# yyNoBug/VAE_segmentation

Measured on AMD Instinct MI355X. Metric: 3D train-step volumes/sec at 96^3 batch=2 (joint VAE+seg), higher is better.
Workload: dtype bf16; 1 GPU; configs[1]: 96^3 joint VAE+seg training step (joint_train), batch=2/GPU, bf16 activations + fp32 accumulate, SGD momentum 0.9, VAE frozen, HIP-graph replay; global_batch=2, parallelism=dp1, activation_recomputation=False, tail_in_graph=True, nranks=1, grad_exchange=none (1 rank)

## Files before the change

### include/vaeseg.h

```cpp
#ifndef VAESEG_H
#define VAESEG_H
#include <stddef.h>
#include <stdint.h>

#ifdef __cplusplus
extern "C" {
#endif

#define VS_VERSION 500

enum { VS_F32 = 0, VS_BF16 = 1, VS_F16 = 2, VS_F32X3 = 3  };
#ifndef VS_STAT_SLOTS
#define VS_STAT_SLOTS 4
#endif
enum { VS_OK = 0, VS_EINVAL = -1, VS_ESHAPE = -2, VS_EDTYPE = -3, VS_EWORKSPACE = -4, VS_EALIGN = -5 };

enum {
    VS_CONV_K3 = 0,
    VS_CONV_K2S2 = 1,
    VS_CONV_T2S2 = 2,
    VS_WGRAD_SLABS = 16,
    VS_CONV_UP = 3
};

// ... 1 lines not shown
    VS_PACK_ROWS_D0 = 0,
    VS_PACK_ROWS_D1_FLIP = 1,
    VS_PACK_SCATTER_D1 = 2
};

int vs_version(void);
int vs_stat_slots(void);
int vs_stat_interleaved(void);
const char* vs_strerror(int code);
int vs_get_deterministic(void);

int vs_up_supported(int cin, int cm, int co, int dtype);
int vs_up_compose_sizes(int cin, int cm, int co, size_t* out6);
int vs_up_compose(const float* w2, const float* b2, const float* w3, float* weff, void* img_fwd, void* img_bwd, int* taps_fwd, int* taps_bwd,
                  float* btab, int cin, int cm, int co, int dtype, void* stream);
int vs_up_conv_fwd(const void* x, const double* x_stats, const void* img_fwd, const int* taps_fwd, const float* btab, void* y, double* y_stats,
                   int n, int d, int h, int w, int cin, int co, int dtype, float eps, void* stream);
int vs_up_faces(const void* gy, double* G, int n, int fd, int fh, int fw, int co, int dtype, void* stream);
int vs_up_chain(const float* dweff27, const double* G, const float* w2, const float* b2, const float* w3, float* dw2, float* db2, float* dw3,
                int cin, int cm, int co, void* stream);
int vs_up_conv_bwd_data(const void* gy, const void* img_bwd, const int* taps_bwd, void* gx, const void* mask_x, const double* mask_stats,
                        double* sums, int n, int d, int h, int w, int co, int cin, int dtype, float eps, void* stream);

size_t vs_packed_weight_bytes(int rows, int c_pad, int ntaps, int dtype);
int vs_pack_weight(const float* src, void* dst, int d0, int d1, int ntaps, int c_pad, int form, int dtype, void* stream);

typedef struct vs_pack_desc {
    const float* src;
    void* dst;
    int d0, d1, ntaps, c_pad, form, dtype;
    int first_block;
    int pad_;
    long long total;
} vs_pack_desc;
int vs_pack_weight_multi(const vs_pack_desc* descs, int n_desc, int total_blocks, void* stream);

int vs_conv_gather_fwd(const void* x, const double* x_stats, const void* w_packed, const float* bias,
                       void* y, double* y_stats, int n, int d, int h, int w, int c_in, int m_out,
                       int kind, int dtype, float eps, void* stream);

int vs_conv_scatter_fwd(const void* x, const double* x_stats, const void* w_packed, const float* bias,
                        void* y, int n, int d, int h, int w, int c_in, int m_out, int dtype, float eps, void* stream);

int vs_conv_gather_bwd_data(const void* x, const void* w_packed, void* y, const void* mask_x, const double* mask_stats,
                            double* sums, int n, int d, int h, int w, int c_in, int m_out, int kind, int dtype, float eps,
                            void* stream);
int vs_conv_scatter_bwd_data(const void* x, const void* w_packed, void* y, const void* mask_x, const double* mask_stats,
                             double* sums, int n, int d, int h, int w, int c_in, int m_out, int dtype, float eps, void* stream);
int vs_conv_k3_fused_apply_supported(int n, int d, int h, int w, int c_in, int m_out, int lazy_input, int dtype);
int vs_conv_k3_bwd_data_wgrad_supported(int n, int d, int h, int w, int c_in, int m_out, int dtype);
int vs_conv_k3_bwd_data_wgrad_slabs(int n, int d, int h, int w);
int vs_conv_k3_bwd_data_wgrad(const void* g, const void* act_x, const double* act_stats, const double* act_sums, const void* w_packed, void* y,
                              const void* mask_x, const double* mask_stats, double* sums, float* slabs, int n, int d, int h, int w, int c_in,
                              int m_out, int dtype, float eps, void* stream);
int vs_conv_k3_softmax2_bwd_data(const float* prob, const float* gprob, const void* gprob_cl, const void* w_packed, void* y, const void* mask_x,
                                 const double* mask_stats, double* sums, float* slabs, double* bias_part, int n, int d, int h, int w, int dtype,
                                 float eps, float drop_p, unsigned long long drop_seed, void* stream);
typedef struct vs_config {
    int k3_small;
    int k3_tall;
    int k3_wgs_per_cu;
    int k3t_wgs_per_cu;
    int k3f_min_wgs;
    int mt_min_wgs;
    int f32_limbs;
    int g1_limbs;
    int k3x_ck;
    int k3x_toeplitz;
    int fuse_wgrad;
    int epilogue_apply;
    int chain;
    int k2s2_stream;
    int k2s8_wgs_per_cu;
    int up_wgs_per_cu;
    int up_rb;
    int wgrad_uber;
    int wgrad_mpack;
    int wgrad_swap;
    int wgrad_big;
    int wgrad_xcd;
    int k3_short_tiles;
    int wgrad_bias_fold;
    int hist_form;
    long long wgrad_wgs;
    long long wgrad_f32_tiles;
    long long wgrad_group_wgs;
    long long wgrad_big_min_voxels;
} vs_config;
int vs_config_bytes(void);
int vs_config_from_env(vs_config* c);
int vs_get_config(vs_config* out);
int vs_set_config(const vs_config* cfg);
int vs_conv_k3_bwd_data_applied_supported(int n, int d, int h, int w, int c_in, int m_out, int dtype);
int vs_conv_k3_bwd_data_applied(const void* x, const void* w_packed, void* y, const void* mask_x, const double* mask_stats, double* sums,
                                unsigned int* sync, unsigned int* fault, int n, int d, int h, int w, int c_in, int m_out, int dtype, float eps, void* stream);
int vs_conv_s2_bwd_data_applied_supported(int n, int d, int h, int w, int c_in, int m_out, int scatter, int dtype);
int vs_conv_s2_bwd_data_applied(const void* x, const void* w_packed, void* y, const void* mask_x, const double* mask_stats, double* sums, const void* add,
                                unsigned int* sync, unsigned int* fault, int n, int d, int h, int w, int c_in, int m_out, int scatter, int dtype, float eps,
                                void* stream);
typedef struct vs_chain_layer {
    const void* x;
    const double* x_stats;
    const void* w_packed;
    void* y;
    double* y_stats;
    const void* mask_x;
    const double* mask_stats;
    double* sums;
    int c_in, m_out;
    int apply;
    int reserved_;
} vs_chain_layer;
int vs_conv_k3_chain_supported(int n, int d, int h, int w, int c_max, int dtype);
long long vs_conv_k3_chain_sync_bytes(int n);
int vs_conv_k3_chain(const vs_chain_layer* layers, int n_layers, int backward, const void* add, unsigned int* sync, unsigned int* fault,
                     int n, int d, int h, int w, int dtype, float eps, void* stream);
int vs_conv_k3_f32_limbs(int d, int h, int w, int c_in);

int vs_conv_k3_bwd_data_fused_apply(const void* g, const void* act_x, const double* act_stats, const double* act_sums,
                                    const void* w_packed, void* y, const void* mask_x, const double* mask_stats, double* sums,
                                    void* dx_out, int n, int d, int h, int w, int c_in, int m_out, int dtype, float eps, void* stream);

int vs_conv_k3_softmax2_fwd(const void* x, const double* x_stats, const void* w_packed, const float* bias,
                            float* prob, int n, int d, int h, int w, int c_in, int dtype, float eps, void* stream);
int vs_conv_k3_softmax2_dropout_fwd(const void* x, const double* x_stats, const void* w_packed, const float* bias,
                                    float* prob, int n, int d, int h, int w, int c_in, int dtype, float eps, float drop_p,
                                    unsigned long long drop_seed, void* stream);
int vs_conv_k3_softmax2_cl_fwd(const void* x, const double* x_stats, const void* w_packed, const float* bias,
                               float* prob, void* prob_cl, int n, int d, int h, int w, int c_in, int dtype, float eps, float drop_p,
                               unsigned long long drop_seed, void* stream);

size_t vs_conv_wgrad_workspace_bytes(int n, int dp, int hp, int wp, int m_ch, int c_ch, int kind);
int vs_conv_wgrad(const void* p, const double* p_stats, const void* q, const double* q_stats, float* dw,
                  void* workspace, size_t workspace_bytes, int n, int dp, int hp, int wp, int m_ch, int c_ch,
                  int m_real, int c_real, int kind, int dtype, float eps, void* stream);
typedef struct vs_wgrad_desc {
    const void* p; const double* p_stats;
    const void* q; const double* q_stats;
    float* dw;
    const void* bias_g; float* db;
    long long bias_rows;
    int bias_c_ch, bias_c_real;
    int n, dp, hp, wp, m_ch, c_ch, m_real, c_real, kind;
    int reserved_;
} vs_wgrad_desc;
size_t vs_conv_wgrad_multi_workspace_bytes(const vs_wgrad_desc* descs, int count, int dtype);
int vs_conv_wgrad_multi(const vs_wgrad_desc* descs, int count, void* workspace, size_t workspace_bytes, int dtype,
                        float eps, void* stream);
int vs_bias_grad(const void* g, float* db, long long rows, int c_ch, int c_real, int dtype, void* stream);
int vs_bias_grad_acc(const void* g, float* db, long long rows, int c_ch, int c_real, int dtype, int accumulate, void* stream);

int vs_instnorm_stats(const void* x, double* stats, int n, long long voxels, int c, int dtype, void* stream);
int vs_instnorm_relu_fwd(const void* x, const double* x_stats, const void* x2, const double* x2_stats,
                         void* out, int n, long long voxels, int c, int dtype, float eps, void* stream);
int vs_instnorm_relu_bwd_reduce(const void* g, const void* x, const double* x_stats, double* sums,
                                int n, long long voxels, int c, int dtype, float eps, void* stream);
int vs_instnorm_relu_bwd_apply(const void* g, const void* x, const double* x_stats, const double* sums,
                               void* gx, int n, long long voxels, int c, int dtype, float eps, void* stream);
int vs_instnorm_relu_bwd_apply_add(const void* g, const void* x, const double* x_stats, const double* sums, const void* add,
                                   void* gx, int n, long long voxels, int c, int dtype, float eps, void* stream);
int vs_zero_fill(void* p, long long bytes, void* stream);
int vs_instnorm_relu_bwd_pair(const void* g, const void* x1, const double* x1_stats, double* sums1, void* gx1,
                              const void* x2, const double* x2_stats, double* sums2, void* gx2, int n, long long voxels,
                              int c, int dtype, float eps, void* stream);

enum { VS_NORM_INSTANCE = 0, VS_NORM_BATCH = 1, VS_NORM_BATCH_EVAL = 2, VS_NORM_NONE = 3 };
// ... 89 lines not shown
int vs_fill_holes(const float* mask, float* out, int n, int c, int d, int h, int w, int connectivity, void* workspace, void* stream);

int vs_region_props(const int* labels, int n, int c, int d, int h, int w, int max_rows, long long* table, int* overflow, void* stream);
int vs_contingency(const int* a, const int* b, int n, int c, int d, int h, int w, int rows_a, int rows_b, long long* table, int* overflow,
                   void* stream);

int vs_histogram(const float* x, const int* labels, int n, int c, int d, int h, int w, int bins, int rows, double lo, double hi, int from_data,
                 double* edges, long long* table, long long* outside, int* overflow, void* stream);
int vs_joint_histogram(const float* x, const float* y, int n, int c, int d, int h, int w, int bins_x, int bins_y, const double* range4, int from_data,
                       double* edges_x, double* edges_y, long long* table, long long* outside, void* stream);
int vs_mutual_information(const long long* table, int n, int c, int bins_x, int bins_y, double sigma, int normalized, double* workspace, double* mi,
                          void* stream);

size_t vs_quantile_workspace_bytes(int planes, long long V, int Q);
int vs_quantile(const float* x, const unsigned char* mask, int use_above, float above, const double* p01, int Q, double* q_out, float* lo_out,
                float* hi_out, long long* count, long long* rejected, void* workspace, int planes, int d, int h, int w, void* stream);
int vs_intensity_map(const float* x, const double* src, const double* dst, int L, int clamp, float* y, int planes, int d, int h, int w, void* stream);

#define VS_PATCH_CHUNK 4096
enum { VS_PATCH_F32 = 0, VS_PATCH_U8 = 1 };
int vs_patch_chunk(void);
size_t vs_patch_index_bytes(int d, int h, int w, int n_class);
int vs_patch_index(const void* label, int dtype, int d, int h, int w, int n_class, int* table, void* stream);
int vs_patch_pick(const void* label, int dtype, const int* table, int n_class, int n_sel, int classes, const unsigned int* words, const int* forced,
                  int r, int d, int h, int w, int pd, int ph, int pw, int* picks, void* stream);
int vs_patch_gather(const float* src0, const float* src1, const float* src2, const float* src3, float cval0, float cval1, float cval2, float cval3,
                    int n_src, const int* picks, int r, int d, int h, int w, int pd, int ph, int pw, int margin, float* out, void* stream);

int vs_sw_plan(int d, int h, int w, int patch, double overlap, int* origins, int capacity);
int vs_sw_gather(const float* volume, float* batch, const int* origins, const int* first, int nw, int b, int c, int d, int h, int w, int patch,
                 float cval, void* stream);
int vs_sw_accumulate(const float* prob, float* acc, float* wsum, const int* origins, const int* first, int nw, int b, int k, int d, int h, int w,
                     int patch, const float* wz, const float* wy, const float* wx, void* stream);
int vs_sw_gather_tta(const float* volume, float* batch, const int* origins, const int* first, int nw, int b, int c, int d, int h, int w, int patch,
                     float cval, int nf, int codes, void* stream);
int vs_sw_accumulate_tta(const float* prob, float* acc, float* wsum, const int* origins, const int* first, int nw, int b, int k, int d, int h, int w,
                         int patch, const float* wz, const float* wy, const float* wx, int nf, int codes, void* stream);
int vs_sw_finalize(const float* acc, const float* wsum, float* prob, unsigned char* label, float* onehot, int k, int d, int h, int w, void* stream);

int vs_uncrop(const float* prob, unsigned char* label, float* prob_out, int k, int patch, int d, int h, int w, int lo_z, int lo_y, int lo_x,
              int hi_z, int hi_y, int hi_x, int off_z, int off_y, int off_x, int side, int interp, void* stream);

enum { VS_SCAN_I16 = 0, VS_SCAN_U8 = 1, VS_SCAN_I8 = 2, VS_SCAN_F32 = 3 };
int vs_scan_orient(const void* raw, int dtype, float* out, int x, int y, int z, int flip0, int flip1, int flip2, void* stream);
int vs_scan_to_native(const void* src, int src_is_label, unsigned char* label, float* prob_out, int k, int d1, int h1, int w1, int x, int y, int z,
                      int flip0, int flip1, int flip2, int interp, void* stream);

int vs_linear_fwd(const void* x, int x_dtype, const float* wgt, const float* bias, float* y, int batch, int k_in,
                  int j_out, int pc, int pv, int relu, void* stream);
int vs_linear_fwd_pair(const void* x, int x_dtype, const float* w1, const float* b1, float* y1, int relu1, const float* w2,
                       const float* b2, float* y2, int relu2, int batch, int k_in, int j_out, int pc, int pv, void* stream);
int vs_linear_fwd_perm_out(const float* z, const float* wgt, const float* bias, void* y, int y_dtype, int batch,
                           int k_in, int j_out, int pc, int pv, void* stream);
int vs_linear_bwd(const void* x, int x_dtype, const float* wgt, const float* gy, const float* y_for_relu,
                  void* gx, float* gw, float* gb, int batch, int k_in, int j_out, int pc, int pv, void* stream);
int vs_linear_perm_out_bwd(const float* z, const float* wgt, const void* gy, int y_dtype, float* gz, float* gw,
                           float* gb, int batch, int k_in, int j_out, int pc, int pv, void* stream);

int vs_reparam_fwd(const float* mean, const float* std_, const float* noise, float scale, float* z, long long count, void* stream);
int vs_reparam_bwd(const float* gz, const float* noise, float scale, float* gmean, float* gstd, long long count, void* stream);
int vs_latent_normal_philox(float* noise, long long count, unsigned long long seed, unsigned long long draw, void* stream);
int vs_reparam_philox_fwd(const float* mean, const float* std_, const unsigned long long* state, float scale, float* z, float* noise_out,
                          long long count, void* stream);
int vs_latent_advance(unsigned long long* state, void* stream);
int vs_kl_fwd(const float* mean, const float* std_, float* out, int batch, int dim, void* stream);
int vs_kl_bwd(const float* mean, const float* std_, const float* gout, float* gmean, float* gstd, int batch, int dim, void* stream);

int vs_dice_fwd(const float* s, const float* t, double* sums, float* per_sample, float* mean_out,
                int batch, int channels, long long voxels, int bot, int top, float eps, void* stream);
int vs_dice_bwd(const float* s, const float* t, const double* sums, const float* gout, int gout_is_mean, float* gs,
                float* gt, int batch, int channels, long long voxels, int bot, int top, float eps, void* stream);
size_t vs_dice_loss_multi_scratch_doubles(int k, int batch, int channels);
int vs_dice_loss_multi_fwd(const float* s, const float* const* t, const float* w, int k, double* scratch, float* terms,
                           float* final_out, int batch, int channels, long long voxels, int bot, int top, float eps, void* stream);
int vs_dice_loss_multi_bwd(const float* s, const float* const* t, const float* w, int k, const double* scratch,
                           const float* gout, float* gs, float* const* gt, int batch, int channels, long long voxels,
                           int bot, int top, float eps, void* stream);
int vs_dice_loss_multi_labels_fwd(const float* s, const float* const* t, const float* const* labels, const float* w, int k, double* scratch,
                                  float* terms, float* final_out, int batch, int channels, long long voxels, int bot, int top, float eps,
                                  void* stream);
int vs_dice_loss_multi_labels_bwd(const float* s, const float* const* t, const float* const* labels, const float* w, int k,
                                  const double* scratch, const float* gout, float* gs, float* const* gt, int batch, int channels,
                                  long long voxels, int bot, int top, float eps, void* stream);
size_t vs_seg_loss_scratch_doubles(int batch, int channels);
int vs_seg_loss_fwd(const float* p, const float* label, const float* class_w, double* scratch, float* terms, float* final_out, int batch, int channels,
                    long long voxels, int bot, int top, float eps, float dice_w, float ce_w, int batch_dice, float gamma, void* stream);
int vs_seg_loss_bwd(const float* p, const float* label, const float* class_w, const double* scratch, const float* gout, float* gp, int batch, int channels,
                    long long voxels, int bot, int top, float eps, float dice_w, float ce_w, int batch_dice, float gamma, void* stream);
int vs_bce_fwd(const float* p, const float* t, float* out, double* scratch, long long count, void* stream);
int vs_bce_bwd(const float* p, const float* t, const float* gout, float* gp, long long count, void* stream);

int vs_sgd_momentum_multi(float* const* params, const float* const* grads, float* const* bufs, const long long* sizes,
                          const int* block_map, int n_blocks, float lr, float momentum, float weight_decay,
                          int first_step, void* stream);
int vs_adam_multi(float* const* params, const float* const* grads, float* const* exp_avg, float* const* exp_avg_sq,
                  const long long* sizes, const int* block_map, int n_blocks, float lr, double beta1, double beta2,
                  float eps, float weight_decay, int step, void* stream);
int vs_sgd_momentum_scaled_multi(float* const* params, const float* const* grads, float* const* bufs, const long long* sizes,
                                 const int* block_map, int n_blocks, float lr, float momentum, float weight_decay,
                                 int first_step, const float* loss_scale, const float* found_inf, void* stream);
int vs_sgd_momentum_dev_multi(float* const* params, const float* const* grads, float* const* bufs, const long long* sizes,
                              const int* block_map, int n_blocks, const float* hyper, const float* loss_scale,
                              const float* found_inf, void* stream);
int vs_adam_scaled_multi(float* const* params, const float* const* grads, float* const* exp_avg, float* const* exp_avg_sq,
                         const long long* sizes, const int* block_map, int n_blocks, float lr, double beta1, double beta2,
                         float eps, float weight_decay, int step, const float* loss_scale, const float* found_inf, void* stream);
int vs_grad_finite_multi(const float* const* grads, const long long* sizes, const int* block_map, int n_blocks,
                         float* found_inf, void* stream);
int vs_loss_scale_update(float* scale, int* growth_tracker, float* found_inf, float growth_factor, float backoff_factor,
                         int growth_interval, void* stream);
int vs_ema_multi(float* const* teacher, const float* const* student, const long long* sizes, const int* block_map,
                 int n_blocks, float alpha, void* stream);
int vs_copy_scale_multi(const float* const* srcs, float* const* dsts, const long long* sizes, const int* block_map,
                        int n_blocks, float scale, void* stream);
int vs_scale_copy(const float* src, float* dst, long long count, float scale, void* stream);

#ifdef __cplusplus
}
#endif
#endif
```

### vae_segmentation_amd/csrc/common.h

```cpp
#pragma once
#include <hip/hip_runtime.h>
#include <stdint.h>
#include <stdlib.h>
#include <type_traits>
#include "../../include/vaeseg.h"

const vs_config& vs_cfg();

typedef __attribute__((ext_vector_type(8))) __bf16 bf16x8;
typedef _Float16 vs_half;
typedef __attribute__((ext_vector_type(8))) _Float16 f16x8;
typedef __attribute__((ext_vector_type(2))) _Float16 f16x2;
typedef __attribute__((ext_vector_type(4))) float f32x4;
typedef __attribute__((ext_vector_type(4))) unsigned int u32x4;
typedef __attribute__((ext_vector_type(2))) unsigned int u32x2;

#define VS_WAVE 64

__device__ __forceinline__ float bf2f(unsigned short h) { return __uint_as_float(((unsigned int)h) << 16); }
__device__ __forceinline__ unsigned short f2bf(float f) {
    __bf16 b = (__bf16)f;
    return __builtin_bit_cast(unsigned short, b);
}
__device__ __forceinline__ float round_bf(float f) { return bf2f(f2bf(f)); }
// ... 192 lines not shown
        r -= q * down[s];
        atomicAdd((unsigned long long*)(st + stat_index(pair, pairs, s) + which), (unsigned long long)(long long)q);
    }
#else
    atomicAdd(st + stat_index(pair, pairs, (int)(blockIdx.x & (VS_STAT_SLOTS - 1))) + which, tot);
#endif
}

__device__ __forceinline__ void pair_to_mean_rstd(const double (&st)[2], double inv_count, float eps, float& mean, float& rstd) {
    double m = st[0] * inv_count;
    double var = st[1] * inv_count - m * m;
    if (var < 0.0) var = 0.0;
    mean = (float)m;
    rstd = (float)(1.0 / sqrt(var + (double)eps));
}
__device__ __forceinline__ void stats_to_mean_rstd(const double* st, size_t pair, size_t pairs, double inv_count, float eps, float& mean, float& rstd) {
    double v[2];
    stat_load(st, pair, pairs, v);
    pair_to_mean_rstd(v, inv_count, eps, mean, rstd);
}

__device__ __forceinline__ void stats_to_mean_rstd_fast(const double* st, double inv_count, float eps, float& mean, float& rstd) {
    const double m = st[0] * inv_count;
    double var = st[1] * inv_count - m * m;
    if (var < 0.0) var = 0.0;
    const float v = (float)(var + (double)eps);
    float r = rsqrtf(v);
    r = r * (1.5f - 0.5f * v * r * r);
    mean = (float)m;
    rstd = r;
}
__device__ __forceinline__ void stats_to_mean_rstd_fast(const double* st, size_t pair, size_t pairs, double inv_count, float eps, float& mean, float& rstd) {
    double v[2];
    stat_load(st, pair, pairs, v);
    stats_to_mean_rstd_fast(v, inv_count, eps, mean, rstd);
}

__device__ __forceinline__ float hash_uniform(unsigned long long seed, unsigned long long idx) {
    unsigned long long x = idx * 0x9E3779B97F4A7C15ull + seed;
    x = (x ^ (x >> 30)) * 0xBF58476D1CE4E5B9ull;
    x = (x ^ (x >> 27)) * 0x94D049BB133111EBull;
    x ^= x >> 31;
    return (float)(x >> 40) * (1.0f / 16777216.0f);
}
__device__ __forceinline__ float dropout_scale(unsigned long long seed, unsigned long long idx, float p) {
    return hash_uniform(seed, idx) >= p ? 1.0f / (1.0f - p) : 0.0f;
}

typedef __attribute__((ext_vector_type(2))) float f32x2;
typedef __attribute__((ext_vector_type(2))) short i16x2;
typedef __attribute__((ext_vector_type(2))) __bf16 bf16x2;
typedef __attribute__((ext_vector_type(4))) int i32x4;

__device__ i32x4 vs_raw_buffer_load_b128(i32x4 rsrc, int voffset, int soffset, int aux) __asm("llvm.amdgcn.raw.buffer.load.v4i32");

typedef __attribute__((ext_vector_type(2))) int i32x2;
__device__ i32x2 vs_raw_buffer_load_b64(i32x4 rsrc, int voffset, int soffset, int aux) __asm("llvm.amdgcn.raw.buffer.load.v2i32");
__device__ int vs_raw_buffer_load_b32(i32x4 rsrc, int voffset, int soffset, int aux) __asm("llvm.amdgcn.raw.buffer.load.i32");
__device__ void vs_raw_buffer_store_b128(i32x4 data, i32x4 rsrc, int voffset, int soffset, int aux) __asm("llvm.amdgcn.raw.buffer.store.v4i32");
__device__ void vs_raw_buffer_store_b64(i32x2 data, i32x4 rsrc, int voffset, int soffset, int aux) __asm("llvm.amdgcn.raw.buffer.store.v2i32");

__device__ __forceinline__ int fdiv(int n, unsigned int m, unsigned int sh) { return (int)((__umulhi((unsigned int)n, m) + (unsigned int)n) >> sh); }

__device__ __forceinline__ i32x4 make_rsrc(const void* base, unsigned int bytes) {
    const unsigned long long a = (unsigned long long)base;
    i32x4 r;
    r[0] = (int)(unsigned int)a;
    r[1] = (int)(unsigned int)((a >> 32) & 0xffffu);
    r[2] = (int)bytes;
    r[3] = 0x00020000;
    return r;
}

__device__ __forceinline__ float vs_in_bwd_apply1(float g, float x, float mean, float rstd, float m1, float m2) {
#pragma clang fp contract(off)
    const float xh = (x - mean) * rstd;
    const float gm = xh > 0.f ? g : 0.f;
    const float base = gm - m1;
    float out = rstd * __builtin_fmaf(-xh, m2, base);
    asm volatile("" : "+v"(out));
    return out;
}

template <typename T> struct H16;
template <> struct H16<unsigned short> {
    __device__ static __forceinline__ unsigned int pack2(f32x2 v) { return __builtin_bit_cast(unsigned int, __builtin_convertvector(v, bf16x2)); }
    __device__ static __forceinline__ float lo(unsigned int w) { return __uint_as_float(w << 16); }
    __device__ static __forceinline__ float hi(unsigned int w) { return __uint_as_float(w & 0xffff0000u); }
};
template <> struct H16<vs_half> {
    __device__ static __forceinline__ unsigned int pack2(f32x2 v) { return __builtin_bit_cast(unsigned int, __builtin_convertvector(v, f16x2)); }
    __device__ static __forceinline__ float lo(unsigned int w) { return (float)__builtin_bit_cast(f16x2, w)[0]; }
    __device__ static __forceinline__ float hi(unsigned int w) { return (float)__builtin_bit_cast(f16x2, w)[1]; }
};

template <typename T>
__device__ __forceinline__ void store4(T* p, const float (&v)[4]) {
    if constexpr (sizeof(T) == 4) {
        *(f32x4*)p = f32x4{v[0], v[1], v[2], v[3]};
    } else {
        u32x2 pk;
        pk[0] = H16<T>::pack2(f32x2{v[0], v[1]});
        pk[1] = H16<T>::pack2(f32x2{v[2], v[3]});
        *(u32x2*)p = pk;
    }
}
template <typename T>
__device__ __forceinline__ void widen4(const unsigned int* w, float (&v)[4]) {
    if constexpr (sizeof(T) == 4) {
        v[0] = __uint_as_float(w[0]); v[1] = __uint_as_float(w[1]); v[2] = __uint_as_float(w[2]); v[3] = __uint_as_float(w[3]);
    } else {
        v[0] = H16<T>::lo(w[0]); v[1] = H16<T>::hi(w[0]); v[2] = H16<T>::lo(w[1]); v[3] = H16<T>::hi(w[1]);
    }
}

template <typename T>
__device__ __forceinline__ u32x4 act8(const u32x4 raw, const f32x2 (&sc)[4], const f32x2 (&sh)[4]) {
    u32x4 r;
#pragma unroll
    for (int i = 0; i < 4; ++i) {
        f32x2 v;
        v[0] = H16<T>::lo(raw[i]);
        v[1] = H16<T>::hi(raw[i]);
        v = v * sc[i] + sh[i];
        i16x2 s = __builtin_bit_cast(i16x2, H16<T>::pack2(v));
        s = __builtin_elementwise_max(s, i16x2{0, 0});
        r[i] = __builtin_bit_cast(unsigned int, s);
    }
    return r;
}

__device__ __forceinline__ void vs_limb_split4(const float (&v)[4], unsigned int (&out)[3][2]) {
#pragma unroll
    for (int q = 0; q < 2; ++q) {
        const f32x2 x = f32x2{v[2 * q], v[2 * q + 1]};
        const unsigned int p0 = H16<unsigned short>::pack2(x);
        const f32x2 r1 = x - f32x2{H16<unsigned short>::lo(p0), H16<unsigned short>::hi(p0)};
        const unsigned int p1 = H16<unsigned short>::pack2(r1);
        const f32x2 r2 = r1 - f32x2{H16<unsigned short>::lo(p1), H16<unsigned short>::hi(p1)};
        out[0][q] = p0; out[1][q] = p1; out[2][q] = H16<unsigned short>::pack2(r2);
    }
}

__device__ __forceinline__ void vs_limb_pair(const u32x4& f0, const u32x4& f1, u32x4 (&out)[3]) {
    float v0[4], v1[4];
#pragma unroll
    for (int j = 0; j < 4; ++j) { v0[j] = __uint_as_float(f0[j]); v1[j] = __uint_as_float(f1[j]); }
    unsigned int l0[3][2], l1[3][2];
    vs_limb_split4(v0, l0);
    vs_limb_split4(v1, l1);
#pragma unroll
    for (int l = 0; l < 3; ++l) out[l] = u32x4{l0[l][0], l0[l][1], l1[l][0], l1[l][1]};
}
__device__ __forceinline__ void vs_limb_mfma(const u32x4 (&al)[3], const u32x4 (&bl)[3], f32x4& lead, f32x4& small) {
    small = mfma16(al[0], bl[2], small, (unsigned short*)nullptr);
    small = mfma16(al[1], bl[1], small, (unsigned short*)nullptr);
    small = mfma16(al[2], bl[0], small, (unsigned short*)nullptr);
    small = mfma16(al[0], bl[1], small, (unsigned short*)nullptr);
    small = mfma16(al[1], bl[0], small, (unsigned short*)nullptr);
    lead = mfma16(al[0], bl[0], lead, (unsigned short*)nullptr);
}

static __host__ __device__ inline bool vs_k3_toeplitz(int rows, int c_pad, int ntaps, int dtype) {
    return (dtype == VS_BF16 || dtype == VS_F16) && ntaps == 27 && c_pad == 8 && rows <= 8;
}
static __host__ __device__ inline bool vs_k3_toeplitz_f32(int rows, int c_pad, int ntaps, int dtype) {
// ... 38 lines not shown
```

### vae_segmentation_amd/csrc/config.hip

```cpp
#include <mutex>
#include <stdlib.h>
#include "common.h"

static vs_config g_cfg;
static std::once_flag g_cfg_once;
static std::mutex g_cfg_mutex;

static int env_int(const char* name, int dflt) { const char* s = getenv(name); return s ? atoi(s) : dflt; }
static long long env_ll(const char* name, long long dflt) { const char* s = getenv(name); return s ? atoll(s) : dflt; }

extern "C" int vs_config_from_env(vs_config* c) {
    if (!c) return VS_EINVAL;
    c->k3_small = env_int("VS_K3_SMALL", 1);
    c->k3_tall = env_int("VS_K3_TALL", -1);
    c->k3_wgs_per_cu = env_int("VS_K3_WGS_PER_CU", 0);
    c->k3t_wgs_per_cu = env_int("VS_K3T_WGS_PER_CU", 2);
    c->k3f_min_wgs = env_int("VS_K3F_MIN_WGS", 512);
    c->mt_min_wgs = env_int("VS_MT_MIN_WGS", 1024);
    c->f32_limbs = env_int("VS_F32_LIMBS", 1);
    c->g1_limbs = env_int("VS_G1_LIMBS", 1);
    c->k3x_ck = env_int("VS_K3X_CK", 8);
    c->k3x_toeplitz = env_int("VS_K3X_TOEPLITZ", 1);
    c->fuse_wgrad = env_int("VS_FUSE_WGRAD", 1);
    c->epilogue_apply = env_int("VS_EPILOGUE_APPLY", 1);
    c->chain = env_int("VS_CHAIN", 1);
    c->k2s2_stream = env_int("VS_K2S2_STREAM", 1);
    c->k2s8_wgs_per_cu = env_int("VS_K2S8_WGS_PER_CU", 4);
    c->up_wgs_per_cu = env_int("VS_UP_WGS_PER_CU", 2);
    c->up_rb = env_int("VS_UP_RB", 0);
    c->wgrad_uber = env_int("VS_WGRAD_UBER", 1);
    c->wgrad_mpack = env_int("VS_WGRAD_MPACK", 1);
    c->wgrad_swap = env_int("VS_WGRAD_SWAP", 1);
    c->wgrad_big = env_int("VS_WGRAD_BIG", 1);
    c->wgrad_xcd = env_int("VS_WGRAD_XCD", 2);
    c->k3_short_tiles = env_int("VS_K3_SHORT_TILES", 2);
    c->wgrad_bias_fold = env_int("VS_WGRAD_BIAS_FOLD", 1);
    c->hist_form = env_int("VS_HIST_FORM", 0);
    c->wgrad_wgs = env_ll("VS_WGRAD_WGS", 512);
    c->wgrad_f32_tiles = env_ll("VS_WGRAD_F32_TILES", 8);
    c->wgrad_group_wgs = env_ll("VS_WGRAD_GROUP_WGS", 0);
    c->wgrad_big_min_voxels = env_ll("VS_WGRAD_BIG_MIN_VOXELS", 400000);
    return VS_OK;
}

const vs_config& vs_cfg() {
    std::call_once(g_cfg_once, [] { vs_config_from_env(&g_cfg); });
    return g_cfg;
}

extern "C" int vs_config_bytes(void) { return (int)sizeof(vs_config); }

extern "C" int vs_get_config(vs_config* out) {
    if (!out) return VS_EINVAL;
    const vs_config& c = vs_cfg();
    std::lock_guard<std::mutex> lock(g_cfg_mutex);
    *out = c;
    return VS_OK;
}

extern "C" int vs_set_config(const vs_config* in) {
    if (!in) return VS_EINVAL;
    if (in->k3x_ck != 8 && in->k3x_ck != 16) return VS_EINVAL;
    if (in->k3_wgs_per_cu < 0 || in->k3t_wgs_per_cu < 1 || in->k2s8_wgs_per_cu < 1 || in->up_wgs_per_cu < 1 || in->wgrad_wgs < 1 || in->wgrad_f32_tiles < 1 ||
        in->wgrad_group_wgs < 0 || in->wgrad_big_min_voxels < 0 || in->mt_min_wgs < 0 || in->k3f_min_wgs < 0 || in->hist_form < 0 || in->hist_form > 3) return VS_EINVAL;
    vs_cfg();
    std::lock_guard<std::mutex> lock(g_cfg_mutex);
    g_cfg = *in;
    return VS_OK;
}
```

### vae_segmentation_amd/csrc/conv_api.hip

```cpp
#include <stdlib.h>
#include "igemm_dispatch.h"

int g1_dispatch_k3_f32(const G1Params& p, int ck, int mt, int epi, int tiles, int row_tiles, hipStream_t s);
int g1_dispatch_k3_bf16(const G1Params& p, int ck, int mt, int epi, int tiles, int row_tiles, hipStream_t s);
int g1_dispatch_k3_f16(const G1Params& p, int ck, int mt, int epi, int tiles, int row_tiles, hipStream_t s);
int g1_dispatch_k3_x3(const G1Params& p, int ck, int mt, int epi, int tiles, int row_tiles, hipStream_t s);
int g1_k3_fa_supported(const G1Params& p, int ck, int mt, int lazy_in);
int g1_k3_ea_supported(const G1Params& p, int ck, int mt, long long wgs);
int k3x_fa_supported(const G1Params& p, int ck, int mt);
int k3x_ea_supported(const G1Params& p, int ck, int mt, long long wgs);
int k3tw_slab_count(int n, int d, int h, int w);
int k2s2_scatter8_launch(const G1Params& p, int dtype, hipStream_t stream);

extern "C" int vs_conv_k3_f32_limbs(int d, int h, int w, int c_in) {
    const int on = vs_cfg().f32_limbs;
    if (!on) return 0;
    const int small = vs_cfg().k3_small;
    if (small && c_in % 32 == 0 && c_in <= 1024 && (long long)(d + 2) * (h + 2) * (w + 2) <= 512) return 0;
    return 1;
}

struct ConvTiles { int ck, mt, row_tiles; bool limbs; };

static ConvTiles k3_tiles(G1Params& p, int dtype, int ck, int mt, int rows16, long long tiles) {
// ... 220 lines not shown
    return plan_wgrad(n, d, h, w, c_in, m_out, false, dtype).status == VS_OK;
}

extern "C" int vs_conv_k3_bwd_data_wgrad_slabs(int n, int d, int h, int w) {
    if (n <= 0 || d <= 0 || h <= 0 || w <= 0) return 0;
    return k3tw_slab_count(n, d, h, w);
}

extern "C" int vs_conv_k3_bwd_data_wgrad(const void* g, const void* act_x, const double* act_stats, const double* act_sums, const void* w_packed, void* y,
                                         const void* mask_x, const double* mask_stats, double* sums, float* slabs, int n, int d, int h, int w, int c_in,
                                         int m_out, int dtype, float eps, void* stream) {
    if (!g || !slabs || !mask_x || !mask_stats || !sums) return VS_EINVAL;
    if ((act_x == nullptr) != (act_stats == nullptr) || (act_x == nullptr) != (act_sums == nullptr)) return VS_EINVAL;
    const ConvPlan pl = plan_wgrad(n, d, h, w, c_in, m_out, act_x != nullptr, dtype);
    if (pl.status) return VS_ESHAPE;
    if (((uintptr_t)slabs & 15) || (act_x && ((uintptr_t)act_x & 15))) return VS_EALIGN;
    G1Params p = bwd_params(pl, g, w_packed, y, mask_x, mask_stats, sums, eps);
    p.x_stats = act_stats; p.fa_x = act_x; p.fa_sums = act_sums; p.wg_ws = slabs;
    return launch_conv(pl, p, stream);
}

extern "C" int vs_conv_k3_softmax2_bwd_data(const float* prob, const float* gprob, const void* gprob_cl, const void* w_packed, void* y, const void* mask_x,
                                            const double* mask_stats, double* sums, float* slabs, double* bias_part, int n, int d, int h, int w, int dtype,
                                            float eps, float drop_p, unsigned long long drop_seed, void* stream) {
    if (!prob || (!gprob && !gprob_cl) || !w_packed || !y || !mask_x || !mask_stats || !sums) return VS_EINVAL;
    if (bias_part && !slabs) return VS_EINVAL;
    const ConvPlan pl = plan_wgrad(n, d, h, w, 8, 8, false, dtype);
    if (pl.status) return VS_ESHAPE;
    if (((uintptr_t)w_packed & 15) || ((uintptr_t)y & 15) || ((uintptr_t)mask_x & 15) || (gprob_cl && ((uintptr_t)gprob_cl & 15)) || (slabs && ((uintptr_t)slabs & 15)) ||
        ((uintptr_t)prob & 3) || ((uintptr_t)gprob & 3)) return VS_EALIGN;
    if (!(drop_p >= 0.f && drop_p < 1.f)) return VS_EINVAL;
    G1Params p = bwd_params(pl, nullptr, w_packed, y, mask_x, mask_stats, sums, eps);
    p.sm_prob = prob; p.sm_gprob = gprob; p.sm_gcl = gprob_cl; p.wg_ws = slabs; p.wg_bias = bias_part;
    p.drop_p = drop_p; p.drop_seed = drop_seed;
    return dispatch_k3(p, dtype, pl.t, EPI_RAW, 0, (hipStream_t)stream);
}

extern "C" int vs_conv_scatter_fwd(const void* x, const double* x_stats, const void* w_packed, const float* bias, void* y,
                                   int n, int d, int h, int w, int c_in, int m_out, int dtype, float eps, void* stream) {
    const ConvPlan pl = plan_scatter({n, d, h, w, c_in, m_out, VS_CONV_T2S2, dtype, (x_stats ? X_STATS : 0) | (bias ? BIAS : 0)});
    G1Params p = pl.g;
    p.x = x; p.x_stats = x_stats; p.wp = w_packed; p.bias = bias; p.y = y; p.eps = eps;
    return launch_conv(pl, p, stream);
}

extern "C" int vs_conv_scatter_bwd_data(const void* x, const void* w_packed, void* y, const void* mask_x, const double* mask_stats, double* sums,
                                        int n, int d, int h, int w, int c_in, int m_out, int dtype, float eps, void* stream) {
    if (!mask_x || !mask_stats || !sums) return VS_EINVAL;
    const ConvPlan pl = plan_scatter({n, d, h, w, c_in, m_out, VS_CONV_T2S2, dtype, SUMS});
    return launch_conv(pl, bwd_params(pl, x, w_packed, y, mask_x, mask_stats, sums, eps), stream);
}

static ConvPlan plan_s2_applied(int n, int d, int h, int w, int c_in, int m_out, int scatter, int dtype) {
    return scatter ? plan_scatter({n, d, h, w, c_in, m_out, VS_CONV_T2S2, dtype, SUMS | EA}) : plan_gather({n, d, h, w, c_in, m_out, VS_CONV_K2S2, dtype, SUMS | EA});
}
extern "C" int vs_conv_s2_bwd_data_applied_supported(int n, int d, int h, int w, int c_in, int m_out, int scatter, int dtype) {
    return plan_s2_applied(n, d, h, w, c_in, m_out, scatter, dtype).status == VS_OK;
}

extern "C" int vs_conv_s2_bwd_data_applied(const void* x, const void* w_packed, void* y, const void* mask_x, const double* mask_stats, double* sums, const void* add,
                                           unsigned int* sync, unsigned int* fault, int n, int d, int h, int w, int c_in, int m_out, int scatter, int dtype, float eps,
                                           void* stream) {
    if (!mask_x || !mask_stats || !sums || !sync || !fault) return VS_EINVAL;
    if (((uintptr_t)sync & 127) || ((uintptr_t)fault & 3) || (add && ((uintptr_t)add & 15))) return VS_EALIGN;
    const ConvPlan pl = plan_s2_applied(n, d, h, w, c_in, m_out, scatter, dtype);
    if (pl.status) return VS_ESHAPE;
    G1Params p = bwd_params(pl, x, w_packed, y, mask_x, mask_stats, sums, eps);
    p.ea_sync = sync; p.ea_fault = fault; p.ea_add = add;
    return launch_conv(pl, p, stream);
}

extern "C" int vs_conv_k3_softmax2_fwd(const void* x, const double* x_stats, const void* w_packed, const float* bias,
                                       float* prob, int n, int d, int h, int w, int c_in, int dtype, float eps,
                                       void* stream) {
    return vs_conv_k3_softmax2_dropout_fwd(x, x_stats, w_packed, bias, prob, n, d, h, w, c_in, dtype, eps, 0.f, 0ull, stream);
}

extern "C" int vs_conv_k3_softmax2_dropout_fwd(const void* x, const double* x_stats, const void* w_packed, const float* bias,
                                               float* prob, int n, int d, int h, int w, int c_in, int dtype, float eps,
                                               float drop_p, unsigned long long drop_seed, void* stream) {
    return vs_conv_k3_softmax2_cl_fwd(x, x_stats, w_packed, bias, prob, nullptr, n, d, h, w, c_in, dtype, eps, drop_p, drop_seed, stream);
}

extern "C" int vs_conv_k3_softmax2_cl_fwd(const void* x, const double* x_stats, const void* w_packed, const float* bias, float* prob, void* prob_cl,
                                          int n, int d, int h, int w, int c_in, int dtype, float eps, float drop_p, unsigned long long drop_seed, void* stream) {
    if (drop_p < 0.f || drop_p >= 1.f) return VS_EINVAL;
    if (prob_cl && dtype == VS_F32) return VS_EDTYPE;
    if (prob_cl && ((uintptr_t)prob_cl & 15)) return VS_EALIGN;
    int rc = check_common(x, w_packed, n, d, h, w, c_in, dtype);
    if (rc) return rc;
    if (!prob || c_in != 8) return VS_ESHAPE;
    const ConvPlan pl = plan_gather({n, d, h, w, 8, 8, VS_CONV_K3, dtype, 0});
    G1Params p = pl.g;
    p.x = x; p.x_stats = x_stats; p.wp = w_packed; p.bias = bias; p.y = prob_cl; p.prob = prob; p.eps = eps;
    p.drop_p = drop_p; p.drop_seed = drop_seed;
    return dispatch_k3(p, dtype, pl.t, EPI_SOFTMAX2, (int)pl.tiles, (hipStream_t)stream);
}
```

### vae_segmentation_amd/csrc/igemm.h

```cpp
#pragma once
#include <type_traits>
#include "common.h"
#include "handoff.h"

enum { G1_K3 = 0, G1_K2S2 = 1, G1_PW = 2 };
enum { EPI_RAW = 0, EPI_SOFTMAX2 = 1, EPI_SCATTER = 2 };

struct G1Params {
    const void* x;
    const double* x_stats;
    const void* wp;
    const float* bias;
    void* y;
    double* y_stats;
    float* prob;
    const void* mask_x;
    const double* mask_stats;
    double* sums;
    double inv_count_out;
    float drop_p;
    unsigned long long drop_seed;
    int N, D, H, W;
    int Do, Ho, Wo;
    int C;
    int M;
    int rb_total;
    int nch;
    int tiles_per_sample;
    int tyn, txn;
    float eps;
    double inv_count_in;
    unsigned int fd_m[3], fd_s[3];
    const void* fa_x;
    const double* fa_sums;
    void* fa_dx;
    const void* up_taps;
    const float* up_btab;
    int up_co;
    float* wg_ws;
    const float* sm_prob;
    const float* sm_gprob;
    const void* sm_gcl;
    double* wg_bias;
    unsigned int* ea_sync;
    unsigned int* ea_fault;
    int ea_items;
    const void* ea_add;
};

#define G1_LDS_MEAN 0
#define G1_LDS_RSTD 2048
#define G1_LDS_RED 4096
#define G1_LDS_BYTES 6144
#define G1_TILE_VOX 648

template <typename T, int CK>
__device__ __forceinline__ u32x4 act_transform(u32x4 raw, const float* s_mean, const float* s_rstd, int c0) {
    constexpr int EPL = ET<T>::EPL;
    float v[EPL];
    frag_unpack(raw, v, (T*)nullptr);
#pragma unroll
    for (int j = 0; j < EPL; ++j) {
        float t = (v[j] - s_mean[c0 + j]) * s_rstd[c0 + j];
        v[j] = t > 0.f ? t : 0.f;
    }
    return frag_pack(v, (T*)nullptr);
}

template <typename T, int CK, int KIND, int MT, int EPI, bool LIMB = false, bool EA = false>
__global__ __launch_bounds__(256) void g1_kernel(const G1Params p) {
    using E = ET<T>;
    constexpr int EPL = E::EPL, KG = E::KG;
    static_assert(!LIMB || sizeof(T) == 4, "limb arithmetic: fp32 storage");
    static_assert(KIND == G1_K2S2 || KIND == G1_PW, "the 3x3x3 kernels live in igemm_k3b.h / igemm_k3.h");
    static_assert(EPI == EPI_RAW || EPI == EPI_SCATTER, "softmax epilogue: 3x3x3 kernels only");
    constexpr int NTAPS = KIND == G1_K2S2 ? 8 : 1;
    constexpr int NKG = (NTAPS * CK + KG - 1) / KG;
    constexpr int RB = MT / 16;
    constexpr int CKB = CK * (int)sizeof(T);
    constexpr int TPK = KG > CK ? KG / CK : 1;
    constexpr int KPT = KG > CK ? 1 : CK / KG;
    extern __shared__ __attribute__((aligned(16))) char smem[];
    float* s_mean = (float*)(smem + G1_LDS_MEAN);
    float* s_rstd = (float*)(smem + G1_LDS_RSTD);
    float* s_red = (float*)(smem + G1_LDS_RED);

    const int tid = threadIdx.x;
    const int lane = tid & 63;
    const int wave = tid >> 6;
    const int col = lane & 15;
    const int g = lane >> 4;
    const int n = blockIdx.x / p.tiles_per_sample;
    const int tile = blockIdx.x - n * p.tiles_per_sample;
    const int rb0 = blockIdx.y * RB;
    const bool has_stats = p.x_stats != nullptr;
    const T* __restrict__ xin = (const T*)p.x;

    if (has_stats) {
        for (int c = tid; c < p.C; c += 256) {
            float m, r;
            stats_to_mean_rstd(p.x_stats, (size_t)n * p.C + c, (size_t)p.N * p.C, p.inv_count_in, p.eps, m, r);
            s_mean[c] = m;
            s_rstd[c] = r;
        }
    }
    if (p.sums != nullptr) {
        for (int c = tid; c < p.M; c += 256) {
            float m, r;
            stats_to_mean_rstd(p.mask_stats, (size_t)n * p.M + c, (size_t)p.N * p.M, p.inv_count_out, p.eps, m, r);
            s_mean[c] = m;
            s_rstd[c] = r;
        }
    }
    const bool splitw = KIND == G1_K2S2 && CK == 32 && p.tyn == 64;
    const int cwave = splitw ? 0 : wave;
    const int ctile = splitw ? 64 : 256;
    long long gofs[4];
    bool cvalid[4];
    int oz[4], oy[4], ox[4];
    {
        const int vcol = p.Do * p.Ho * p.Wo;
#pragma unroll
        for (int cg = 0; cg < 4; ++cg) {
            int v = tile * ctile + cwave * 64 + cg * 16 + col;
            cvalid[cg] = v < vcol;
            if (!cvalid[cg]) v = 0;
            ox[cg] = v % p.Wo;
            const int t2 = v / p.Wo;
            oy[cg] = t2 % p.Ho;
            oz[cg] = t2 / p.Ho;
// ... 429 lines not shown
```

### vae_segmentation_amd/csrc/igemm_k3t.h

```cpp
#pragma once
#include <stdlib.h>
#include "igemm_tile.h"

#define K3T_LDS_RED 0
#define K3T_LDS_TILE 512

template <int YT>
struct K3TGeom {
    static constexpr int PX = 34, PY = YT + 2, PLANE = PX * PY, TV = 6 * PLANE;
    static constexpr int TILE_BYTES = ((TV + 255) / 256) * 256 * 16;
    static constexpr int NIT = (TV + 255) / 256;
};

template <int EPI, bool SUMS, int YT, bool HS, typename T = unsigned short, bool FA = false>
__global__ __launch_bounds__(256) __attribute__((amdgpu_waves_per_eu(2, 2))) void k3t_kernel(const G1Params p) {
    K3_TICK_INIT
    using GEO = K3TGeom<YT>;
    constexpr int PX = GEO::PX, PY = GEO::PY, PLANE = GEO::PLANE, TV = GEO::TV, NIT = GEO::NIT;
    extern __shared__ __attribute__((aligned(16))) char smem[];
    float* s_red = (float*)(smem + K3T_LDS_RED);
    char* s_tile = smem + K3T_LDS_TILE;
    float* s_scale = (float*)(s_tile + GEO::TILE_BYTES);
    float* s_shift = s_scale + p.N * 8;
    float* s_mkm = s_shift + p.N * 8;
    float* s_mkr = s_mkm + p.N * 8;
    float* s_fa = s_mkr + p.N * 8;
    static_assert(!FA || (!HS && EPI == EPI_RAW), "fused apply: backward-data use (materialised gradient in), with or without the fused IN-backward sums");

    const int tid = threadIdx.x, lane = tid & 63, wave = tid >> 6, col = lane & 15, g = lane >> 4;
    const int dx2 = g >> 1, c4 = 4 * (g & 1);
    constexpr bool has_stats = HS;
    const int total_tiles = p.tiles_per_sample * p.N;
    const i32x4 xrsrc = make_rsrc(p.x, (unsigned int)((long long)p.N * p.D * p.H * p.W * 16));
    const i32x4 frsrc = make_rsrc(FA ? p.fa_x : p.x, (unsigned int)((long long)p.N * p.D * p.H * p.W * 16));
    const i32x4 dxrsrc = make_rsrc(FA && p.fa_dx != nullptr ? p.fa_dx : p.y, (FA && p.fa_dx != nullptr) ? (unsigned int)((long long)p.N * p.D * p.H * p.W * 16) : 0u);

    const double* st_src = SUMS ? p.mask_stats : p.x_stats;
    const int st_n = SUMS ? p.N * 8 : (has_stats ? p.N * 8 : 0);
    double st_pre[2] = {0.0, 1.0};
    if (tid < st_n) stat_load(st_src, (size_t)tid, (size_t)st_n, st_pre);
    double fa_pre[2][2] = {{0.0, 1.0}, {0.0, 0.0}};
    if constexpr (FA) {
        if (tid >= 64 && tid < 64 + p.N * 8) {
            stat_load(p.x_stats, (size_t)(tid - 64), (size_t)p.N * 8, fa_pre[0]);
            stat_load(p.fa_sums, (size_t)(tid - 64), (size_t)p.N * 8, fa_pre[1]);
        }
    }

    int rel_off[NIT], tzyx[NIT];
    unsigned int cbits = 0;
#pragma unroll
    for (int b = 0; b < NIT; ++b) {
        const int tv = tid + b * 256;
        const int tx_ = tv % PX, ty_ = (tv / PX) % PY, tz_ = tv / PLANE;
        rel_off[b] = ((tz_ * p.H + ty_) * p.W + tx_) * 16;
        tzyx[b] = tv < TV ? (tz_ | (ty_ << 8) | (tx_ << 16)) : 0x00ffffff;
        cbits |= (tv < TV && tz_ >= 1 && tz_ <= 4 && ty_ >= 1 && ty_ <= YT && tx_ >= 1 && tx_ <= 32) ? (1u << b) : 0u;
    }
    u32x4 xv[NIT], fv[FA ? NIT : 1];
    unsigned int okbits = 0;
    auto load_x = [&](const TileCoord& c) {
        const int base = (((c.n * p.D + c.z0 - 1) * p.H + c.y0 - 1) * p.W + c.x0 - 1) * 16;
        okbits = 0;
#pragma unroll
        for (int b = 0; b < NIT; ++b) {
            const int gz = c.z0 - 1 + (tzyx[b] & 0xff), gy = c.y0 - 1 + ((tzyx[b] >> 8) & 0xff), gx = c.x0 - 1 + (tzyx[b] >> 16);
            const bool ok = (unsigned)gz < (unsigned)p.D && (unsigned)gy < (unsigned)p.H && (unsigned)gx < (unsigned)p.W;
            okbits |= ok ? (1u << b) : 0u;
            xv[b] = __builtin_bit_cast(u32x4, vs_raw_buffer_load_b128(xrsrc, ok ? base + rel_off[b] : -1, 0, 0));
            if constexpr (FA) fv[b] = __builtin_bit_cast(u32x4, vs_raw_buffer_load_b128(frsrc, ok ? base + rel_off[b] : -1, 0, 0));
        }
    };
    auto write_x_fa = [&](const TileCoord& c) {
        f32x2 r2[4], s2[4], a2[4], b2[4];
#pragma unroll
        for (int i = 0; i < 4; ++i) {
            r2[i] = *(const f32x2*)(s_fa + 0 * p.N * 8 + c.n * 8 + 2 * i);
            s2[i] = *(const f32x2*)(s_fa + 1 * p.N * 8 + c.n * 8 + 2 * i);
            a2[i] = *(const f32x2*)(s_fa + 2 * p.N * 8 + c.n * 8 + 2 * i);
            b2[i] = *(const f32x2*)(s_fa + 3 * p.N * 8 + c.n * 8 + 2 * i);
        }
        const int base = (((c.n * p.D + c.z0 - 1) * p.H + c.y0 - 1) * p.W + c.x0 - 1) * 16;
#pragma unroll
        for (int b = 0; b < NIT; ++b) {
            u32x4 v;
#pragma unroll
            for (int i = 0; i < 4; ++i) {
                f32x2 g2, x2;
                g2[0] = H16<T>::lo(xv[b][i]); g2[1] = H16<T>::hi(xv[b][i]);
                x2[0] = H16<T>::lo(fv[b][i]); x2[1] = H16<T>::hi(fv[b][i]);
                const f32x2 xh = x2 * r2[i] + s2[i];
                f32x2 gm;
                gm[0] = xh[0] > 0.f ? g2[0] : 0.f;
                gm[1] = xh[1] > 0.f ? g2[1] : 0.f;
                const f32x2 d = r2[i] * (gm - a2[i] - xh * b2[i]);
                v[i] = H16<T>::pack2(d);
            }
            const bool ok = (okbits >> b) & 1u;
#pragma unroll
            for (int i = 0; i < 4; ++i) v[i] = ok ? v[i] : 0u;
            *(u32x4*)(s_tile + (tid + b * 256) * 16) = v;
            if (p.fa_dx != nullptr)
                vs_raw_buffer_store_b128(__builtin_bit_cast(i32x4, v), dxrsrc, (ok && ((cbits >> b) & 1u)) ? base + rel_off[b] : -1, 0, 0);
        }
    };
    auto write_x = [&](int n) {
        f32x2 sc[4], sh[4];
        if (has_stats) {
#pragma unroll
            for (int i = 0; i < 4; ++i) {
                sc[i] = *(const f32x2*)(s_scale + n * 8 + 2 * i);
                sh[i] = *(const f32x2*)(s_shift + n * 8 + 2 * i);
            }
        }
#pragma unroll
        for (int b = 0; b < NIT; ++b) {
            u32x4 v = xv[b];
            if (has_stats) {
                const u32x4 a = act8<T>(v, sc, sh);
                const bool ok = (okbits >> b) & 1u;
#pragma unroll
                for (int i = 0; i < 4; ++i) v[i] = ok ? a[i] : 0u;
            }
            *(u32x4*)(s_tile + (tid + b * 256) * 16) = v;
        }
    };

    int t, t_end, G;
    tile_walk(total_tiles, t, t_end, G);
    TileCoord cur = tile_coord<YT, 32>(p, t < t_end ? t : 0), nxt = cur;
    u32x4 wa[9];
    {
        const u32x4* __restrict__ wp = (const u32x4*)p.wp;
#pragma unroll
        for (int kg = 0; kg < 9; ++kg) wa[kg] = wp[kg * 64 + lane];
    }
    if (t < t_end) load_x(cur);
    float bv[4];
#pragma unroll
    for (int r = 0; r < 4; ++r) bv[r] = (p.bias != nullptr && c4 + r < (EPI == EPI_SOFTMAX2 ? 2 : p.M)) ? p.bias[c4 + r] : 0.f;
    const i32x4 yrsrc = make_rsrc(p.y, (unsigned int)((long long)p.N * p.D * p.H * p.W * 16));
    const i32x4 mrsrc = make_rsrc(p.mask_x, (unsigned int)((long long)p.N * p.D * p.H * p.W * 16));
    for (int i = tid; i < st_n; i += 256) {
        double st[2] = {st_pre[0], st_pre[1]};
        if (i != tid) stat_load(st_src, (size_t)i, (size_t)st_n, st);
        float m, r;
        stats_to_mean_rstd_fast(st, SUMS ? p.inv_count_out : p.inv_count_in, p.eps, m, r);
        if constexpr (SUMS) { s_mkm[i] = m; s_mkr[i] = r; }
        else { s_scale[i] = r; s_shift[i] = -m * r; }
    }
    if constexpr (FA) {
        if (tid >= 64 && tid < 64 + p.N * 8) {
            const int i = tid - 64;
            float m, r;
            stats_to_mean_rstd_fast(fa_pre[0], p.inv_count_in, p.eps, m, r);
            s_fa[0 * p.N * 8 + i] = r;
            s_fa[1 * p.N * 8 + i] = -m * r;
            s_fa[2 * p.N * 8 + i] = (float)(fa_pre[1][0] * p.inv_count_in);
            s_fa[3 * p.N * 8 + i] = (float)(fa_pre[1][1] * p.inv_count_in);
        }
    }
    const char* s_b = s_tile + ((wave * PY) * PX + 2 * col + g) * 16;
    float ssum[4] = {0.f, 0.f, 0.f, 0.f}, ssq[4] = {0.f, 0.f, 0.f, 0.f};
#pragma unroll
    for (int r = 0; r < 4; ++r) asm volatile("" : "+v"(bv[r]));
#pragma unroll
    for (int kg = 0; kg < 9; ++kg) asm volatile("" : "+v"(wa[kg]));
    bool first = true;
    __syncthreads();
    K3_TICK(0);

    for (; t < t_end; t += G) {
        const int n = cur.n, z0 = cur.z0, y0 = cur.y0, x0 = cur.x0;
        const int oz = z0 + wave, ox = x0 + 2 * col + dx2;
        const int ebase = ((((n * p.D + oz) * p.H + y0) * p.W + ox) * 8 + c4) * 2;
        const bool zx_ok = oz < p.D && ox < p.W;
        if (!first) __syncthreads();
        first = false;
        K3_TICK(1);
        if constexpr (FA) write_x_fa(cur); else write_x(n);
        K3_TICK(2);
        __syncthreads();
        K3_TICK(3);
        u32x2 mk[YT];
        if constexpr (SUMS) {
#pragma unroll
            for (int cg = 0; cg < YT; ++cg)
                mk[cg] = __builtin_bit_cast(u32x2, vs_raw_buffer_load_b64(mrsrc, (zx_ok && y0 + cg < p.H) ? ebase + cg * p.W * 16 : -1, 0, 0));
        }
        nxt = tile_coord<YT, 32>(p, t + G < t_end ? t + G : t);
        if (t + G < t_end) load_x(nxt);
        K3_TICK(4);

        f32x4 acc[YT];
#pragma unroll
        for (int cg = 0; cg < YT; ++cg) acc[cg] = f32x4{0.f, 0.f, 0.f, 0.f};
#pragma unroll
        for (int tz = 0; tz < 3; ++tz) {
            u32x4 fb[PY];
#pragma unroll
            for (int yy = 0; yy < PY; ++yy) fb[yy] = *(const u32x4*)(s_b + ((tz * PY + yy) * PX) * 16);
#pragma unroll
            for (int ty = 0; ty < 3; ++ty)
#pragma unroll
                for (int cg = 0; cg < YT; ++cg) acc[cg] = mfma16(wa[tz * 3 + ty], fb[cg + ty], acc[cg], (T*)nullptr);
            __builtin_amdgcn_sched_barrier(0);
        }

        K3_TICK(5);
        if constexpr (EPI == EPI_SOFTMAX2) {
            const size_t V = (size_t)p.D * p.H * p.W;
#pragma unroll
            for (int cg = 0; cg < YT; ++cg) {
                const int oy = y0 + cg;
                const bool valid = zx_ok && oy < p.H;
                float l0 = acc[cg][0] + bv[0], l1 = acc[cg][1] + bv[1];
                const size_t v = ((size_t)oz * p.H + oy) * p.W + ox;
                if (p.drop_p > 0.f) {
                    l0 *= dropout_scale(p.drop_seed, ((unsigned long long)n * 2 + 0) * V + v, p.drop_p);
                    l1 *= dropout_scale(p.drop_seed, ((unsigned long long)n * 2 + 1) * V + v, p.drop_p);
                }
                const float mx = fmaxf(l0, l1);
                const float e0 = __expf(l0 - mx), e1 = __expf(l1 - mx);
                const float inv = 1.f / (e0 + e1);
                if (valid && (g & 1) == 0) {
                    p.prob[((size_t)n * 2 + 0) * V + v] = e0 * inv;
                    p.prob[((size_t)n * 2 + 1) * V + v] = e1 * inv;
                }
                if (p.y != nullptr) {
                    f32x2 pr;
                    pr[0] = e0 * inv; pr[1] = e1 * inv;
                    i32x2 pk;
                    pk[0] = (g & 1) == 0 ? (int)H16<T>::pack2(pr) : 0;
                    pk[1] = 0;
                    vs_raw_buffer_store_b64(pk, yrsrc, valid ? ebase + cg * p.W * 16 : -1, 0, 0);
                }
            }
        } else {
            float mm[4] = {0.f, 0.f, 0.f, 0.f}, mr[4] = {0.f, 0.f, 0.f, 0.f};
            if constexpr (SUMS) {
#pragma unroll
                for (int r = 0; r < 4; ++r) { mm[r] = s_mkm[n * 8 + c4 + r]; mr[r] = s_mkr[n * 8 + c4 + r]; }
            }
#pragma unroll
            for (int cg = 0; cg < YT; ++cg) {
                const bool valid = zx_ok && y0 + cg < p.H;
                f32x2 lo, hi;
                lo[0] = acc[cg][0] + bv[0]; lo[1] = acc[cg][1] + bv[1];
                hi[0] = acc[cg][2] + bv[2]; hi[1] = acc[cg][3] + bv[3];
                i32x2 pk;
                pk[0] = (int)H16<T>::pack2(lo);
                pk[1] = (int)H16<T>::pack2(hi);
                vs_raw_buffer_store_b64(pk, yrsrc, valid ? ebase + cg * p.W * 16 : -1, 0, 0);
                float v[4];
                v[0] = H16<T>::lo((unsigned int)pk[0]); v[1] = H16<T>::hi((unsigned int)pk[0]);
                v[2] = H16<T>::lo((unsigned int)pk[1]); v[3] = H16<T>::hi((unsigned int)pk[1]);
                if (!valid) { v[0] = 0.f; v[1] = 0.f; v[2] = 0.f; v[3] = 0.f; }
                if constexpr (SUMS) {
                    const u32x2 xx = mk[cg];
                    float xv4[4];
                    xv4[0] = H16<T>::lo(xx[0]); xv4[1] = H16<T>::hi(xx[0]);
                    xv4[2] = H16<T>::lo(xx[1]); xv4[3] = H16<T>::hi(xx[1]);
#pragma unroll
                    for (int r = 0; r < 4; ++r) {
                        const float xh = (xv4[r] - mm[r]) * mr[r];
                        const float gm = xh > 0.f ? v[r] : 0.f;
                        ssum[r] += gm; ssq[r] += gm * xh;
                    }
                } else {
#pragma unroll
                    for (int r = 0; r < 4; ++r) { ssum[r] += v[r]; ssq[r] += v[r] * v[r]; }
                }
            }
            double* const red_dst0 = SUMS ? p.sums : p.y_stats;
            double* const red_dst = red_dst0;
            if (red_dst != nullptr) {
                const bool flush = t + G >= t_end || nxt.n != n;
                if (flush) {
#pragma unroll
                    for (int r = 0; r < 4; ++r) {
                        float s = ssum[r], q = ssq[r];
                        { s = row16_sum(s); q = row16_sum(q); }
                        s += __shfl_xor(s, 32, 64); q += __shfl_xor(q, 32, 64);
                        if (col == 0 && dx2 == 0) {
                            s_red[(wave * 8 + c4 + r) * 2 + 0] = s;
                            s_red[(wave * 8 + c4 + r) * 2 + 1] = q;
                        }
                        ssum[r] = 0.f; ssq[r] = 0.f;
                    }
                    __syncthreads();
                    if (tid < 16) {
                        const int ch = tid >> 1, st = tid & 1;
                        if (ch < p.M) {
                            const double tot = (double)s_red[(0 * 8 + ch) * 2 + st] + (double)s_red[(1 * 8 + ch) * 2 + st] +
                                               (double)s_red[(2 * 8 + ch) * 2 + st] + (double)s_red[(3 * 8 + ch) * 2 + st];
                            stat_add(red_dst, (size_t)n * 8 + ch, (size_t)p.N * 8, st, tot);
                        }
                    }
                }
            }
        }
        cur = nxt;
        K3_TICK(6);
    }
    K3_TICK_FLUSH;
}

template <typename T, int EPI, bool SUMS, int YT, bool HS, bool FA = false>
static int k3t_launch_t(const G1Params& p_in, hipStream_t stream) {
    using GEO = K3TGeom<YT>;
    G1Params p = p_in;
    if (p.C != 8 || p.M != 8) return VS_ESHAPE;
    if (FA && p.N * 8 > 192) return VS_ESHAPE;
    const size_t lds = K3T_LDS_TILE + (size_t)GEO::TILE_BYTES + (size_t)(FA ? 8 : 4) * p.N * 8 * sizeof(float);
    if (lds > 160 * 1024) return VS_ESHAPE;
    p.txn = (p.W + 31) / 32;
    p.tyn = (p.H + YT - 1) / YT;
    p.tiles_per_sample = ((p.D + 3) / 4) * p.tyn * p.txn;
    const long long tiles = (long long)p.tiles_per_sample * p.N;
    if ((long long)p.N * p.D * p.H * p.W * 16 >= 2147483648ll || tiles >= 2147483647ll) return VS_ESHAPE;
    tile_fastdiv_fill(p);
    if (SUMS != (p.sums != nullptr) || (SUMS && !FA && p.x_stats != nullptr)) return VS_EINVAL;
    if (FA && (!p.x_stats || !p.fa_x || !p.fa_sums)) return VS_EINVAL;
    auto kern = k3t_kernel<EPI, SUMS, YT, HS, T, FA>;
    static const hipError_t attr_err =
        hipFuncSetAttribute((const void*)kern, hipFuncAttributeMaxDynamicSharedMemorySize, 160 * 1024);
    if (attr_err != hipSuccess) return (int)attr_err;
    const int per_cu = vs_cfg().k3t_wgs_per_cu;
    const int cap = 256 * per_cu;
    const int gx = tiles < cap ? (int)tiles : cap;
    hipLaunchKernelGGL(kern, dim3(gx), dim3(256), lds, stream, p);
    VS_CHECK_LAUNCH();
    return VS_OK;
}

template <typename T, int EPI, bool SUMS, int YT>
static int k3t_launch(const G1Params& p, hipStream_t stream) {
    if constexpr (EPI == EPI_RAW) {
        if (p.fa_x != nullptr) return k3t_launch_t<T, EPI, SUMS, YT, false, true>(p, stream);
    }
    if (!SUMS && p.x_stats != nullptr) return k3t_launch_t<T, EPI, SUMS, YT, !SUMS>(p, stream);
    return k3t_launch_t<T, EPI, SUMS, YT, false>(p, stream);
}
```

### vae_segmentation_amd/csrc/igemm_k3tw.h

```cpp
#pragma once
#include <stdlib.h>
#include "igemm_tile.h"
#include "igemm_k3t.h"

typedef __attribute__((ext_vector_type(4))) short k3tw_s16x4;
typedef __attribute__((address_space(3))) k3tw_s16x4 k3tw_lds_s16x4;
__device__ __forceinline__ u32x4 pw_tr_pair(const char* s_base, int off0, int off1) {
    const k3tw_s16x4 lo = __builtin_amdgcn_ds_read_tr16_b64_v4i16((k3tw_lds_s16x4*)(s_base + off0));
    const k3tw_s16x4 hi = __builtin_amdgcn_ds_read_tr16_b64_v4i16((k3tw_lds_s16x4*)(s_base + off1));
    typedef __attribute__((ext_vector_type(8))) short s16x8;
    const s16x8 v = __builtin_shufflevector(lo, hi, 0, 1, 2, 3, 4, 5, 6, 7);
    return __builtin_bit_cast(u32x4, v);
}

#define K3TW_Q_BYTES 16384
#define K3TW_ACC_BYTES (4 * 6 * 64 * 16)
#define K3TW_SLAB_ELEMS 1728

template <typename T, int MODE, bool WG>
__global__ __launch_bounds__(256) __attribute__((amdgpu_waves_per_eu(2, 2))) void k3tw_kernel(const G1Params p) {
    constexpr int YT = 8;
    constexpr bool FA = MODE == 1, SM = MODE == 2;
    static_assert(WG || SM, "without the weight gradient this is k3t_kernel, except for the softmax-backward staging");
    using GEO = K3TGeom<YT>;
    constexpr int PX = GEO::PX, PY = GEO::PY, PLANE = GEO::PLANE, TV = GEO::TV, NIT = GEO::NIT;
    extern __shared__ __attribute__((aligned(16))) char smem[];
    float* s_red = (float*)(smem + K3T_LDS_RED);
    char* s_tile = smem + K3T_LDS_TILE;
    char* s_q = s_tile + GEO::TILE_BYTES;
    f32x4* s_acc = (f32x4*)(s_q + K3TW_Q_BYTES);
    float* s_scale = (float*)((char*)s_acc + K3TW_ACC_BYTES);
    float* s_shift = s_scale + p.N * 8;
    float* s_mkm = s_shift + p.N * 8;
    float* s_mkr = s_mkm + p.N * 8;
    float* s_fa = s_mkr + p.N * 8;

    const int tid = threadIdx.x, lane = tid & 63, wave = tid >> 6, col = lane & 15, g = lane >> 4;
    const int dx2 = g >> 1, c4 = 4 * (g & 1);
    const int total_tiles = p.tiles_per_sample * p.N;
    const long long vol = (long long)p.D * p.H * p.W;
    const i32x4 xrsrc = make_rsrc(SM ? (const void*)p.sm_prob : p.x, (unsigned int)(SM ? p.N * vol * 8 : p.N * vol * 16));
    const i32x4 frsrc = make_rsrc(FA ? p.fa_x : (SM ? p.sm_gcl : p.x), (unsigned int)((FA || (SM && p.sm_gcl != nullptr)) ? p.N * vol * 16 : 0));
    const i32x4 grsrc = make_rsrc(SM ? (const void*)p.sm_gprob : p.x, (unsigned int)((SM && p.sm_gprob != nullptr) ? p.N * vol * 8 : 0));

    const double* st_src = p.mask_stats;
    const int st_n = p.N * 8;
    double st_pre[2] = {0.0, 1.0};
    if (tid < st_n) stat_load(st_src, (size_t)tid, (size_t)st_n, st_pre);
    double fa_pre[2][2] = {{0.0, 1.0}, {0.0, 0.0}};
    if constexpr (FA) {
        if (tid >= 64 && tid < 64 + p.N * 8) {
            stat_load(p.x_stats, (size_t)(tid - 64), (size_t)p.N * 8, fa_pre[0]);
            stat_load(p.fa_sums, (size_t)(tid - 64), (size_t)p.N * 8, fa_pre[1]);
        }
    }

    int rel_off[NIT], tzyx[NIT];
#pragma unroll
    for (int b = 0; b < NIT; ++b) {
        const int tv = tid + b * 256;
        const int tx_ = tv % PX, ty_ = (tv / PX) % PY, tz_ = tv / PLANE;
        rel_off[b] = ((tz_ * p.H + ty_) * p.W + tx_) * 16;
        tzyx[b] = tv < TV ? (tz_ | (ty_ << 8) | (tx_ << 16)) : 0x00ffffff;
    }
    u32x4 xv[NIT], fv[(FA || SM) ? NIT : 1];
    unsigned int okbits = 0;
    unsigned int cbits = 0;
    float bsum[2] = {0.f, 0.f};
    if constexpr (SM) {
#pragma unroll
        for (int b = 0; b < NIT; ++b) {
            const int tv = tid + b * 256;
            const int tx_ = tv % PX, ty_ = (tv / PX) % PY, tz_ = tv / PLANE;
            cbits |= (tv < TV && tz_ >= 1 && tz_ <= 4 && ty_ >= 1 && ty_ <= YT && tx_ >= 1 && tx_ <= 32) ? (1u << b) : 0u;
        }
    }
    auto load_x = [&](const TileCoord& c) {
        const int base = (((c.n * p.D + c.z0 - 1) * p.H + c.y0 - 1) * p.W + c.x0 - 1) * 16;
        okbits = 0;
#pragma unroll
        for (int b = 0; b < NIT; ++b) {
            const int gz = c.z0 - 1 + (tzyx[b] & 0xff), gy = c.y0 - 1 + ((tzyx[b] >> 8) & 0xff), gx = c.x0 - 1 + (tzyx[b] >> 16);
            const bool ok = (unsigned)gz < (unsigned)p.D && (unsigned)gy < (unsigned)p.H && (unsigned)gx < (unsigned)p.W;
            okbits |= ok ? (1u << b) : 0u;
            if constexpr (SM) {
                const int vi = ((base + rel_off[b]) >> 4) - c.n * (int)vol;
                const int o0 = ok ? ((c.n * 2) * (int)vol + vi) * 4 : -1, o1 = ok ? ((c.n * 2 + 1) * (int)vol + vi) * 4 : -1;
                xv[b][0] = (unsigned int)vs_raw_buffer_load_b32(xrsrc, o0, 0, 0);
                xv[b][1] = (unsigned int)vs_raw_buffer_load_b32(xrsrc, o1, 0, 0);
                xv[b][2] = (unsigned int)vs_raw_buffer_load_b32(grsrc, o0, 0, 0);
                xv[b][3] = (unsigned int)vs_raw_buffer_load_b32(grsrc, o1, 0, 0);
                fv[b] = __builtin_bit_cast(u32x4, vs_raw_buffer_load_b128(frsrc, ok ? base + rel_off[b] : -1, 0, 0));
            } else {
                xv[b] = __builtin_bit_cast(u32x4, vs_raw_buffer_load_b128(xrsrc, ok ? base + rel_off[b] : -1, 0, 0));
                if constexpr (FA) fv[b] = __builtin_bit_cast(u32x4, vs_raw_buffer_load_b128(frsrc, ok ? base + rel_off[b] : -1, 0, 0));
            }
        }
    };
    auto write_x_sm = [&](const TileCoord& c) {
        const int base = (((c.n * p.D + c.z0 - 1) * p.H + c.y0 - 1) * p.W + c.x0 - 1) * 16;
#pragma unroll
        for (int b = 0; b < NIT; ++b) {
            const float p0 = __uint_as_float(xv[b][0]), p1 = __uint_as_float(xv[b][1]);
            const float g0 = __uint_as_float(xv[b][2]) + H16<T>::lo(fv[b][0]), g1 = __uint_as_float(xv[b][3]) + H16<T>::hi(fv[b][0]);
            const float dot = p0 * g0 + p1 * g1;
            f32x2 f;
            f[0] = p0 * (g0 - dot);
            f[1] = p1 * (g1 - dot);
            if (p.drop_p > 0.f) {
                const long long vi = (long long)((base + rel_off[b]) >> 4) - (long long)c.n * vol;
                f[0] *= dropout_scale(p.drop_seed, ((unsigned long long)c.n * 2 + 0) * (unsigned long long)vol + (unsigned long long)vi, p.drop_p);
                f[1] *= dropout_scale(p.drop_seed, ((unsigned long long)c.n * 2 + 1) * (unsigned long long)vol + (unsigned long long)vi, p.drop_p);
            }
            const bool ok = (okbits >> b) & 1u;
            u32x4 v = u32x4{ok ? H16<T>::pack2(f) : 0u, 0u, 0u, 0u};
            *(u32x4*)(s_tile + (tid + b * 256) * 16) = v;
            if (ok && ((cbits >> b) & 1u)) { bsum[0] += H16<T>::lo(v[0]); bsum[1] += H16<T>::hi(v[0]); }
        }
    };
    auto write_x_fa = [&](const TileCoord& c) {
        f32x2 r2[4], s2[4], a2[4], b2[4];
#pragma unroll
        for (int i = 0; i < 4; ++i) {
            r2[i] = *(const f32x2*)(s_fa + 0 * p.N * 8 + c.n * 8 + 2 * i);
            s2[i] = *(const f32x2*)(s_fa + 1 * p.N * 8 + c.n * 8 + 2 * i);
            a2[i] = *(const f32x2*)(s_fa + 2 * p.N * 8 + c.n * 8 + 2 * i);
            b2[i] = *(const f32x2*)(s_fa + 3 * p.N * 8 + c.n * 8 + 2 * i);
        }
#pragma unroll
        for (int b = 0; b < NIT; ++b) {
            u32x4 v;
#pragma unroll
            for (int i = 0; i < 4; ++i) {
                f32x2 g2, x2;
                g2[0] = H16<T>::lo(xv[b][i]); g2[1] = H16<T>::hi(xv[b][i]);
                x2[0] = H16<T>::lo(fv[b][i]); x2[1] = H16<T>::hi(fv[b][i]);
                const f32x2 xh = x2 * r2[i] + s2[i];
                f32x2 gm;
                gm[0] = xh[0] > 0.f ? g2[0] : 0.f;
                gm[1] = xh[1] > 0.f ? g2[1] : 0.f;
                const f32x2 d = r2[i] * (gm - a2[i] - xh * b2[i]);
                v[i] = H16<T>::pack2(d);
            }
            const bool ok = (okbits >> b) & 1u;
#pragma unroll
            for (int i = 0; i < 4; ++i) v[i] = ok ? v[i] : 0u;
            *(u32x4*)(s_tile + (tid + b * 256) * 16) = v;
        }
    };
    auto write_x = [&](int n) {
#pragma unroll
        for (int b = 0; b < NIT; ++b) *(u32x4*)(s_tile + (tid + b * 256) * 16) = xv[b];
    };

    int t, t_end, G;
    tile_walk(total_tiles, t, t_end, G);
    TileCoord cur = tile_coord<YT, 32>(p, t < t_end ? t : 0), nxt = cur;
    u32x4 wa[9];
    {
        const u32x4* __restrict__ wp = (const u32x4*)p.wp;
#pragma unroll
        for (int kg = 0; kg < 9; ++kg) wa[kg] = wp[kg * 64 + lane];
    }
    if (t < t_end) load_x(cur);
    const i32x4 yrsrc = make_rsrc(p.y, (unsigned int)((long long)p.N * p.D * p.H * p.W * 16));
    const i32x4 mrsrc = make_rsrc(p.mask_x, (unsigned int)((long long)p.N * p.D * p.H * p.W * 16));
    for (int i = tid; i < st_n; i += 256) {
        double st[2] = {st_pre[0], st_pre[1]};
        if (i != tid) stat_load(st_src, (size_t)i, (size_t)st_n, st);
        float m, r;
        stats_to_mean_rstd_fast(st, p.inv_count_out, p.eps, m, r);
        s_mkm[i] = m; s_mkr[i] = r;
    }
    if constexpr (FA) {
        if (tid >= 64 && tid < 64 + p.N * 8) {
            const int i = tid - 64;
            float m, r;
            stats_to_mean_rstd_fast(fa_pre[0], p.inv_count_in, p.eps, m, r);
            s_fa[0 * p.N * 8 + i] = r;
            s_fa[1 * p.N * 8 + i] = -m * r;
            s_fa[2 * p.N * 8 + i] = (float)(fa_pre[1][0] * p.inv_count_in);
            s_fa[3 * p.N * 8 + i] = (float)(fa_pre[1][1] * p.inv_count_in);
        }
    }
    const char* s_b = s_tile + ((wave * PY) * PX + 2 * col + g) * 16;
    float ssum[4] = {0.f, 0.f, 0.f, 0.f}, ssq[4] = {0.f, 0.f, 0.f, 0.f};
#pragma unroll
    for (int kg = 0; kg < 9; ++kg) asm volatile("" : "+v"(wa[kg]));

    const int q4 = col >> 2, p4 = col & 3, hi2 = p4 >> 1, half = p4 & 1;
    const int a_lane = ((hi2 * 32) + 4 * g + q4) * 16 + half * 8;
    const int b_lane = (4 * g + q4) * 16 + half * 8;
    int b_blk[6];
    if constexpr (WG) {
#pragma unroll
        for (int j = 0; j < 6; ++j) {
            const int blk = wave + 4 * j;
            const int dz = blk >> 3, dyp = (blk & 7) >> 1, dxb = blk & 1;
            b_blk[j] = ((dz * PY + dyp) * PX + (dxb ? 2 : hi2)) * 16 + b_lane;
            s_acc[(wave * 6 + j) * 64 + lane] = f32x4{0.f, 0.f, 0.f, 0.f};
        }
    }
    bool first = true;
    __syncthreads();

    for (; t < t_end; t += G) {
        const int n = cur.n, z0 = cur.z0, y0 = cur.y0, x0 = cur.x0;
        const int oz = z0 + wave, ox = x0 + 2 * col + dx2;
        const int ebase = ((((n * p.D + oz) * p.H + y0) * p.W + ox) * 8 + c4) * 2;
        const bool zx_ok = oz < p.D && ox < p.W;
        if (!first) __syncthreads();
        first = false;
        if constexpr (FA) write_x_fa(cur); else if constexpr (SM) write_x_sm(cur); else write_x(n);
        __syncthreads();
        u32x2 mk[YT];
#pragma unroll
        for (int cg = 0; cg < YT; ++cg)
            mk[cg] = __builtin_bit_cast(u32x2, vs_raw_buffer_load_b64(mrsrc, (zx_ok && y0 + cg < p.H) ? ebase + cg * p.W * 16 : -1, 0, 0));
        nxt = tile_coord<YT, 32>(p, t + G < t_end ? t + G : t);
        if (t + G < t_end) load_x(nxt);

        f32x4 acc[YT];
#pragma unroll
        for (int cg = 0; cg < YT; ++cg) acc[cg] = f32x4{0.f, 0.f, 0.f, 0.f};
#pragma unroll
        for (int tz = 0; tz < 3; ++tz) {
            u32x4 fb[PY];
#pragma unroll
            for (int yy = 0; yy < PY; ++yy) fb[yy] = *(const u32x4*)(s_b + ((tz * PY + yy) * PX) * 16);
#pragma unroll
            for (int ty = 0; ty < 3; ++ty)
#pragma unroll
                for (int cg = 0; cg < YT; ++cg) acc[cg] = mfma16(wa[tz * 3 + ty], fb[cg + ty], acc[cg], (T*)nullptr);
            __builtin_amdgcn_sched_barrier(0);
        }

        {
            float mm[4], mr[4];
#pragma unroll
            for (int r = 0; r < 4; ++r) { mm[r] = s_mkm[n * 8 + c4 + r]; mr[r] = s_mkr[n * 8 + c4 + r]; }
#pragma unroll
            for (int cg = 0; cg < YT; ++cg) {
                const bool valid = zx_ok && y0 + cg < p.H;
                f32x2 lo, hi;
                lo[0] = acc[cg][0]; lo[1] = acc[cg][1];
                hi[0] = acc[cg][2]; hi[1] = acc[cg][3];
                i32x2 pk;
                pk[0] = (int)H16<T>::pack2(lo);
                pk[1] = (int)H16<T>::pack2(hi);
                vs_raw_buffer_store_b64(pk, yrsrc, valid ? ebase + cg * p.W * 16 : -1, 0, 0);
                float v[4];
                v[0] = H16<T>::lo((unsigned int)pk[0]); v[1] = H16<T>::hi((unsigned int)pk[0]);
                v[2] = H16<T>::lo((unsigned int)pk[1]); v[3] = H16<T>::hi((unsigned int)pk[1]);
                if (!valid) { v[0] = 0.f; v[1] = 0.f; v[2] = 0.f; v[3] = 0.f; }
                const u32x2 xx = mk[cg];
                float xv4[4], qv[4];
                xv4[0] = H16<T>::lo(xx[0]); xv4[1] = H16<T>::hi(xx[0]);
                xv4[2] = H16<T>::lo(xx[1]); xv4[3] = H16<T>::hi(xx[1]);
#pragma unroll
                for (int r = 0; r < 4; ++r) {
                    const float xh = (xv4[r] - mm[r]) * mr[r];
                    const float gm = xh > 0.f ? v[r] : 0.f;
                    ssum[r] += gm; ssq[r] += gm * xh;
                    qv[r] = valid ? fmaxf(fmaf(xv4[r], mr[r], -mm[r] * mr[r]), 0.f) : 0.f;
                }
                if constexpr (WG) {
                    f32x2 q0, q1;
                    q0[0] = qv[0]; q0[1] = qv[1]; q1[0] = qv[2]; q1[1] = qv[3];
                    *(u32x2*)(s_q + ((wave * 8 + cg) * 32 + 2 * col + dx2) * 16 + c4 * 2) = u32x2{H16<T>::pack2(q0), H16<T>::pack2(q1)};
                }
            }
            const bool flush = t + G >= t_end || nxt.n != n;
            if (flush) {
#pragma unroll
                for (int r = 0; r < 4; ++r) {
                    float s = ssum[r], q = ssq[r];
                    { s = row16_sum(s); q = row16_sum(q); }
                    s += __shfl_xor(s, 32, 64); q += __shfl_xor(q, 32, 64);
                    if (col == 0 && dx2 == 0) {
                        s_red[(wave * 8 + c4 + r) * 2 + 0] = s;
                        s_red[(wave * 8 + c4 + r) * 2 + 1] = q;
                    }
                    ssum[r] = 0.f; ssq[r] = 0.f;
                }
                __syncthreads();
                if (tid < 16) {
                    const int ch = tid >> 1, st = tid & 1;
                    const double tot = (double)s_red[(0 * 8 + ch) * 2 + st] + (double)s_red[(1 * 8 + ch) * 2 + st] +
                                       (double)s_red[(2 * 8 + ch) * 2 + st] + (double)s_red[(3 * 8 + ch) * 2 + st];
                    stat_add(p.sums, (size_t)n * 8 + ch, (size_t)p.N * 8, st, tot);
                }
            }
        }

        if constexpr (WG) {
            __syncthreads();
            f32x4 wacc[6];
#pragma unroll
            for (int j = 0; j < 6; ++j) wacc[j] = s_acc[(wave * 6 + j) * 64 + lane];
            u32x4 af[4][4];
#pragma unroll
            for (int z = 0; z < 4; ++z)
#pragma unroll
                for (int s = 0; s < 4; ++s) {
                    const int ao = a_lane + ((z * 8 + 2 * s) * 32) * 16;
                    af[z][s] = pw_tr_pair(s_q, ao, ao + 16 * 16);
                }
            const int b_row0 = b_blk[0];
#pragma unroll
            for (int tz = 0; tz < 6; ++tz) {
                u32x4 rows[5];
#pragma unroll
                for (int k = 0; k < 5; ++k) {
                    const int bn = b_row0 + ((tz * PY + 2 * k) * PX) * 16;
                    rows[k] = pw_tr_pair(s_tile, bn, bn + 16 * 16);
                }
#pragma unroll
                for (int dz = 0; dz < 3; ++dz) {
                    const int z = tz - dz;
                    if (z >= 0 && z <= 3) {
#pragma unroll
                        for (int s = 0; s < 4; ++s) {
                            wacc[2 * dz] = mfma16(af[z][s], rows[s], wacc[2 * dz], (T*)nullptr);
                            wacc[2 * dz + 1] = mfma16(af[z][s], rows[s + 1], wacc[2 * dz + 1], (T*)nullptr);
                        }
                    }
                }
            }
#pragma unroll
            for (int j = 0; j < 6; ++j) s_acc[(wave * 6 + j) * 64 + lane] = wacc[j];
        }
        cur = nxt;
    }

    __syncthreads();
    if constexpr (SM) {
        if (p.wg_bias != nullptr) {
#pragma unroll
            for (int k = 0; k < 2; ++k) {
                float sb = bsum[k];
#pragma unroll
                for (int off = 32; off >= 1; off >>= 1) sb += __shfl_xor(sb, off, 64);
                if (lane == 0) s_red[wave * 2 + k] = sb;
            }
            __syncthreads();
            if (tid < 2) p.wg_bias[(size_t)blockIdx.x * 2 + tid] = (double)s_red[tid] + (double)s_red[2 + tid] + (double)s_red[4 + tid] + (double)s_red[6 + tid];
        }
    }
    if constexpr (WG) {
        float* wsg = p.wg_ws + (size_t)blockIdx.x * 1728;
        const float* s_accf = (const float*)s_acc;
        for (int o = tid; o < 1728; o += 256) {
            const int tap = o >> 6, c = (o >> 3) & 7, m = o & 7;
            const int dz = tap / 9, dy = (tap / 3) % 3, dx = tap % 3;
            const int dxb = dx >> 1, colx = 8 * (dx & 1) + m;
            float v = 0.f;
#pragma unroll
            for (int r = 0; r < 2; ++r) {
                const int blk = dz * 8 + (dy + r) * 2 + dxb;
                const int ln = 16 * (2 * r + (c >> 2)) + colx;
                v += s_accf[((((blk & 3) * 6 + (blk >> 2)) * 64 + ln) << 2) + (c & 3)];
            }
            wsg[o] = v;
        }
    }
}

static inline int k3tw_grid(int n, int d, int h, int w) {
    const int per_cu = vs_cfg().k3t_wgs_per_cu;
    const long long tiles = (long long)((d + 3) / 4) * ((h + 7) / 8) * ((w + 31) / 32) * n;
    const int cap = 256 * per_cu;
    return tiles < cap ? (int)tiles : cap;
}

template <typename T>
static int k3tw_launch(const G1Params& p_in, hipStream_t stream) {
    using GEO = K3TGeom<8>;
    G1Params p = p_in;
    if (p.C != 8 || p.M != 8 || p.N * 8 > 192) return VS_ESHAPE;
    if (!p.sums || !p.mask_x || !p.mask_stats) return VS_EINVAL;
    const bool fa = p.fa_x != nullptr, sm = p.sm_prob != nullptr, wg = p.wg_ws != nullptr;
    if (fa && (sm || !p.x_stats || !p.fa_sums)) return VS_EINVAL;
    if (sm ? (!p.sm_gprob && !p.sm_gcl) : (!wg || !p.x)) return VS_EINVAL;
    if ((long long)p.N * p.D * p.H * p.W * 8 >= 2147483648ll) return VS_ESHAPE;
    const size_t lds = K3T_LDS_TILE + (size_t)GEO::TILE_BYTES + K3TW_Q_BYTES + K3TW_ACC_BYTES + (size_t)8 * p.N * 8 * sizeof(float);
    p.txn = (p.W + 31) / 32;
    p.tyn = (p.H + 7) / 8;
    p.tiles_per_sample = ((p.D + 3) / 4) * p.tyn * p.txn;
    const long long tiles = (long long)p.tiles_per_sample * p.N;
    if ((long long)p.N * p.D * p.H * p.W * 16 >= 2147483648ll || tiles >= 2147483647ll) return VS_ESHAPE;
    tile_fastdiv_fill(p);
    const int gx = k3tw_grid(p.N, p.D, p.H, p.W);
#define K3TW_GO(MODEV, WGV)                                                                                                              \
    {                                                                                                                                    \
        auto kern = k3tw_kernel<T, MODEV, WGV>;                                                                                          \
        static const hipError_t attr_err = hipFuncSetAttribute((const void*)kern, hipFuncAttributeMaxDynamicSharedMemorySize, 160 * 1024); \
        if (attr_err != hipSuccess) return (int)attr_err;                                                                                \
        hipLaunchKernelGGL(kern, dim3(gx), dim3(256), lds, stream, p);                                                                   \
    }
    if (sm) { if (wg) K3TW_GO(2, true) else K3TW_GO(2, false) }
    else if (fa) K3TW_GO(1, true)
    else K3TW_GO(0, true)
#undef K3TW_GO
    VS_CHECK_LAUNCH();
    return VS_OK;
}
```

### vae_segmentation_amd/csrc/misc.hip

```cpp
#include "common.h"
#include "philox.h"
#include <math.h>

extern "C" int vs_get_deterministic(void) { return VS_DET_BUILD; }

extern "C" int vs_version(void) { return VS_VERSION; }
extern "C" int vs_stat_slots(void) { return VS_STAT_SLOTS; }
extern "C" int vs_stat_interleaved(void) { return VS_STAT_INTERLEAVE; }
extern "C" const char* vs_strerror(int code) {
    switch (code) {
        case VS_OK: return "ok";
        case VS_EINVAL: return "invalid argument (null pointer or non-positive size)";
        case VS_ESHAPE: return "unsupported shape (channels must be 8, 16 or a multiple of 32 up to 512; even dims for stride 2; batch <= 16 for wgrad)";
        case VS_EDTYPE: return "unsupported dtype (VS_F32, VS_BF16 or VS_F16)";
        case VS_EWORKSPACE: return "workspace too small";
        case VS_EALIGN: return "pointer not 16-byte aligned";
        default: return code > 0 ? hipGetErrorString((hipError_t)code) : "unknown libvaeseg error";
    }
}

#define GRID1D(n) dim3((unsigned)((((n) + 255) / 256) < 65536LL * 16 ? (((n) + 255) / 256) : 65536LL * 16))

template <typename T>
__global__ void dropout_kernel(const T* __restrict__ x, T* __restrict__ out, long long frags, float p, unsigned long long seed) {
// ... 710 lines not shown
        float m = 0.f;
        for (int i = 0; i < batch; ++i) m += ps[i];
        mean_out[0] = m / batch;
    }
}
extern "C" int vs_dice_fwd(const float* s, const float* t, double* sums, float* per_sample, float* mean_out, int batch,
                           int channels, long long voxels, int bot, int top, float eps, void* stream) {
    if (!s || !t || !sums || batch <= 0 || batch > 64 || channels <= 0 || voxels <= 0 || bot < 0 || top > channels || bot >= top) return VS_EINVAL;
    if (((uintptr_t)s & 15) || ((uintptr_t)t & 15) || (voxels & 3)) return VS_EALIGN;
    hipError_t e = vs_zero_async(sums, sizeof(double) * 3 * batch * channels, (hipStream_t)stream);
    if (e != hipSuccess) return (int)e;
    long long blocks = (voxels / 4 + 256 * 8 - 1) / (256 * 8);
    if (blocks < 1) blocks = 1;
    if (blocks > 1024) blocks = 1024;
    if (VS_DET_BUILD) blocks = 1;
    hipLaunchKernelGGL(dice_sums_kernel, dim3((unsigned)blocks, top - bot, batch), dim3(256), 0, (hipStream_t)stream, s, t, sums, channels, voxels, bot);
    VS_CHECK_LAUNCH();
    hipLaunchKernelGGL(dice_finish_kernel, dim3(1), dim3(64), 0, (hipStream_t)stream, sums, per_sample, mean_out, batch, channels, bot, top, eps);
    VS_CHECK_LAUNCH();
    return VS_OK;
}

__global__ __launch_bounds__(256) void dice_bwd_kernel(const float* __restrict__ s, const float* __restrict__ t, const double* __restrict__ sums,
                                                       const float* __restrict__ gout, int gout_is_mean, int batch,
                                                       float* __restrict__ gs, float* __restrict__ gt,
                                                       int channels, long long voxels, int bot, int top, float eps) {
    const int c = blockIdx.y, b = blockIdx.z;
    const size_t plane = ((size_t)b * channels + c) * voxels;
    const long long v4 = voxels / 4;
    if (c < bot || c >= top) {
        const f32x4 z = f32x4{0.f, 0.f, 0.f, 0.f};
        for (long long i = (long long)blockIdx.x * 256 + threadIdx.x; i < v4; i += (long long)gridDim.x * 256) {
            if (gs) *(f32x4*)(gs + plane + i * 4) = z;
            if (gt) *(f32x4*)(gt + plane + i * 4) = z;
        }
        return;
    }
    const double* q = sums + ((size_t)b * channels + c) * 3;
    const float I = (float)q[0], den = (float)q[1] + (float)q[2] + eps;
    const float g = (gout_is_mean ? gout[0] / (float)batch : gout[b]) / (float)(top - bot);
    const float k1 = g * 2.f / den, k2 = g * 2.f * I / (den * den);
    for (long long i = (long long)blockIdx.x * 256 + threadIdx.x; i < v4; i += (long long)gridDim.x * 256) {
        if (gs) { const f32x4 y = *(const f32x4*)(t + plane + i * 4); *(f32x4*)(gs + plane + i * 4) = f32x4{k1 * y[0] - k2, k1 * y[1] - k2, k1 * y[2] - k2, k1 * y[3] - k2}; }
        if (gt) { const f32x4 x = *(const f32x4*)(s + plane + i * 4); *(f32x4*)(gt + plane + i * 4) = f32x4{k1 * x[0] - k2, k1 * x[1] - k2, k1 * x[2] - k2, k1 * x[3] - k2}; }
    }
}
extern "C" int vs_dice_bwd(const float* s, const float* t, const double* sums, const float* gout, int gout_is_mean, float* gs,
                           float* gt, int batch, int channels, long long voxels, int bot, int top, float eps, void* stream) {
    if (!s || !t || !sums || !gout || batch <= 0 || channels <= 0 || voxels <= 0 || (voxels & 3)) return VS_EINVAL;
    long long blocks = (voxels / 4 + 256 * 4 - 1) / (256 * 4);
    if (blocks > 2048) blocks = 2048;
    hipLaunchKernelGGL(dice_bwd_kernel, dim3((unsigned)blocks, channels, batch), dim3(256), 0, (hipStream_t)stream, s, t, sums, gout, gout_is_mean, batch, gs, gt, channels, voxels, bot, top, eps);
    VS_CHECK_LAUNCH();
    return VS_OK;
}

#define DICE_MULTI_MAX 4
struct DiceMulti {
    const float* s;
    const float* t[DICE_MULTI_MAX];
    const float* lab[DICE_MULTI_MAX];
    float* gt[DICE_MULTI_MAX];
    float w[DICE_MULTI_MAX];
    int k;
};
#define DICE_MULTI_BLOCKS 256
__device__ __forceinline__ f32x4 dice_target4(const DiceMulti& a, int j, size_t plane, int b, int c, long long voxels, long long i) {
    if (a.lab[j] != nullptr) {
        const f32x4 l = *(const f32x4*)(a.lab[j] + (size_t)b * voxels + i * 4);
        return f32x4{(int)l[0] == c ? 1.f : 0.f, (int)l[1] == c ? 1.f : 0.f, (int)l[2] == c ? 1.f : 0.f, (int)l[3] == c ? 1.f : 0.f};
    }
    return *(const f32x4*)(a.t[j] + plane + i * 4);
}
__global__ __launch_bounds__(256) void dice_multi_partial_kernel(const DiceMulti a, double* __restrict__ part, int channels, long long voxels, int bot) {
    const int c = bot + blockIdx.y, b = blockIdx.z, K = a.k;
    const size_t plane = ((size_t)b * channels + c) * voxels;
    const float* sp = a.s + plane;
    double aS = 0.0, aI[DICE_MULTI_MAX], aT[DICE_MULTI_MAX];
#pragma unroll
    for (int j = 0; j < DICE_MULTI_MAX; ++j) { aI[j] = 0.0; aT[j] = 0.0; }
    const long long v4 = voxels / 4;
    for (long long i = (long long)blockIdx.x * 256 + threadIdx.x; i < v4; i += (long long)gridDim.x * 256) {
        const f32x4 x = *(const f32x4*)(sp + i * 4);
        aS += (double)(x[0] + x[1]) + (double)(x[2] + x[3]);
#pragma unroll
        for (int j = 0; j < DICE_MULTI_MAX; ++j) {
            if (j < K) {
                const f32x4 y = dice_target4(a, j, plane, b, c, voxels, i);
                aI[j] += (double)(x[0] * y[0] + x[1] * y[1]) + (double)(x[2] * y[2] + x[3] * y[3]);
                aT[j] += (double)(y[0] + y[1]) + (double)(y[2] + y[3]);
            }
        }
    }
    __shared__ double red[4][1 + 2 * DICE_MULTI_MAX];
    const int wave = threadIdx.x >> 6;
    aS = wave_sum_d(aS);
#pragma unroll
    for (int j = 0; j < DICE_MULTI_MAX; ++j) { aI[j] = wave_sum_d(aI[j]); aT[j] = wave_sum_d(aT[j]); }
    if ((threadIdx.x & 63) == 0) {
        red[wave][0] = aS;
#pragma unroll
        for (int j = 0; j < DICE_MULTI_MAX; ++j) { red[wave][1 + 2 * j] = aI[j]; red[wave][2 + 2 * j] = aT[j]; }
    }
    __syncthreads();
    const int NQ = 1 + 2 * K;
    if (threadIdx.x < NQ) {
        const int q = threadIdx.x;
        part[(((size_t)b * gridDim.y + blockIdx.y) * NQ + q) * gridDim.x + blockIdx.x] = red[0][q] + red[1][q] + red[2][q] + red[3][q];
    }
}

__global__ __launch_bounds__(256) void dice_multi_finish_kernel(const DiceMulti a, const double* __restrict__ part, double* __restrict__ sums,
                                                               float* __restrict__ terms, float* __restrict__ final_out, int batch,
                                                               int channels, int bot, int top, int nblk, float eps) {
    const int K = a.k, NQ = 1 + 2 * K, nc = top - bot;
    __shared__ double s_tot[64 * 2 * (1 + 2 * DICE_MULTI_MAX)];
    __shared__ double s_p16[16][17];
    const int sl = threadIdx.x & 15, sg = threadIdx.x >> 4;
    for (int i0 = 0; i0 < batch * nc * NQ; i0 += 16) {
        const int i = i0 + sg;
        double t = 0.0;
        if (i < batch * nc * NQ) {
            const double* src = part + (size_t)i * nblk;
            int blk = sl;
            for (; blk + 7 * 16 < nblk; blk += 8 * 16) {
                double v[8];
#pragma unroll
                for (int u = 0; u < 8; ++u) v[u] = src[blk + 16 * u];
#pragma unroll
                for (int u = 0; u < 8; ++u) t += v[u];
            }
            for (; blk < nblk; blk += 16) t += src[blk];
        }
        s_p16[sg][sl] = t;
        __syncthreads();
        if (sl == 0 && i < batch * nc * NQ) {
            double tt = 0.0;
#pragma unroll
            for (int u = 0; u < 16; ++u) tt += s_p16[sg][u];
            s_tot[i] = tt;
        }
        __syncthreads();
    }
    for (int i = threadIdx.x; i < batch * nc * NQ; i += 256) {
        const double t = s_tot[i];
        const int q = i % NQ, bc = i / NQ, ci = bc % nc, b = bc / nc;
        if (q == 0) {
            for (int j = 0; j < K; ++j) sums[(((size_t)j * batch + b) * channels + bot + ci) * 3 + 1] = t;
        } else {
            const int j = (q - 1) >> 1;
            sums[(((size_t)j * batch + b) * channels + bot + ci) * 3 + (((q - 1) & 1) ? 2 : 0)] = t;
        }
    }
    __syncthreads();
    __shared__ float s_term[DICE_MULTI_MAX];
    if (threadIdx.x < K) {
        const int j = threadIdx.x;
        float m = 0.f;
        for (int b = 0; b < batch; ++b) {
            float v = 0.f;
            for (int ci = 0; ci < nc; ++ci) {
                const double* q = s_tot + (b * nc + ci) * NQ;
                const float I = (float)q[1 + 2 * j], S = (float)q[0], T = (float)q[2 + 2 * j];
                v += 2.f * I / (S + T + eps);
            }
            m += v / (float)nc;
        }
        const float term = 1.f - m / (float)batch;
        terms[j] = term;
        s_term[j] = term;
    }
    __syncthreads();
    if (threadIdx.x == 0) {
        float f = __fmul_rn(a.w[0], s_term[0]);
        for (int j = 1; j < K; ++j) f = __fadd_rn(f, __fmul_rn(a.w[j], s_term[j]));
        final_out[0] = f;
    }
}

static int dice_multi_args(DiceMulti& a, const float* s, const float* const* t, const float* w, float* const* gt, int k, const float* const* lab = nullptr) {
    if (!s || !t || !w || k <= 0 || k > DICE_MULTI_MAX) return VS_EINVAL;
    a = DiceMulti{};
    a.s = s; a.k = k;
    if ((uintptr_t)s & 15) return VS_EALIGN;
    for (int j = 0; j < k; ++j) {
        const float* lj = lab ? lab[j] : nullptr;
        if (!t[j] && !lj) return VS_EINVAL;
        if (lj && gt && gt[j]) return VS_EINVAL;
        if (((uintptr_t)t[j] & 15) || ((uintptr_t)lj & 15) || (gt && gt[j] && ((uintptr_t)gt[j] & 15))) return VS_EALIGN;
        a.t[j] = lj ? nullptr : t[j]; a.lab[j] = lj; a.w[j] = w[j]; a.gt[j] = gt ? gt[j] : nullptr;
    }
    return VS_OK;
}

extern "C" size_t vs_dice_loss_multi_scratch_doubles(int k, int batch, int channels) {
    if (k <= 0 || batch <= 0 || channels <= 0) return 0;
    return (size_t)3 * k * batch * channels + (size_t)batch * channels * (1 + 2 * k) * DICE_MULTI_BLOCKS;
}

extern "C" int vs_dice_loss_multi_fwd(const float* s, const float* const* t, const float* w, int k, double* scratch, float* terms,
                                      float* final_out, int batch, int channels, long long voxels, int bot, int top, float eps, void* stream) {
    return vs_dice_loss_multi_labels_fwd(s, t, nullptr, w, k, scratch, terms, final_out, batch, channels, voxels, bot, top, eps, stream);
}

extern "C" int vs_dice_loss_multi_labels_fwd(const float* s, const float* const* t, const float* const* labels, const float* w, int k, double* scratch,
                                             float* terms, float* final_out, int batch, int channels, long long voxels, int bot, int top, float eps,
                                             void* stream) {
    DiceMulti a;
    int rc = dice_multi_args(a, s, t, w, nullptr, k, labels);
    if (rc) return rc;
    if (!scratch || !terms || !final_out || batch <= 0 || batch > 64 || channels <= 0 || voxels <= 0 || bot < 0 || top > channels || bot >= top) return VS_EINVAL;
    if (voxels & 3) return VS_EALIGN;
    if ((long long)batch * (top - bot) > 128) return VS_ESHAPE;
    long long blocks = (voxels / 4 + 256 * 2 - 1) / (256 * 2);
    if (blocks < 1) blocks = 1;
    if (blocks > DICE_MULTI_BLOCKS) blocks = DICE_MULTI_BLOCKS;
    double* part = scratch + (size_t)3 * k * batch * channels;
    hipLaunchKernelGGL(dice_multi_partial_kernel, dim3((unsigned)blocks, top - bot, batch), dim3(256), 0, (hipStream_t)stream, a, part, channels,
                       voxels, bot);
    VS_CHECK_LAUNCH();
    hipLaunchKernelGGL(dice_multi_finish_kernel, dim3(1), dim3(256), 0, (hipStream_t)stream, a, part, scratch, terms, final_out, batch, channels,
                       bot, top, (int)blocks, eps);
    VS_CHECK_LAUNCH();
    return VS_OK;
}

__global__ __launch_bounds__(256) void dice_multi_bwd_kernel(const DiceMulti a, const double* __restrict__ sums, const float* __restrict__ gout,
                                                            float* __restrict__ gs, int batch, int channels, long long voxels, int bot,
                                                            int top, float eps) {
    const int c = blockIdx.y, b = blockIdx.z, K = a.k;
    const size_t plane = ((size_t)b * channels + c) * voxels;
    const long long v4 = voxels / 4;
    if (c < bot || c >= top) {
        const f32x4 z = f32x4{0.f, 0.f, 0.f, 0.f};
        for (long long i = (long long)blockIdx.x * 256 + threadIdx.x; i < v4; i += (long long)gridDim.x * 256) {
            if (gs) *(f32x4*)(gs + plane + i * 4) = z;
#pragma unroll
            for (int j = 0; j < DICE_MULTI_MAX; ++j)
                if (j < K && a.gt[j]) *(f32x4*)(a.gt[j] + plane + i * 4) = z;
        }
        return;
    }
    float k1[DICE_MULTI_MAX], k2[DICE_MULTI_MAX], k2sum = 0.f;
    const float g0 = -gout[0] / ((float)batch * (float)(top - bot));
#pragma unroll
    for (int j = 0; j < DICE_MULTI_MAX; ++j) {
        k1[j] = 0.f; k2[j] = 0.f;
        if (j < K) {
            const double* q = sums + (((size_t)j * batch + b) * channels + c) * 3;
            const float I = (float)q[0], den = (float)q[1] + (float)q[2] + eps;
            const float g = g0 * a.w[j];
            k1[j] = g * 2.f / den;
            k2[j] = g * 2.f * I / (den * den);
            k2sum += k2[j];
        }
    }
    for (long long i = (long long)blockIdx.x * 256 + threadIdx.x; i < v4; i += (long long)gridDim.x * 256) {
        const f32x4 x = *(const f32x4*)(a.s + plane + i * 4);
        f32x4 acc = f32x4{-k2sum, -k2sum, -k2sum, -k2sum};
#pragma unroll
        for (int j = 0; j < DICE_MULTI_MAX; ++j) {
            if (j < K) {
                if (gs) {
                    const f32x4 y = dice_target4(a, j, plane, b, c, voxels, i);
                    acc[0] += k1[j] * y[0]; acc[1] += k1[j] * y[1]; acc[2] += k1[j] * y[2]; acc[3] += k1[j] * y[3];
                }
                if (a.gt[j]) *(f32x4*)(a.gt[j] + plane + i * 4) = f32x4{k1[j] * x[0] - k2[j], k1[j] * x[1] - k2[j], k1[j] * x[2] - k2[j], k1[j] * x[3] - k2[j]};
            }
        }
        if (gs) *(f32x4*)(gs + plane + i * 4) = acc;
    }
}

extern "C" int vs_dice_loss_multi_bwd(const float* s, const float* const* t, const float* w, int k, const double* scratch, const float* gout,
                                      float* gs, float* const* gt, int batch, int channels, long long voxels, int bot, int top, float eps,
                                      void* stream) {
    return vs_dice_loss_multi_labels_bwd(s, t, nullptr, w, k, scratch, gout, gs, gt, batch, channels, voxels, bot, top, eps, stream);
}

extern "C" int vs_dice_loss_multi_labels_bwd(const float* s, const float* const* t, const float* const* labels, const float* w, int k,
                                             const double* scratch, const float* gout, float* gs, float* const* gt, int batch, int channels,
                                             long long voxels, int bot, int top, float eps, void* stream) {
    DiceMulti a;
    int rc = dice_multi_args(a, s, t, w, gt, k, labels);
    if (rc) return rc;
    if (!scratch || !gout || batch <= 0 || channels <= 0 || voxels <= 0 || (voxels & 3) || bot < 0 || top > channels || bot >= top) return VS_EINVAL;
    if (gs && ((uintptr_t)gs & 15)) return VS_EALIGN;
    long long blocks = (voxels / 4 + 256 * 4 - 1) / (256 * 4);
    if (blocks > 2048) blocks = 2048;
    hipLaunchKernelGGL(dice_multi_bwd_kernel, dim3((unsigned)blocks, channels, batch), dim3(256), 0, (hipStream_t)stream, a, scratch, gout, gs,
                       batch, channels, voxels, bot, top, eps);
    VS_CHECK_LAUNCH();
    return VS_OK;
}

__global__ __launch_bounds__(256) void bce_sum_kernel(const float* __restrict__ p, const float* __restrict__ t, double* __restrict__ acc, long long count) {
    double s = 0.0;
    for (long long i = (long long)blockIdx.x * 256 + threadIdx.x; i < count; i += (long long)gridDim.x * 256) {
        const float lp = fmaxf(logf(p[i]), -100.f), lq = fmaxf(logf(1.f - p[i]), -100.f);
        s -= (double)(t[i] * lp + (1.f - t[i]) * lq);
    }
    __shared__ double red[4];
    s = wave_sum_d(s);
    if ((threadIdx.x & 63) == 0) red[threadIdx.x >> 6] = s;
    __syncthreads();
    if (threadIdx.x == 0) atomicAdd(acc, red[0] + red[1] + red[2] + red[3]);
}
__global__ void bce_finish_kernel(const double* acc, float* out, long long count) { out[0] = (float)(acc[0] / (double)count); }
__global__ void bce_bwd_kernel(const float* __restrict__ p, const float* __restrict__ t, const float* __restrict__ gout, float* __restrict__ gp, long long count) {
    const float g = gout[0] / (float)count;
    for (long long i = (long long)blockIdx.x * 256 + threadIdx.x; i < count; i += (long long)gridDim.x * 256) {
        const float d = fmaxf(p[i] * (1.f - p[i]), 1e-12f);
        gp[i] = g * (p[i] - t[i]) / d;
    }
}
extern "C" int vs_bce_fwd(const float* p, const float* t, float* out, double* scratch, long long count, void* stream) {
    if (!p || !t || !out || !scratch || count <= 0) return VS_EINVAL;
    hipError_t e = vs_zero_async(scratch, sizeof(double), (hipStream_t)stream);
    if (e != hipSuccess) return (int)e;
    long long blocks = (count + 256 * 16 - 1) / (256 * 16);
    if (blocks > 1024) blocks = 1024;
    if (VS_DET_BUILD) blocks = 1;
    hipLaunchKernelGGL(bce_sum_kernel, dim3((unsigned)blocks), dim3(256), 0, (hipStream_t)stream, p, t, scratch, count);
    VS_CHECK_LAUNCH();
    hipLaunchKernelGGL(bce_finish_kernel, dim3(1), dim3(1), 0, (hipStream_t)stream, scratch, out, count);
    VS_CHECK_LAUNCH();
    return VS_OK;
}
extern "C" int vs_bce_bwd(const float* p, const float* t, const float* gout, float* gp, long long count, void* stream) {
    if (!p || !t || !gout || !gp || count <= 0) return VS_EINVAL;
    hipLaunchKernelGGL(bce_bwd_kernel, GRID1D(count), dim3(256), 0, (hipStream_t)stream, p, t, gout, gp, count);
    VS_CHECK_LAUNCH();
    return VS_OK;
}

#define MT_CHUNK 4096
__global__ __launch_bounds__(256) void sgd_multi_kernel(float* const* params, const float* const* grads, float* const* bufs,
                                                        const long long* sizes, const int* block_map, float lr, float momentum,
                                                        float wd, int first, const float* __restrict__ loss_scale,
                                                        const float* __restrict__ found_inf, const float* __restrict__ hyper) {
    if (found_inf != nullptr && found_inf[0] != 0.f) return;
    if (hyper != nullptr) { lr = hyper[0]; momentum = hyper[1]; wd = hyper[2]; }
    const float inv_scale = loss_scale != nullptr ? 1.f / loss_scale[0] : 1.f;
    const int ti = block_map[2 * blockIdx.x], start = block_map[2 * blockIdx.x + 1];
    float* p = params[ti];
    const float* g = grads[ti];
    float* m = bufs[ti];
    const long long n = sizes[ti];
    const long long end = (long long)start + MT_CHUNK < n ? (long long)start + MT_CHUNK : n;
    constexpr int R = MT_CHUNK / 256;
    if (end - start == MT_CHUNK && ((((uintptr_t)p | (uintptr_t)g | (uintptr_t)m) & 15) == 0)) {
        constexpr int R4 = R / 4;
        f32x4 g4[R4], p4[R4], m4[R4];
// ... 245 lines not shown
```

### vae_segmentation_amd/ops.py

```python
import ctypes as _ctypes
import os
import weakref as _weakref

import torch

from . import _lib
from ._lib import (VS_BF16, VS_CONV_K2S2, VS_CONV_K3, VS_CONV_UP, VS_F16, VS_F32, VS_PACK_ROWS_D0, VS_PACK_ROWS_D1_FLIP,
                   VS_PACK_SCATTER_D1, _contig, _p, _require_cuda, _stream, check, lib)
from .volume import *
from .volume import (PATCH_CHUNK, PATCH_LABEL_DTYPES, PATCH_MAX_CLASSES, PATCH_MAX_SOURCES, patch_gather, patch_index,
                     patch_pick)

_DT_TORCH = {VS_F32: torch.float32, VS_BF16: torch.bfloat16, VS_F16: torch.float16}
_DT_VS = {v: k for k, v in _DT_TORCH.items()}
KERNEL_DTYPES = tuple(_DT_VS)
VS_F32X3 = 3
F32X3 = "f32x3"
_DT_TORCH[VS_F32X3] = F32X3
_DT_VS[F32X3] = VS_F32X3
_F32_LIMBS = bool(lib.vs_conv_k3_f32_limbs(96, 96, 96, 8))


def k3_pack_dtype(x):
    if x.dtype == torch.float32 and lib.vs_conv_k3_f32_limbs(x.shape[1], x.shape[2], x.shape[3], x.shape[4]):
        return F32X3
    return x.dtype


def vs_of(dtype):
    try:
        return _DT_VS[dtype]
    except KeyError:
        raise TypeError("kernel dtype must be float32, bfloat16 or float16, got %s" % (dtype,)) from None

EPS_IN = 1e-5


PROFILE = None


def _esize(t):
    return 4 if t.dtype == torch.float32 else 2


class VsConfig(_ctypes.Structure):
    _fields_ = [(n, _ctypes.c_int) for n in ("k3_small", "k3_tall", "k3_wgs_per_cu", "k3t_wgs_per_cu", "k3f_min_wgs", "mt_min_wgs", "f32_limbs", "g1_limbs", "k3x_ck",
                                            "k3x_toeplitz", "fuse_wgrad", "epilogue_apply", "chain", "k2s2_stream", "k2s8_wgs_per_cu", "up_wgs_per_cu", "up_rb",
                                            "wgrad_uber", "wgrad_mpack", "wgrad_swap", "wgrad_big", "wgrad_xcd", "k3_short_tiles", "wgrad_bias_fold", "hist_form")] + \
               [(n, _ctypes.c_longlong) for n in ("wgrad_wgs", "wgrad_f32_tiles", "wgrad_group_wgs", "wgrad_big_min_voxels")]


def get_config():
    if lib.vs_config_bytes() != _ctypes.sizeof(VsConfig):
        raise _lib.VaesegError("vs_config layout mismatch: the library's struct has %d bytes, this binding %d" % (lib.vs_config_bytes(), _ctypes.sizeof(VsConfig)))
    c = VsConfig()
    check(lib.vs_get_config(_ctypes.addressof(c)), "get_config")
    return {n: getattr(c, n) for n, _ in VsConfig._fields_ if n != "reserved_"}


def set_config(**kw):
    cur = get_config()
    unknown = [k for k in kw if k not in cur]
    if unknown:
        raise KeyError("not a vs_config field: %s" % ", ".join(unknown))
    old = {k: cur[k] for k in kw}
    cur.update(kw)
    c = VsConfig(**cur)
    for l in lib.loaded():
        check(l.vs_set_config(_ctypes.addressof(c)), "set_config")
    return old


class config:

    def __init__(self, **kw):
        self.kw = kw

    def __enter__(self):
        self.old = set_config(**self.kw)
        return self

    def __exit__(self, *exc):
        set_config(**self.old)
        return False


def _pick_mt(rows16, tiles):
    min_wgs = get_config()["mt_min_wgs"]
    for mt in (64, 32, 16):
        if rows16 % mt:
            continue
        if tiles * (rows16 // mt) >= min_wgs or mt == 16:
            return mt
    return 16


def _k3_kid(tname, ck, mt, sums=False, geom=None, m=None, lazy=False):
    if tname == "float":
        return "k3_kernel<float,%d,%d,0>" % (ck, mt)
    hs = "true" if (lazy and not sums) else "false"
    if ck == 8 and m == 8:
        return "k3t_kernel<0,%s,8,%s,%s>" % ("true" if sums else "false", hs, tname)
    cfg = get_config()
    if ck == 32 and geom is not None and (geom[1] + 2) * (geom[2] + 2) * (geom[3] + 2) <= 512 and cfg["k3_small"] != 0:
        tv = (geom[1] + 2) * (geom[2] + 2) * (geom[3] + 2)
        return "k3s_kernel<%s,%d,%s,%s>" % ("true" if sums else "false", 128 if tv <= 128 else 512, hs, tname)
    yt = 4
    if geom is not None and ck == 32 and mt == 16 and m is not None and cfg["k3_short_tiles"]:
        n, d, h, w = geom
        rt = (m + 15) // 16
        zx = n * ((d + 3) // 4) * ((w + 15) // 16)
        if zx * ((h + 3) // 4) * rt <= 128 and zx * ((h + 1) // 2) * rt <= 256:
            yt = 1 if (cfg["k3_short_tiles"] >= 2 and zx * ((h + 1) // 2) * rt <= 128 and zx * h * rt <= 256) else 2
    if geom is not None and ck < 32 and mt == 16 and cfg["k3_tall"] != 0:
        n, d, h, w = geom
        tiles = n * ((d + 3) // 4) * ((h + 3) // 4) * ((w + 15) // 16)
        tall = n * ((d + 3) // 4) * ((h + 7) // 8) * ((w + 15) // 16)
        if cfg["k3_tall"] == 1 or (tall >= 256 and tiles <= 2048):
            yt = 8
    return "k3b_kernel<%d,%d,0,%s,%d,%s,%s>" % (ck, min(mt, 32), "true" if sums else "false", yt, hs, tname)


PROFILE_PRIME_US = 80
PROFILE_SPIN = [None]


class _timed:
    def __init__(self, kid, nbytes, flops, detail=""):
        self.rec = None if PROFILE is None else [kid, float(nbytes), float(flops), detail]

    def __enter__(self):
# ... 893 lines not shown
            keep.append(wp)
            nb += (cur.numel() + y.numel() + wt.numel()) * _esize(x)
            fl += 2.0 * n * d * h * w * 27 * wt.shape[0] * wt.shape[1]
            outs.append((y, ys))
            cur, curs = y, ys
            if ctx.needs_input_grad[2 + 2 * l]:
                _count_use(wt)
        sync = _chain_sync(n, x.device)
        with _timed("k3_chain<%s,fwd,%d>" % (_tname(x), nl), nb, fl, "x%s" % (tuple(x.shape),)):
            check(lib.vs_conv_k3_chain(_ctypes.addressof(layers), nl, 0, None, sync.data_ptr(), _chain_fault_word(x.device).data_ptr(), n, d, h, w,
                                       vs_dtype(x), EPS_IN, _stream()), "conv_k3_chain (forward)")
        ctx.nl = nl
        ctx.bias_refs = biases
        ctx.save_for_backward(x, xs, *[t for pair in outs[:-1] for t in pair], *weights)
        ctx.mark_non_differentiable(outs[-1][1])
        ctx.set_materialize_grads(False)
        return outs[-1]

    @staticmethod
    def backward(ctx, gy, _gys):
        nl = ctx.nl
        saved = ctx.saved_tensors
        none = (None,) * (2 + 2 * nl)
        if gy is None:
            return none
        acts = [(saved[0], saved[1])] + [(saved[2 + 2 * i], saved[3 + 2 * i]) for i in range(nl - 1)]
        weights = saved[2 * nl:]
        gy = _contig(gy)
        lazy = _take_lazy(gy)
        if lazy is not None:
            gy = apply_lazy(gy, lazy)
        n, d, h, w, _ = gy.shape
        dev = gy.device
        layers = (ChainLayer * nl)()
        applied = [None] * nl
        applied[nl - 1] = gy
        g_in, add, keep = gy, None, []
        nb = fl = 0.0
        for k, l in enumerate(range(nl - 1, -1, -1)):
            ax, axs = acts[l]
            wt = weights[l]
            wpb = pack_weight_cached(wt, VS_PACK_ROWS_D1_FLIP, g_in.shape[-1], k3_pack_dtype(g_in))
            g = torch.empty_like(ax)
            sums = _new_stats(n, ax.shape[-1], dev) if axs is not None else None
            if l == 0 and axs is not None:
                add = _collect_gradient(ax)
            layers[k] = ChainLayer(g_in.data_ptr(), None, wpb.data_ptr(), g.data_ptr(), None, ax.data_ptr() if axs is not None else None, _p(axs), _p(sums),
                                   g_in.shape[-1], ax.shape[-1], 1 if axs is not None else 0, 0)
            keep += [wpb, sums]
            nb += (g_in.numel() + (4 if axs is not None else 1) * g.numel() + wt.numel()) * _esize(gy)
            fl += 2.0 * n * d * h * w * 27 * wt.shape[0] * wt.shape[1]
            if l > 0:
                applied[l - 1] = g
            g_in = g
        sync = _chain_sync(n, dev)
        with _timed("k3_chain<%s,bwd,%d>" % (_tname(gy), nl), nb, fl, "gy%s" % (tuple(gy.shape),)):
            check(lib.vs_conv_k3_chain(_ctypes.addressof(layers), nl, 1, _p(add), sync.data_ptr(), _chain_fault_word(dev).data_ptr(), n, d, h, w,
                                       vs_dtype(gy), EPS_IN, _stream()), "conv_k3_chain (backward)")
        out = [g_in if ctx.needs_input_grad[0] else None, None]
        for l in range(nl):
            wt, bias = weights[l], ctx.bias_refs[l]
            gw = gb = None
            if ctx.needs_input_grad[2 + 2 * l]:
                ax, axs = acts[l]
                gw, _ = _side_grads(wt, (applied[l], ax, axs), (applied[l], None, ax, axs, wt.shape[0], wt.shape[1], VS_CONV_K3), None, None)
            if bias is not None and ctx.needs_input_grad[3 + 2 * l]:
                gb = _dead_bias_grad(bias, bias.shape[0], dev)
            out += [gw, gb]
        return tuple(out)


class ConvK3Softmax(torch.autograd.Function):

    @staticmethod
    def forward(ctx, x, xs, weight, bias, drop_p=0.0, drop_seed=0):
        _require_cuda(x, weight)
        nc = weight.shape[0]
        if not 1 <= nc <= 8:
            raise NotImplementedError("out_block + softmax: n_class must be 1..8, got %d" % nc)
        n, d, h, w, c = x.shape
        wp = pack_weight_cached(weight, VS_PACK_ROWS_D0, c, k3_pack_dtype(x))
        prob = torch.empty((n, nc, d, h, w), dtype=torch.float32, device=x.device)
        ctx.fused2 = nc == 2 and c == 8
        if ctx.fused2:
            check(lib.vs_conv_k3_softmax2_dropout_fwd(x.data_ptr(), _p(xs), wp.data_ptr(), _p(bias), prob.data_ptr(), n, d, h, w, c,
                                                      vs_dtype(x), EPS_IN, float(drop_p), drop_seed, _stream()), "conv_k3_softmax2_fwd")
        else:
            bias8 = None if bias is None else torch.nn.functional.pad(bias.detach().float(), (0, 8 - nc))
            logits, _ = conv_gather(x, xs, wp, bias8, 8, VS_CONV_K3, False, real_channels=(weight.shape[1], nc))
            check(lib.vs_softmax_cl_fwd(logits.data_ptr(), prob.data_ptr(), n, d * h * w, 8, nc, vs_dtype(x), float(drop_p), drop_seed, _stream()),
                  "softmax_cl_fwd")
        ctx.save_for_backward(x, xs, weight, prob)
        ctx.has_bias = bias is not None
        ctx.bias_ref = bias
        ctx.drop = (float(drop_p), drop_seed)
        ctx.defer = bool(getattr(x, "_vs_defer_apply", False)) and xs is not None
        if ctx.needs_input_grad[2]:
            _count_use(weight)
        return prob

    @staticmethod
    def backward(ctx, gprob):
        x, xs, weight, prob = ctx.saved_tensors
        n, d, h, w, c = x.shape
        gprob = _contig(gprob.float())
        nc = weight.shape[0]
        if nc == 2 and x.dtype != torch.float32:
            fused = _out_block_bwd_fused(ctx, x, xs, weight, prob, gprob, None)
            if fused is not None:
                return fused
        gl = torch.empty((n, d, h, w, 8), dtype=x.dtype, device=x.device)
        if ctx.fused2:
            check(lib.vs_softmax2_dropout_bwd(prob.data_ptr(), gprob.data_ptr(), gl.data_ptr(), n, d * h * w, 8, vs_dtype(x),
                                              ctx.drop[0], ctx.drop[1], _stream()), "softmax2_bwd")
        else:
            check(lib.vs_softmax_cl_bwd(prob.data_ptr(), gprob.data_ptr(), gl.data_ptr(), n, d * h * w, 8, nc, vs_dtype(x),
                                        ctx.drop[0], ctx.drop[1], _stream()), "softmax_cl_bwd")
        gx = gw = gb = None
        if ctx.needs_input_grad[0]:
            wpb = pack_weight_cached(weight, VS_PACK_ROWS_D1_FLIP, 8, k3_pack_dtype(x))
            if xs is not None:
                gx = conv_bwd_data_lazy(gl, wpb, x, xs, VS_CONV_K3, real_channels=(nc, weight.shape[1]), defer=ctx.defer)
            else:
                gx, _ = conv_gather(gl, None, wpb, None, c, VS_CONV_K3, False)
        if ctx.needs_input_grad[2]:
            gw, gb = _side_grads(weight, (gl, x, xs), (gl, None, x, xs, nc, weight.shape[1], VS_CONV_K3),
                                 (gl, nc) if ctx.has_bias and ctx.needs_input_grad[3] else None, ctx.bias_ref)
        elif ctx.has_bias and ctx.needs_input_grad[3]:
            gb = bias_grad(gl, nc)
        return gx, None, gw, gb, None, None


class ConvK3SoftmaxCL(torch.autograd.Function):

    @staticmethod
    def forward(ctx, x, xs, weight, bias, drop_p=0.0, drop_seed=0):
        _require_cuda(x, weight)
        if weight.shape[0] != 2 or x.dtype == torch.float32:
            raise NotImplementedError("fused out_block+softmax with a channels-last copy: n_class == 2, 16-bit storage")
        n, d, h, w, c = x.shape
        wp = pack_weight_cached(weight, VS_PACK_ROWS_D0, c, k3_pack_dtype(x))
        prob = torch.empty((n, 2, d, h, w), dtype=torch.float32, device=x.device)
        prob_cl = torch.empty((n, d, h, w, 8), dtype=x.dtype, device=x.device)
        check(lib.vs_conv_k3_softmax2_cl_fwd(x.data_ptr(), _p(xs), wp.data_ptr(), _p(bias), prob.data_ptr(), prob_cl.data_ptr(), n, d, h, w, c,
                                             vs_dtype(x), EPS_IN, float(drop_p), drop_seed, _stream()), "conv_k3_softmax2_cl_fwd")
        ctx.save_for_backward(x, xs, weight, prob)
        ctx.has_bias = bias is not None
        ctx.bias_ref = bias
        ctx.drop = (float(drop_p), drop_seed)
        ctx.defer = bool(getattr(x, "_vs_defer_apply", False)) and xs is not None
        if ctx.needs_input_grad[2]:
            _count_use(weight)
        ctx.set_materialize_grads(False)
        return prob, prob_cl

    @staticmethod
    def backward(ctx, gprob, gcl):
        x, xs, weight, prob = ctx.saved_tensors
        if gprob is None and gcl is None:
            return None, None, None, None, None, None
        n, d, h, w, c = x.shape
        gprob = None if gprob is None else _contig(gprob.float())
        gcl = None if gcl is None else _contig(gcl)
        fused = _out_block_bwd_fused(ctx, x, xs, weight, prob, gprob, gcl)
        if fused is not None:
            return fused
        gl = torch.empty((n, d, h, w, 8), dtype=x.dtype, device=x.device)
        check(lib.vs_softmax2_cl_bwd(prob.data_ptr(), _p(gprob), _p(gcl), gl.data_ptr(), n, d * h * w, 8, vs_dtype(x), ctx.drop[0], ctx.drop[1],
                                     _stream()), "softmax2_cl_bwd")
        gx = gw = gb = None
        if ctx.needs_input_grad[0]:
            wpb = pack_weight_cached(weight, VS_PACK_ROWS_D1_FLIP, 8, k3_pack_dtype(x))
            if xs is not None:
                gx = conv_bwd_data_lazy(gl, wpb, x, xs, VS_CONV_K3, real_channels=(2, weight.shape[1]), defer=ctx.defer)
            else:
                gx, _ = conv_gather(gl, None, wpb, None, c, VS_CONV_K3, False)
        if ctx.needs_input_grad[2]:
            gw, gb = _side_grads(weight, (gl, x, xs), (gl, None, x, xs, 2, weight.shape[1], VS_CONV_K3),
                                 (gl, 2) if ctx.has_bias and ctx.needs_input_grad[3] else None, ctx.bias_ref)
        elif ctx.has_bias and ctx.needs_input_grad[3]:
            gb = bias_grad(gl, 2)
        return gx, None, gw, gb, None, None


FUSE_SOFTMAX_BWD = os.environ.get("VS_FUSE_SOFTMAX_BWD", "1") != "0"


def _out_block_bwd_fused(ctx, x, xs, weight, prob, gprob, gcl):
    n, d, h, w, c = x.shape
    want_w, want_b = ctx.needs_input_grad[2], ctx.has_bias and ctx.needs_input_grad[3]
    if not (FUSE_SOFTMAX_BWD and ctx.needs_input_grad[0] and xs is not None and c == 8 and (gcl is None or gcl.shape[-1] == 8)):
        return None
    if not lib.vs_conv_k3_bwd_data_wgrad_supported(n, d, h, w, 8, 8, vs_dtype(x)):
        return None
    if want_w:
        if not _wgrad_fusable(x, x, weight):
            return None
        bias = ctx.bias_ref
        if want_b and not (bias.is_leaf and bias.grad is None and not _has_hooks(bias)):
            return None
    elif want_b:
        return None
    wpb = pack_weight_cached(weight, VS_PACK_ROWS_D1_FLIP, 8, k3_pack_dtype(x))
    sums = _new_stats(n, c, x.device)
    g = torch.empty_like(x)
    nslabs = lib.vs_conv_k3_bwd_data_wgrad_slabs(n, d, h, w) if want_w else 0
    slabs = torch.empty(nslabs * 1728, dtype=torch.float32, device=x.device) if want_w else None
    bpart = torch.empty(nslabs * 2, dtype=torch.float64, device=x.device) if (want_w and want_b) else None
    kid = nb = fl = None
    if PROFILE is not None:
        kid = "k3tw_kernel<%s,2,%s>" % (_tname(x), "true" if want_w else "false")
        nb = (4 * n * d * h * w * 4) + (0 if gcl is None else gcl.numel() * _esize(x)) + 2 * g.numel() * _esize(x)
        fl = (2.0 if want_w else 1.0) * 2.0 * (g.numel() // c) * 27 * 2 * weight.shape[1]
    with _timed(kid, nb, fl, "out_block bwd%s (%d, %d, %d, %d)" % ("+wgrad" if want_w else "", n, d, h, w)):
        check(lib.vs_conv_k3_softmax2_bwd_data(prob.data_ptr(), _p(gprob), _p(gcl), wpb.data_ptr(), g.data_ptr(), x.data_ptr(), xs.data_ptr(), sums.data_ptr(),
                                               _p(slabs), _p(bpart), n, d, h, w, vs_dtype(x), EPS_IN, ctx.drop[0], ctx.drop[1], _stream()),
              "conv_k3_softmax2_bwd_data")
    gw = gb = None
    if want_w:
        if want_b:
            gw, gb = _group_submit_slabs(weight, slabs, nslabs, 2, weight.shape[1], (x,), bias=(ctx.bias_ref, bpart))
        else:
            gw = _group_submit_slabs(weight, slabs, nslabs, 2, weight.shape[1], (x,))
    if ctx.defer:
        _defer_register(g, x, xs, sums)
    else:
        _apply_in_place(g, x, xs, sums)
    return g, None, gw, gb, None, None


def out_block_softmax(x, xs, weight, bias, drop_p=0.0, drop_seed=0):
    if x.dtype != torch.float32 and weight.shape[0] == 2 and x.shape[-1] == 8 and os.environ.get("VS_SOFTMAX_CL", "1") != "0":
        prob, prob_cl = ConvK3SoftmaxCL.apply(x, xs, weight, bias, drop_p, drop_seed)
        prob._vs_cl = prob_cl
        return prob
    return ConvK3Softmax.apply(x, xs, weight, bias, drop_p, drop_seed)


def planar_input(x, dtype):
    cl = getattr(x, "_vs_cl", None)
    if cl is not None and cl.dtype == dtype and cl.shape[0] == x.shape[0] and tuple(cl.shape[1:4]) == tuple(x.shape[2:]):
        return cl
    return PackPlanar.apply(x, dtype)


class ConvK2S2(torch.autograd.Function):

    @staticmethod
    def forward(ctx, x, xs, weight, bias):
        _require_cuda(x, weight)
        wp = pack_weight_cached(weight, VS_PACK_ROWS_D0, x.shape[-1], x.dtype)
        y, _ = conv_gather(x, xs, wp, bias, cpad(weight.shape[0]), VS_CONV_K2S2, False)
        ctx.save_for_backward(x, xs, weight)
        ctx.has_bias = bias is not None
        ctx.bias_ref = bias
        ctx.defer = bool(getattr(x, "_vs_defer_apply", False)) and xs is not None
        return y

    @staticmethod
    def backward(ctx, gy):
        x, xs, weight = ctx.saved_tensors
        gy = _contig(gy)
        cout, cin = weight.shape[0], weight.shape[1]
        gx = gw = gb = None
        if ctx.needs_input_grad[0]:
            wpb = pack_weight_cached(weight, VS_PACK_SCATTER_D1, gy.shape[-1], gy.dtype)
            if xs is not None:
                gx = conv_bwd_data_lazy(gy, wpb, x, xs, VS_CONV_K2S2, scatter=True, defer=ctx.defer)
            else:
                gx = conv_scatter(gy, None, wpb, None, x.shape[-1])
        if ctx.needs_input_grad[2]:
            gw, gb = _side_grads(weight, (gy, x, xs), (gy, None, x, xs, cout, cin, VS_CONV_K2S2),
                                 (gy, cout) if ctx.has_bias and ctx.needs_input_grad[3] else None, ctx.bias_ref)
        elif ctx.has_bias and ctx.needs_input_grad[3]:
            gb = bias_grad(gy, cout)
        return gx, None, gw, gb


class ConvT2S2(torch.autograd.Function):

    @staticmethod
    def forward(ctx, x, xs, weight, bias):
        _require_cuda(x, weight)
        wp = pack_weight_cached(weight, VS_PACK_SCATTER_D1, x.shape[-1], x.dtype)
        y = conv_scatter(x, xs, wp, bias, cpad(weight.shape[1]))
        ctx.save_for_backward(x, xs, weight)
        ctx.has_bias = bias is not None
        ctx.bias_ref = bias
        ctx.defer = bool(getattr(x, "_vs_defer_apply", False)) and xs is not None
        return y

    @staticmethod
    def backward(ctx, gy):
        x, xs, weight = ctx.saved_tensors
        gy = _contig(gy)
        cin, cout = weight.shape[0], weight.shape[1]
        gx = gw = gb = None
        if ctx.needs_input_grad[0]:
            wpb = pack_weight_cached(weight, VS_PACK_ROWS_D0, gy.shape[-1], gy.dtype)
            if xs is not None:
# ... 644 lines not shown

def _pad_quads(x, b, c, value):
    voxels = x.numel() // (b * c)
    if voxels % 4 == 0:
        return x
    return torch.nn.functional.pad(x.reshape(b, c, voxels), (0, (-voxels) % 4), value=value)


def _unpad_quads(g, shape):
    if g is None or tuple(g.shape) == tuple(shape):
        return g
    voxels = 1
    for d in shape[2:]:
        voxels *= d
    return g[:, :, :voxels].reshape(shape)


class Dice(torch.autograd.Function):

    @staticmethod
    def forward(ctx, s, t, bot, top, eps, return_mean):
        _require_cuda(s, t)
        s, t = _contig(s.float()), _contig(t.float())
        b, c = s.shape[0], s.shape[1]
        ctx.shape = tuple(s.shape)
        s, t = _pad_quads(s, b, c, 0.0), _pad_quads(t, b, c, 0.0)
        voxels = s.numel() // (b * c)
        sums = torch.empty((b, c, 3), dtype=torch.float64, device=s.device)
        per = torch.empty(b, dtype=torch.float32, device=s.device)
        mean = torch.empty((), dtype=torch.float32, device=s.device)
        check(lib.vs_dice_fwd(s.data_ptr(), t.data_ptr(), sums.data_ptr(), per.data_ptr(), mean.data_ptr(), b, c, voxels,
                              bot, top, float(eps), _stream()), "dice_fwd")
        ctx.save_for_backward(s, t, sums)
        ctx.cfg = (bot, top, float(eps), bool(return_mean))
        return mean if return_mean else per

    @staticmethod
    def backward(ctx, g):
        s, t, sums = ctx.saved_tensors
        bot, top, eps, return_mean = ctx.cfg
        g = _contig(g.float())
        b, c = s.shape[0], s.shape[1]
        voxels = s.numel() // (b * c)
        gs = torch.empty_like(s) if ctx.needs_input_grad[0] else None
        gt = torch.empty_like(t) if ctx.needs_input_grad[1] else None
        if gs is not None or gt is not None:
            check(lib.vs_dice_bwd(s.data_ptr(), t.data_ptr(), sums.data_ptr(), g.data_ptr(), 1 if return_mean else 0,
                                  _p(gs), _p(gt), b, c, voxels, bot, top, eps, _stream()), "dice_bwd")
        return _unpad_quads(gs, ctx.shape), _unpad_quads(gt, ctx.shape), None, None, None, None


class LabelTarget:

    def __init__(self, label):
        _require_cuda(label)
        self.label = _contig(label.float())


class DiceLossSum(torch.autograd.Function):

    @staticmethod
    def forward(ctx, s, bot, top, eps, weights, *targets):
        is_lab = [isinstance(w, tuple) and bool(w[1]) for w in weights]
        weights = [w[0] if isinstance(w, tuple) else w for w in weights]
        _require_cuda(s, *targets)
        k = len(targets)
        s = _contig(s.float())
        ts = [_contig(t.float()) for t in targets]
        b, c = s.shape[0], s.shape[1]
        voxels = s.numel() // (b * c)
        for t, lab in zip(ts, is_lab):
            if lab and t.numel() != b * voxels:
                raise ValueError("label target: expected %d x %d labels, got %s" % (b, voxels, tuple(t.shape)))
        ctx.shapes = [tuple(s.shape)] + [tuple(t.shape) for t in ts]
        s = _pad_quads(s, b, c, 0.0)
        ts = [_pad_quads(t, b, 1, -1.0) if lab else _pad_quads(t, b, c, 0.0) for t, lab in zip(ts, is_lab)]
        voxels = s.numel() // (b * c)
        scratch = torch.empty(lib.vs_dice_loss_multi_scratch_doubles(k, b, c), dtype=torch.float64, device=s.device)
        terms = torch.empty(k, dtype=torch.float32, device=s.device)
        final = torch.empty((), dtype=torch.float32, device=s.device)
        tp = (_ctypes.c_void_p * k)(*[None if lab else t.data_ptr() for t, lab in zip(ts, is_lab)])
        lp = (_ctypes.c_void_p * k)(*[t.data_ptr() if lab else None for t, lab in zip(ts, is_lab)])
        wp = (_ctypes.c_float * k)(*[float(w) for w in weights])
        check(lib.vs_dice_loss_multi_labels_fwd(s.data_ptr(), _ctypes.addressof(tp), _ctypes.addressof(lp), _ctypes.addressof(wp), k, scratch.data_ptr(),
                                                terms.data_ptr(), final.data_ptr(), b, c, voxels, bot, top, float(eps), _stream()), "dice_loss_multi_fwd")
        ctx.save_for_backward(s, scratch, *ts)
        ctx.cfg = (bot, top, float(eps), [float(w) for w in weights], is_lab)
        ctx.mark_non_differentiable(terms)
        ctx.set_materialize_grads(False)
        return final, terms

    @staticmethod
    def backward(ctx, g, _gterms):
        s, scratch = ctx.saved_tensors[:2]
        ts = ctx.saved_tensors[2:]
        bot, top, eps, weights, is_lab = ctx.cfg
        if g is None:
            return (None,) * (5 + len(ts))
        k = len(ts)
        b, c = s.shape[0], s.shape[1]
        voxels = s.numel() // (b * c)
        g = _contig(g.float())
        gs = torch.empty_like(s) if ctx.needs_input_grad[0] else None
        gts = [torch.empty_like(t) if ctx.needs_input_grad[5 + j] and not is_lab[j] else None for j, t in enumerate(ts)]
        if gs is not None or any(x is not None for x in gts):
            tp = (_ctypes.c_void_p * k)(*[None if lab else t.data_ptr() for t, lab in zip(ts, is_lab)])
            lp = (_ctypes.c_void_p * k)(*[t.data_ptr() if lab else None for t, lab in zip(ts, is_lab)])
            gp = (_ctypes.c_void_p * k)(*[_p(x) for x in gts])
            wp = (_ctypes.c_float * k)(*weights)
            check(lib.vs_dice_loss_multi_labels_bwd(s.data_ptr(), _ctypes.addressof(tp), _ctypes.addressof(lp), _ctypes.addressof(wp), k, scratch.data_ptr(),
                                                    g.data_ptr(), _p(gs), _ctypes.addressof(gp), b, c, voxels, bot, top, eps, _stream()), "dice_loss_multi_bwd")
        return (_unpad_quads(gs, ctx.shapes[0]), None, None, None, None) + tuple(_unpad_quads(x, sh) for x, sh in zip(gts, ctx.shapes[1:]))


FUSED_LOSS = [os.environ.get("VS_FUSED_LOSS", "1") != "0"]


def dice_loss_sum(source, targets_and_weights, botindex=0, topindex=2, eps=1e-6):
    channels = source.shape[1]
    bot, top = (botindex, min(topindex, channels)) if channels > 1 else (0, 1)
    if not FUSED_LOSS[0] or len(targets_and_weights) > 4:
        targets_and_weights = [(onehot(t.label, channels) if isinstance(t, LabelTarget) else t, w) for t, w in targets_and_weights]
        terms = [1 - Dice.apply(source, t, bot, top, eps, True) for t, _ in targets_and_weights]
        final = None
        for term, (_, w) in zip(terms, targets_and_weights):
            part = term if w == 1 else w * term
            final = part if final is None else final + part
        return final, terms
    final, terms = DiceLossSum.apply(source, bot, top, eps, [(w, isinstance(t, LabelTarget)) for t, w in targets_and_weights],
                                     *[t.label if isinstance(t, LabelTarget) else t for t, _ in targets_and_weights])
    return final, list(terms.unbind(0))


class SegLoss(torch.autograd.Function):

    @staticmethod
    def forward(ctx, p, label, bot, top, eps, dice_weight, ce_weight, batch_dice, class_weights, gamma):
        _require_cuda(p, label)
        p, label = _contig(p.float()), _contig(label.float())
        b, c = p.shape[0], p.shape[1]
        voxels = p.numel() // (b * c)
        if label.numel() != b * voxels:
            raise ValueError("label target: expected %d x %d labels, got %s" % (b, voxels, tuple(label.shape)))
        ctx.shape = tuple(p.shape)
        p, label = _pad_quads(p, b, c, 0.0), _pad_quads(label, b, 1, -1.0)
        voxels = p.numel() // (b * c)
        scratch = torch.empty(max(1, lib.vs_seg_loss_scratch_doubles(b, c)), dtype=torch.float64, device=p.device)
        terms = torch.empty(2, dtype=torch.float32, device=p.device)
        final = torch.empty((), dtype=torch.float32, device=p.device)
        cfg = (b, c, voxels, int(bot), int(top), float(eps), float(dice_weight), float(ce_weight), 1 if batch_dice else 0, float(gamma))
        wp = (_ctypes.c_float * 8)(*([float(w) for w in class_weights] + [0.0] * 8)[:8])
        check(lib.vs_seg_loss_fwd(p.data_ptr(), label.data_ptr(), _ctypes.addressof(wp), scratch.data_ptr(), terms.data_ptr(), final.data_ptr(), *cfg,
                                  _stream()), "seg_loss_fwd")
        ctx.save_for_backward(p, label, scratch)
        ctx.cfg, ctx.class_weights = cfg, [float(w) for w in class_weights]
        ctx.mark_non_differentiable(terms)
        ctx.set_materialize_grads(False)
        return final, terms

    @staticmethod
    def backward(ctx, g, _gterms):
        p, label, scratch = ctx.saved_tensors
        gp = None
        if g is not None and ctx.needs_input_grad[0]:
            g = _contig(g.float())
            gp = torch.empty_like(p)
            wp = (_ctypes.c_float * 8)(*(ctx.class_weights + [0.0] * 8)[:8])
            check(lib.vs_seg_loss_bwd(p.data_ptr(), label.data_ptr(), _ctypes.addressof(wp), scratch.data_ptr(), g.data_ptr(), gp.data_ptr(), *ctx.cfg,
                                      _stream()), "seg_loss_bwd")
        return (_unpad_quads(gp, ctx.shape),) + (None,) * 9


def seg_loss(p, target, dice_weight=1.0, ce_weight=1.0, batch_dice=False, class_weights=None, gamma=0.0, botindex=0, topindex=2, eps=1e-6):
    if not isinstance(target, LabelTarget):
        raise TypeError("seg_loss takes its target as an ops.LabelTarget (a label volume); for a tensor target use dice_loss_sum")
    channels = p.shape[1]
    bot, top = (botindex, min(topindex, channels)) if channels > 1 else (0, 1)
    if class_weights is None:
        class_weights = [1.0] * channels
    class_weights = [float(w) for w in class_weights]
    if len(class_weights) != channels:
        raise ValueError("seg_loss: %d class weights for %d channels" % (len(class_weights), channels))
    final, terms = SegLoss.apply(p, target.label, bot, top, eps, dice_weight, ce_weight, bool(batch_dice), class_weights, gamma)
    return final, tuple(terms.unbind(0))


class BCE(torch.autograd.Function):

    @staticmethod
    def forward(ctx, p, t):
        _require_cuda(p, t)
        p, t = _contig(p.float()), _contig(t.float())
        out = torch.empty((), dtype=torch.float32, device=p.device)
        scratch = torch.empty(1, dtype=torch.float64, device=p.device)
        check(lib.vs_bce_fwd(p.data_ptr(), t.data_ptr(), out.data_ptr(), scratch.data_ptr(), p.numel(), _stream()), "bce_fwd")
        ctx.save_for_backward(p, t)
        return out

    @staticmethod
    def backward(ctx, g):
        p, t = ctx.saved_tensors
        gp = torch.empty_like(p)
        g = _contig(g.float())
# ... 37 lines not shown
```

### vae_segmentation_amd/train.py

```python
import os

import torch

from . import ops
from .evaluation import EPS_EVALUATION, EPS_MAIN_SOURCE, KLloss, avg_dsc, binarize, confident_binarize


LAZY_ONEHOT = os.environ.get("VS_LAZY_ONEHOT", "1") != "0"


def _gt(batch, label, n_class):
    if LAZY_ONEHOT and label.is_cuda:
        batch["label"] = label
        return ops.LabelTarget(label)
    batch["gt"] = ops.onehot(label, n_class)
    return batch["gt"]


def _seg_loss_args(loss):
    kw = dict(loss._asdict() if hasattr(loss, "_asdict") else loss)
    unknown = set(kw) - {"dice_weight", "ce_weight", "batch_dice", "class_weights", "gamma"}
    if unknown:
        raise TypeError("loss: unknown argument(s) %s" % ", ".join(sorted(unknown)))
    return kw


def joint_train_losses(joint, img, label, lambda_vae=0.1, eps=EPS_MAIN_SOURCE, n_class=2, loss=None):
    batch = {"img": img}
    if loss is not None:
        batch["label"] = label
        batch = joint(batch, "img", "pred", "recon")
        vae_part, (recon_loss,) = ops.dice_loss_sum(batch["pred"], [(batch["recon"], lambda_vae)], botindex=1, topindex=n_class, eps=eps)
        seg_part, (dsc_loss, ce_loss) = ops.seg_loss(batch["pred"], ops.LabelTarget(label), botindex=1, topindex=n_class, eps=eps, **_seg_loss_args(loss))
        return vae_part + seg_part, {"recon_loss": recon_loss, "dice_loss": dsc_loss, "ce_loss": ce_loss, "batch": batch}
    gt = _gt(batch, label, n_class)
    batch = joint(batch, "img", "pred", "recon")
    final, (recon_loss, dsc_loss) = ops.dice_loss_sum(batch["pred"], [(batch["recon"], lambda_vae), (gt, 1.0)],
                                                      botindex=1, topindex=n_class, eps=eps)
    return final, {"recon_loss": recon_loss, "dice_loss": dsc_loss, "batch": batch}


def seg_train_losses(seg, img, label, eps=EPS_MAIN_SOURCE, n_class=2, loss=None):
    batch = {"img": img}
    if loss is not None:
        batch["label"] = label
        batch = seg(batch, "img", "pred")
        final, (dsc_loss, ce_loss) = ops.seg_loss(batch["pred"], ops.LabelTarget(label), botindex=1, topindex=n_class, eps=eps, **_seg_loss_args(loss))
        return final, {"dice_loss": dsc_loss, "ce_loss": ce_loss, "batch": batch}
    gt = _gt(batch, label, n_class)
    batch = seg(batch, "img", "pred")
    final, (dsc_loss,) = ops.dice_loss_sum(batch["pred"], [(gt, 1.0)], botindex=1, topindex=n_class, eps=eps)
    return final, {"dice_loss": dsc_loss, "batch": batch}


def vae_train_losses(vae, label, scale=0.35, noise=None, eps=EPS_MAIN_SOURCE, n_class=2):
    gt = ops.onehot(label, n_class)
    recon, mean, std = vae(gt, if_random=True, scale=scale, noise=noise)
    batch = {"gt": gt, "recon": recon, "mean": mean, "std": std}
    kl = KLloss(batch)
    dsc_loss = 1 - avg_dsc(batch, "recon", "gt", botindex=1, topindex=n_class, eps=eps)
    final = dsc_loss + 0.00002 * kl
    return final, {"dice_loss": dsc_loss, "kl_loss": kl, "batch": batch}


def lambda_schedule(recon_loss, lambda_vae):
    r = float(recon_loss)
    if r < 0.15:
        return lambda_vae * 0.6
    if r < 0.225:
        return lambda_vae * 1.2
    if r < 0.3:
        return lambda_vae * 2.0
    return lambda_vae * 3.0


def domain_adaptation_losses(student, teacher, img, label, lambda_vae=1.0, domain_loss_type=0, kl=False,
                             use_confident_binarize=False, eps=EPS_EVALUATION, n_class=2, only_pseudo=False, epoch=0,
                             turn_epoch=-1, lambda_vae_warmup=0, host_schedule=True):
    batch = {"img": img, "gt": ops.onehot(label, n_class)}
    batch = student(batch, "img", "pred", "recon", dropout=True)
    with torch.no_grad():
        batch = teacher(batch, "img", "fake", "_unused")
    batch["fake"] = confident_binarize(batch["fake"]) if use_confident_binarize else binarize(batch["fake"])
    recon_loss = 1 - avg_dsc(batch, "pred", "recon", botindex=1, topindex=n_class, eps=eps)
    klloss = KLloss(batch)
    dsc_loss = 1 - avg_dsc(batch, "pred", "gt", botindex=1, topindex=n_class, eps=eps)
    fake_loss = 1 - avg_dsc(batch, "pred", "fake", botindex=1, topindex=n_class, eps=eps)
    if only_pseudo:
        final = fake_loss
    elif domain_loss_type in (8, 15, 16, 9) and not host_schedule:
        final = finetune_loss(recon_loss, fake_loss, klloss, lambda_vae, 9 if domain_loss_type == 9 else 8, kl, False)
    elif domain_loss_type in (8, 15, 16):
        cur = lambda_schedule(recon_loss.detach(), lambda_vae)
        if cur > 1:
            final = recon_loss + (klloss if kl else 0) + 1 / cur * fake_loss
        else:
            final = cur * (recon_loss + (klloss if kl else 0)) + fake_loss
    elif domain_loss_type == 9:
        cur = lambda_schedule(recon_loss.detach(), lambda_vae)
        final = (cur * recon_loss + fake_loss) / (1 + cur)
    elif domain_loss_type == 11:
        final = lambda_vae * recon_loss + fake_loss + recon_loss * fake_loss
    elif domain_loss_type == 12:
        final = lambda_vae * recon_loss + fake_loss - recon_loss * fake_loss
    elif domain_loss_type == 13:
        recon_loss = torch.clamp(recon_loss - 0.15, min=0)
        final = lambda_vae * recon_loss
    elif domain_loss_type == 14:
        recon_loss = torch.clamp(recon_loss - 0.1, min=0)
        final = lambda_vae * recon_loss + fake_loss
    elif domain_loss_type == 10:
        raise NotImplementedError("domain_loss_type 10 reads `val_batch`, undefined in the reference's training loop (main_target.py:568)")
    elif turn_epoch != -1:
        final = lambda_vae * recon_loss if (epoch // turn_epoch) % 2 == 0 else lambda_vae * recon_loss + fake_loss
    elif epoch >= lambda_vae_warmup:
        final = lambda_vae * recon_loss + fake_loss
        if kl:
            final = final + 0.00002 * lambda_vae * klloss
# ... 393 lines not shown
```

Before: 892.5 volumes/s.

## Fuse Dice loss sums and gradients into the softmax out-block conv kernels

Adds a Dice-fusion descriptor so the final 3x3x3 conv with two-class softmax epilogue accumulates the per-sample Dice partial sums (intersection, source and target sums) as it writes probabilities. A small finish kernel then reduces the per-workgroup slots into the loss terms. In backward, the softmax-backward data/wgrad kernel computes the Dice gradient inline instead of materialising a dense gradient tensor. This removes separate full-volume Dice forward and backward passes and their memory traffic, at the cost of a complex announce/descriptor protocol in Python and extra registers and loads in the conv epilogue.

```diff
diff --git a/include/vaeseg.h b/include/vaeseg.h
--- a/include/vaeseg.h
+++ b/include/vaeseg.h
@@ -107,6 +107,7 @@
     int k3_short_tiles;
     int wgrad_bias_fold;
     int hist_form;
+    int fuse_dice;
     long long wgrad_wgs;
     long long wgrad_f32_tiles;
     long long wgrad_group_wgs;
@@ -362,6 +363,29 @@
 int vs_dice_loss_multi_labels_bwd(const float* s, const float* const* t, const float* const* labels, const float* w, int k,
                                   const double* scratch, const float* gout, float* gs, float* const* gt, int batch, int channels,
                                   long long voxels, int bot, int top, float eps, void* stream);
+typedef struct vs_dice_fuse {
+    const float* tensor;
+    const float* label;
+    const double* sums;
+    double* part;
+    const float* gout;
+    float w[2];
+    float eps;
+    int k;
+    int kind[2];
+    int source;
+    int cls;
+} vs_dice_fuse;
+int vs_dice_fuse_slots(int n, int d, int h, int w);
+size_t vs_dice_fuse_scratch_doubles(int k, int batch, int channels, int slots);
+int vs_conv_k3_softmax2_cl_dice_fwd(const void* x, const double* x_stats, const void* w_packed, const float* bias, float* prob, void* prob_cl,
+                                    const vs_dice_fuse* dice, int n, int d, int h, int w, int c_in, int dtype, float eps, float drop_p,
+                                    unsigned long long drop_seed, void* stream);
+int vs_dice_loss_multi_finish(const float* w, int k, double* scratch, float* terms, float* final_out, int batch, int channels, int bot, int top,
+                              int slots, float eps, void* stream);
+int vs_conv_k3_softmax2_dice_bwd_data(const float* prob, const vs_dice_fuse* dice, const void* gprob_cl, const void* w_packed, void* y, const void* mask_x,
+                                      const double* mask_stats, double* sums, float* slabs, double* bias_part, int n, int d, int h, int w, int dtype,
+                                      float eps, float drop_p, unsigned long long drop_seed, void* stream);
 size_t vs_seg_loss_scratch_doubles(int batch, int channels);
 int vs_seg_loss_fwd(const float* p, const float* label, const float* class_w, double* scratch, float* terms, float* final_out, int batch, int channels,
                     long long voxels, int bot, int top, float eps, float dice_w, float ce_w, int batch_dice, float gamma, void* stream);
diff --git a/vae_segmentation_amd/csrc/common.h b/vae_segmentation_amd/csrc/common.h
--- a/vae_segmentation_amd/csrc/common.h
+++ b/vae_segmentation_amd/csrc/common.h
@@ -298,6 +298,31 @@
     return out;
 }
 
+__device__ __forceinline__ float vs_dice_g(float gout, int batch, int classes, float w) {
+#pragma clang fp contract(off)
+    const float g0 = -gout / ((float)batch * (float)classes);
+    return g0 * w;
+}
+__device__ __forceinline__ void vs_dice_coef(const double* __restrict__ q, float g, float eps, float& k1, float& k2) {
+#pragma clang fp contract(off)
+    const float I = (float)q[0], den = (float)q[1] + (float)q[2] + eps;
+    k1 = g * 2.f / den;
+    k2 = g * 2.f * I / (den * den);
+}
+template <int KMAX>
+__device__ __forceinline__ float vs_dice_grad_source(const float (&k1)[KMAX], float k2sum, const float (&y)[KMAX], int K) {
+#pragma clang fp contract(off)
+    float acc = -k2sum;
+#pragma unroll
+    for (int j = 0; j < KMAX; ++j)
+        if (j < K) acc = __builtin_fmaf(k1[j], y[j], acc);
+    return acc;
+}
+__device__ __forceinline__ float vs_dice_grad_target(float k1, float k2, float x) {
+#pragma clang fp contract(off)
+    return __builtin_fmaf(k1, x, -k2);
+}
+
 template <typename T> struct H16;
 template <> struct H16<unsigned short> {
     __device__ static __forceinline__ unsigned int pack2(f32x2 v) { return __builtin_bit_cast(unsigned int, __builtin_convertvector(v, bf16x2)); }
diff --git a/vae_segmentation_amd/csrc/config.hip b/vae_segmentation_amd/csrc/config.hip
--- a/vae_segmentation_amd/csrc/config.hip
+++ b/vae_segmentation_amd/csrc/config.hip
@@ -36,6 +36,7 @@
     c->k3_short_tiles = env_int("VS_K3_SHORT_TILES", 2);
     c->wgrad_bias_fold = env_int("VS_WGRAD_BIAS_FOLD", 1);
     c->hist_form = env_int("VS_HIST_FORM", 0);
+    c->fuse_dice = env_int("VS_FUSE_DICE", 1);
     c->wgrad_wgs = env_ll("VS_WGRAD_WGS", 512);
     c->wgrad_f32_tiles = env_ll("VS_WGRAD_F32_TILES", 8);
     c->wgrad_group_wgs = env_ll("VS_WGRAD_GROUP_WGS", 0);
diff --git a/vae_segmentation_amd/csrc/conv_api.hip b/vae_segmentation_amd/csrc/conv_api.hip
--- a/vae_segmentation_amd/csrc/conv_api.hip
+++ b/vae_segmentation_amd/csrc/conv_api.hip
@@ -326,6 +326,66 @@
     return vs_conv_k3_softmax2_cl_fwd(x, x_stats, w_packed, bias, prob, nullptr, n, d, h, w, c_in, dtype, eps, drop_p, drop_seed, stream);
 }
 
+static int dice_fuse_check(const vs_dice_fuse* dc, int dtype) {
+    if (!dc || dc->k < 1 || dc->k > 2 || (unsigned)dc->cls > 1u || (unsigned)dc->source > 1u) return VS_EINVAL;
+    if (dtype == VS_F32) return VS_EDTYPE;
+    bool own = dc->source == 0;
+    if (dc->source == 1 && !dc->tensor) return VS_EINVAL;
+    for (int j = 0; j < dc->k; ++j) {
+        if ((unsigned)dc->kind[j] > 2u || dc->kind[j] == dc->source) return VS_EINVAL;
+        if ((dc->kind[j] == 1 && !dc->tensor) || (dc->kind[j] == 2 && !dc->label)) return VS_EINVAL;
+        own = own || dc->kind[j] == 0;
+    }
+    if (!own) return VS_EINVAL;
+    if (((uintptr_t)dc->tensor & 3) || ((uintptr_t)dc->label & 3)) return VS_EALIGN;
+    return VS_OK;
+}
+
+extern "C" int vs_dice_fuse_slots(int n, int d, int h, int w) {
+    if (n <= 0 || d <= 0 || h <= 0 || w <= 0) return 0;
+    return k3tw_slab_count(n, d, h, w);
+}
+
+extern "C" int vs_conv_k3_softmax2_cl_dice_fwd(const void* x, const double* x_stats, const void* w_packed, const float* bias, float* prob, void* prob_cl,
+                                               const vs_dice_fuse* dice, int n, int d, int h, int w, int c_in, int dtype, float eps, float drop_p,
+                                               unsigned long long drop_seed, void* stream) {
+    if (drop_p < 0.f || drop_p >= 1.f) return VS_EINVAL;
+    int rc = dice_fuse_check(dice, dtype);
+    if (rc) return rc;
+    if (!dice->part || ((uintptr_t)dice->part & 7) || n > 32) return VS_EINVAL;
+    if (prob_cl && ((uintptr_t)prob_cl & 15)) return VS_EALIGN;
+    rc = check_common(x, w_packed, n, d, h, w, c_in, dtype);
+    if (rc) return rc;
+    if (!prob || c_in != 8) return VS_ESHAPE;
+    const ConvPlan pl = plan_gather({n, d, h, w, 8, 8, VS_CONV_K3, dtype, 0});
+    if (pl.status) return pl.status;
+    G1Params p = pl.g;
+    p.x = x; p.x_stats = x_stats; p.wp = w_packed; p.bias = bias; p.y = prob_cl; p.prob = prob; p.eps = eps;
+    p.drop_p = drop_p; p.drop_seed = drop_seed;
+    p.dice = *dice;
+    return dispatch_k3(p, dtype, pl.t, EPI_SOFTMAX2, (int)pl.tiles, (hipStream_t)stream);
+}
+
+extern "C" int vs_conv_k3_softmax2_dice_bwd_data(const float* prob, const vs_dice_fuse* dice, const void* gprob_cl, const void* w_packed, void* y, const void* mask_x,
+                                                 const double* mask_stats, double* sums, float* slabs, double* bias_part, int n, int d, int h, int w, int dtype,
+                                                 float eps, float drop_p, unsigned long long drop_seed, void* stream) {
+    if (!prob || !w_packed || !y || !mask_x || !mask_stats || !sums) return VS_EINVAL;
+    if (bias_part && !slabs) return VS_EINVAL;
+    int rc = dice_fuse_check(dice, dtype);
+    if (rc) return rc;
+    if (!dice->sums || !dice->gout || ((uintptr_t)dice->sums & 7) || ((uintptr_t)dice->gout & 3)) return VS_EINVAL;
+    const ConvPlan pl = plan_wgrad(n, d, h, w, 8, 8, false, dtype);
+    if (pl.status) return VS_ESHAPE;
+    if (((uintptr_t)w_packed & 15) || ((uintptr_t)y & 15) || ((uintptr_t)mask_x & 15) || (gprob_cl && ((uintptr_t)gprob_cl & 15)) || (slabs && ((uintptr_t)slabs & 15)) ||
+        ((uintptr_t)prob & 3)) return VS_EALIGN;
+    if (!(drop_p >= 0.f && drop_p < 1.f)) return VS_EINVAL;
+    G1Params p = bwd_params(pl, nullptr, w_packed, y, mask_x, mask_stats, sums, eps);
+    p.sm_prob = prob; p.sm_gcl = gprob_cl; p.wg_ws = slabs; p.wg_bias = bias_part;
+    p.drop_p = drop_p; p.drop_seed = drop_seed;
+    p.dice = *dice;
+    return dispatch_k3(p, dtype, pl.t, EPI_RAW, 0, (hipStream_t)stream);
+}
+
 extern "C" int vs_conv_k3_softmax2_cl_fwd(const void* x, const double* x_stats, const void* w_packed, const float* bias, float* prob, void* prob_cl,
                                           int n, int d, int h, int w, int c_in, int dtype, float eps, float drop_p, unsigned long long drop_seed, void* stream) {
     if (drop_p < 0.f || drop_p >= 1.f) return VS_EINVAL;
diff --git a/vae_segmentation_amd/csrc/igemm.h b/vae_segmentation_amd/csrc/igemm.h
--- a/vae_segmentation_amd/csrc/igemm.h
+++ b/vae_segmentation_amd/csrc/igemm.h
@@ -4,7 +4,7 @@
 #include "handoff.h"
 
 enum { G1_K3 = 0, G1_K2S2 = 1, G1_PW = 2 };
-enum { EPI_RAW = 0, EPI_SOFTMAX2 = 1, EPI_SCATTER = 2 };
+enum { EPI_RAW = 0, EPI_SOFTMAX2 = 1, EPI_SCATTER = 2, EPI_SOFTMAX2_DICE = 3 };
 
 struct G1Params {
     const void* x;
@@ -46,6 +46,7 @@
     unsigned int* ea_fault;
     int ea_items;
     const void* ea_add;
+    vs_dice_fuse dice;
 };
 
 #define G1_LDS_MEAN 0
diff --git a/vae_segmentation_amd/csrc/igemm_k3t.h b/vae_segmentation_amd/csrc/igemm_k3t.h
--- a/vae_segmentation_amd/csrc/igemm_k3t.h
+++ b/vae_segmentation_amd/csrc/igemm_k3t.h
@@ -26,6 +26,7 @@
     float* s_mkr = s_mkm + p.N * 8;
     float* s_fa = s_mkr + p.N * 8;
     static_assert(!FA || (!HS && EPI == EPI_RAW), "fused apply: backward-data use (materialised gradient in), with or without the fused IN-backward sums");
+    constexpr bool DICE = EPI == EPI_SOFTMAX2_DICE, SMX = EPI == EPI_SOFTMAX2 || DICE;
 
     const int tid = threadIdx.x, lane = tid & 63, wave = tid >> 6, col = lane & 15, g = lane >> 4;
     const int dx2 = g >> 1, c4 = 4 * (g & 1);
@@ -138,7 +139,7 @@
     if (t < t_end) load_x(cur);
     float bv[4];
 #pragma unroll
-    for (int r = 0; r < 4; ++r) bv[r] = (p.bias != nullptr && c4 + r < (EPI == EPI_SOFTMAX2 ? 2 : p.M)) ? p.bias[c4 + r] : 0.f;
+    for (int r = 0; r < 4; ++r) bv[r] = (p.bias != nullptr && c4 + r < ((EPI == EPI_SOFTMAX2 || EPI == EPI_SOFTMAX2_DICE) ? 2 : p.M)) ? p.bias[c4 + r] : 0.f;
     const i32x4 yrsrc = make_rsrc(p.y, (unsigned int)((long long)p.N * p.D * p.H * p.W * 16));
     const i32x4 mrsrc = make_rsrc(p.mask_x, (unsigned int)((long long)p.N * p.D * p.H * p.W * 16));
     for (int i = tid; i < st_n; i += 256) {
@@ -162,6 +163,11 @@
     }
     const char* s_b = s_tile + ((wave * PY) * PX + 2 * col + g) * 16;
     float ssum[4] = {0.f, 0.f, 0.f, 0.f}, ssq[4] = {0.f, 0.f, 0.f, 0.f};
+    double dsum[5] = {0.0, 0.0, 0.0, 0.0, 0.0};
+    unsigned int dseen = 0;
+    const int dvol = p.D * p.H * p.W;
+    const i32x4 dtrsrc = make_rsrc(DICE ? (const void*)p.dice.tensor : p.x, (unsigned int)((DICE && p.dice.tensor != nullptr) ? (long long)p.N * dvol * 8 : 0));
+    const i32x4 dlrsrc = make_rsrc(DICE ? (const void*)p.dice.label : p.x, (unsigned int)((DICE && p.dice.label != nullptr) ? (long long)p.N * dvol * 4 : 0));
 #pragma unroll
     for (int r = 0; r < 4; ++r) asm volatile("" : "+v"(bv[r]));
 #pragma unroll
@@ -188,6 +194,16 @@
             for (int cg = 0; cg < YT; ++cg)
                 mk[cg] = __builtin_bit_cast(u32x2, vs_raw_buffer_load_b64(mrsrc, (zx_ok && y0 + cg < p.H) ? ebase + cg * p.W * 16 : -1, 0, 0));
         }
+        float dpt[DICE ? YT : 1], dlb[DICE ? YT : 1];
+        if constexpr (DICE) {
+#pragma unroll
+            for (int cg = 0; cg < YT; ++cg) {
+                const bool mine = zx_ok && y0 + cg < p.H && (g & 1) == 0;
+                const int v = (oz * p.H + y0 + cg) * p.W + ox;
+                dpt[cg] = __int_as_float(vs_raw_buffer_load_b32(dtrsrc, mine ? ((n * 2 + p.dice.cls) * dvol + v) * 4 : -1, 0, 0));
+                dlb[cg] = __int_as_float(vs_raw_buffer_load_b32(dlrsrc, mine ? (n * dvol + v) * 4 : -1, 0, 0));
+            }
+        }
         nxt = tile_coord<YT, 32>(p, t + G < t_end ? t + G : t);
         if (t + G < t_end) load_x(nxt);
         K3_TICK(4);
@@ -208,7 +224,7 @@
         }
 
         K3_TICK(5);
-        if constexpr (EPI == EPI_SOFTMAX2) {
+        if constexpr (SMX) {
             const size_t V = (size_t)p.D * p.H * p.W;
 #pragma unroll
             for (int cg = 0; cg < YT; ++cg) {
@@ -227,6 +243,22 @@
                     p.prob[((size_t)n * 2 + 0) * V + v] = e0 * inv;
                     p.prob[((size_t)n * 2 + 1) * V + v] = e1 * inv;
                 }
+                if constexpr (DICE) {
+                    if (valid && (g & 1) == 0) {
+                        const float own = p.dice.cls ? e1 * inv : e0 * inv;
+                        const float pt = dpt[cg], lb = (int)dlb[cg] == p.dice.cls ? 1.f : 0.f;
+                        const double sv = (double)(p.dice.source == 0 ? own : pt);
+                        dsum[0] += sv;
+#pragma unroll
+                        for (int j = 0; j < 2; ++j) {
+                            if (j < p.dice.k) {
+                                const double yv = (double)(p.dice.kind[j] == 0 ? own : (p.dice.kind[j] == 1 ? pt : lb));
+                                dsum[1 + 2 * j] += sv * yv;
+                                dsum[2 + 2 * j] += yv;
+                            }
+                        }
+                    }
+                }
                 if (p.y != nullptr) {
                     f32x2 pr;
                     pr[0] = e0 * inv; pr[1] = e1 * inv;
@@ -234,6 +266,23 @@
                     pk[0] = (g & 1) == 0 ? (int)H16<T>::pack2(pr) : 0;
                     pk[1] = 0;
                     vs_raw_buffer_store_b64(pk, yrsrc, valid ? ebase + cg * p.W * 16 : -1, 0, 0);
+                }
+            }
+            if constexpr (DICE) {
+                const bool flush = t + G >= t_end || nxt.n != n;
+                if (flush) {
+                    double* s_redd = (double*)(smem + K3T_LDS_RED);
+#pragma unroll
+                    for (int q = 0; q < 5; ++q) {
+                        const double tot = wave_sum_d(dsum[q]);
+                        if (lane == 0) s_redd[wave * 5 + q] = tot;
+                        dsum[q] = 0.0;
+                    }
+                    __syncthreads();
+                    const int NQ = 1 + 2 * p.dice.k;
+                    if (tid < NQ)
+                        p.dice.part[((size_t)n * NQ + tid) * gridDim.x + blockIdx.x] = ((s_redd[tid] + s_redd[5 + tid]) + s_redd[10 + tid]) + s_redd[15 + tid];
+                    dseen |= 1u << n;
                 }
             }
         } else {
@@ -303,6 +352,11 @@
         cur = nxt;
         K3_TICK(6);
     }
+    if constexpr (DICE) {
+        const int NQ = 1 + 2 * p.dice.k;
+        for (int i = tid; i < p.N * NQ; i += 256)
+            if (!((dseen >> (i / NQ)) & 1u)) p.dice.part[(size_t)i * gridDim.x + blockIdx.x] = 0.0;
+    }
     K3_TICK_FLUSH;
 }
 
@@ -322,6 +376,9 @@
     tile_fastdiv_fill(p);
     if (SUMS != (p.sums != nullptr) || (SUMS && !FA && p.x_stats != nullptr)) return VS_EINVAL;
     if (FA && (!p.x_stats || !p.fa_x || !p.fa_sums)) return VS_EINVAL;
+    constexpr bool DICE = EPI == EPI_SOFTMAX2_DICE;
+    if (DICE != (p.dice.k > 0)) return VS_EINVAL;
+    if (DICE && (!p.dice.part || p.dice.k > 2 || (unsigned)p.dice.cls > 1u || p.N > 32)) return VS_EINVAL;
     auto kern = k3t_kernel<EPI, SUMS, YT, HS, T, FA>;
     static const hipError_t attr_err =
         hipFuncSetAttribute((const void*)kern, hipFuncAttributeMaxDynamicSharedMemorySize, 160 * 1024);
@@ -339,6 +396,9 @@
     if constexpr (EPI == EPI_RAW) {
         if (p.fa_x != nullptr) return k3t_launch_t<T, EPI, SUMS, YT, false, true>(p, stream);
     }
+    if constexpr (EPI == EPI_SOFTMAX2) {
+        if (p.dice.k > 0) return p.x_stats != nullptr ? k3t_launch_t<T, EPI_SOFTMAX2_DICE, SUMS, YT, true>(p, stream) : k3t_launch_t<T, EPI_SOFTMAX2_DICE, SUMS, YT, false>(p, stream);
+    }
     if (!SUMS && p.x_stats != nullptr) return k3t_launch_t<T, EPI, SUMS, YT, !SUMS>(p, stream);
     return k3t_launch_t<T, EPI, SUMS, YT, false>(p, stream);
 }
diff --git a/vae_segmentation_amd/csrc/igemm_k3tw.h b/vae_segmentation_amd/csrc/igemm_k3tw.h
--- a/vae_segmentation_amd/csrc/igemm_k3tw.h
+++ b/vae_segmentation_amd/csrc/igemm_k3tw.h
@@ -20,7 +20,7 @@
 template <typename T, int MODE, bool WG>
 __global__ __launch_bounds__(256) __attribute__((amdgpu_waves_per_eu(2, 2))) void k3tw_kernel(const G1Params p) {
     constexpr int YT = 8;
-    constexpr bool FA = MODE == 1, SM = MODE == 2;
+    constexpr bool FA = MODE == 1, SM = MODE == 2 || MODE == 3, DG = MODE == 3;
     static_assert(WG || SM, "without the weight gradient this is k3t_kernel, except for the softmax-backward staging");
     using GEO = K3TGeom<YT>;
     constexpr int PX = GEO::PX, PY = GEO::PY, PLANE = GEO::PLANE, TV = GEO::TV, NIT = GEO::NIT;
@@ -34,6 +34,7 @@
     float* s_mkm = s_shift + p.N * 8;
     float* s_mkr = s_mkm + p.N * 8;
     float* s_fa = s_mkr + p.N * 8;
+    float* s_dg = s_fa + 4 * p.N * 8;
 
     const int tid = threadIdx.x, lane = tid & 63, wave = tid >> 6, col = lane & 15, g = lane >> 4;
     const int dx2 = g >> 1, c4 = 4 * (g & 1);
@@ -41,7 +42,9 @@
     const long long vol = (long long)p.D * p.H * p.W;
     const i32x4 xrsrc = make_rsrc(SM ? (const void*)p.sm_prob : p.x, (unsigned int)(SM ? p.N * vol * 8 : p.N * vol * 16));
     const i32x4 frsrc = make_rsrc(FA ? p.fa_x : (SM ? p.sm_gcl : p.x), (unsigned int)((FA || (SM && p.sm_gcl != nullptr)) ? p.N * vol * 16 : 0));
-    const i32x4 grsrc = make_rsrc(SM ? (const void*)p.sm_gprob : p.x, (unsigned int)((SM && p.sm_gprob != nullptr) ? p.N * vol * 8 : 0));
+    const i32x4 grsrc = make_rsrc(DG ? (const void*)p.dice.tensor : (SM ? (const void*)p.sm_gprob : p.x),
+                                  (unsigned int)((DG ? p.dice.tensor != nullptr : (SM && p.sm_gprob != nullptr)) ? p.N * vol * 8 : 0));
+    const i32x4 lrsrc = make_rsrc(DG ? (const void*)p.dice.label : p.x, (unsigned int)((DG && p.dice.label != nullptr) ? p.N * vol * 4 : 0));
 
     const double* st_src = p.mask_stats;
     const int st_n = p.N * 8;
@@ -88,8 +91,13 @@
                 const int o0 = ok ? ((c.n * 2) * (int)vol + vi) * 4 : -1, o1 = ok ? ((c.n * 2 + 1) * (int)vol + vi) * 4 : -1;
                 xv[b][0] = (unsigned int)vs_raw_buffer_load_b32(xrsrc, o0, 0, 0);
                 xv[b][1] = (unsigned int)vs_raw_buffer_load_b32(xrsrc, o1, 0, 0);
-                xv[b][2] = (unsigned int)vs_raw_buffer_load_b32(grsrc, o0, 0, 0);
-                xv[b][3] = (unsigned int)vs_raw_buffer_load_b32(grsrc, o1, 0, 0);
+                if constexpr (DG) {
+                    xv[b][2] = (unsigned int)vs_raw_buffer_load_b32(grsrc, p.dice.cls ? o1 : o0, 0, 0);
+                    xv[b][3] = (unsigned int)vs_raw_buffer_load_b32(lrsrc, ok ? (c.n * (int)vol + vi) * 4 : -1, 0, 0);
+                } else {
+                    xv[b][2] = (unsigned int)vs_raw_buffer_load_b32(grsrc, o0, 0, 0);
+                    xv[b][3] = (unsigned int)vs_raw_buffer_load_b32(grsrc, o1, 0, 0);
+                }
                 fv[b] = __builtin_bit_cast(u32x4, vs_raw_buffer_load_b128(frsrc, ok ? base + rel_off[b] : -1, 0, 0));
             } else {
                 xv[b] = __builtin_bit_cast(u32x4, vs_raw_buffer_load_b128(xrsrc, ok ? base + rel_off[b] : -1, 0, 0));
@@ -99,10 +107,27 @@
     };
     auto write_x_sm = [&](const TileCoord& c) {
         const int base = (((c.n * p.D + c.z0 - 1) * p.H + c.y0 - 1) * p.W + c.x0 - 1) * 16;
+        float dk1[2] = {0.f, 0.f}, dk2 = 0.f;
+        if constexpr (DG) { dk1[0] = s_dg[c.n * 4 + 0]; dk1[1] = s_dg[c.n * 4 + 1]; dk2 = s_dg[c.n * 4 + 2]; }
 #pragma unroll
         for (int b = 0; b < NIT; ++b) {
             const float p0 = __uint_as_float(xv[b][0]), p1 = __uint_as_float(xv[b][1]);
-            const float g0 = __uint_as_float(xv[b][2]) + H16<T>::lo(fv[b][0]), g1 = __uint_as_float(xv[b][3]) + H16<T>::hi(fv[b][0]);
+            float gp0 = __uint_as_float(xv[b][2]), gp1 = __uint_as_float(xv[b][3]);
+            if constexpr (DG) {
+                const float pt = gp0, lab = gp1;
+                float gd;
+                if (p.dice.source == 0) {
+                    float y[2];
+#pragma unroll
+                    for (int j = 0; j < 2; ++j) y[j] = p.dice.kind[j] == 1 ? pt : (p.dice.kind[j] == 2 ? ((int)lab == p.dice.cls ? 1.f : 0.f) : 0.f);
+                    gd = vs_dice_grad_source<2>(dk1, dk2, y, p.dice.k);
+                } else {
+                    gd = vs_dice_grad_target(dk1[0], dk2, pt);
+                }
+                gp0 = p.dice.cls == 0 ? gd : 0.f;
+                gp1 = p.dice.cls == 0 ? 0.f : gd;
+            }
+            const float g0 = gp0 + H16<T>::lo(fv[b][0]), g1 = gp1 + H16<T>::hi(fv[b][0]);
             const float dot = p0 * g0 + p1 * g1;
             f32x2 f;
             f[0] = p0 * (g0 - dot);
@@ -181,6 +206,25 @@
             s_fa[1 * p.N * 8 + i] = -m * r;
             s_fa[2 * p.N * 8 + i] = (float)(fa_pre[1][0] * p.inv_count_in);
             s_fa[3 * p.N * 8 + i] = (float)(fa_pre[1][1] * p.inv_count_in);
+        }
+    }
+    if constexpr (DG) {
+        if (tid >= 128 && tid < 128 + p.N) {
+            const int b = tid - 128;
+            const float gout = p.dice.gout[0];
+            float k1[2] = {0.f, 0.f}, k2[2] = {0.f, 0.f}, k2sum = 0.f;
+#pragma unroll
+            for (int j = 0; j < 2; ++j) {
+                if (j < p.dice.k) {
+                    vs_dice_coef(p.dice.sums + (((size_t)j * p.N + b) * 2 + p.dice.cls) * 3, vs_dice_g(gout, p.N, 1, p.dice.w[j]), p.dice.eps, k1[j], k2[j]);
+                    k2sum += k2[j];
+                }
+            }
+            const int jo = (p.dice.k > 1 && p.dice.kind[1] == 0) ? 1 : 0;
+            const bool src = p.dice.source == 0;
+            s_dg[b * 4 + 0] = src ? k1[0] : (jo ? k1[1] : k1[0]);
+            s_dg[b * 4 + 1] = src ? k1[1] : 0.f;
+            s_dg[b * 4 + 2] = src ? k2sum : (jo ? k2[1] : k2[0]);
         }
     }
     const char* s_b = s_tile + ((wave * PY) * PX + 2 * col + g) * 16;
@@ -261,7 +305,7 @@
                 for (int r = 0; r < 4; ++r) {
                     const float xh = (xv4[r] - mm[r]) * mr[r];
                     const float gm = xh > 0.f ? v[r] : 0.f;
-                    ssum[r] += gm; ssq[r] += gm * xh;
+                    ssum[r] += gm; ssq[r] = __builtin_fmaf(gm, xh, ssq[r]);
                     qv[r] = valid ? fmaxf(fmaf(xv4[r], mr[r], -mm[r] * mr[r]), 0.f) : 0.f;
                 }
                 if constexpr (WG) {
@@ -379,11 +423,12 @@
     G1Params p = p_in;
     if (p.C != 8 || p.M != 8 || p.N * 8 > 192) return VS_ESHAPE;
     if (!p.sums || !p.mask_x || !p.mask_stats) return VS_EINVAL;
-    const bool fa = p.fa_x != nullptr, sm = p.sm_prob != nullptr, wg = p.wg_ws != nullptr;
+    const bool fa = p.fa_x != nullptr, sm = p.sm_prob != nullptr, wg = p.wg_ws != nullptr, dg = p.dice.k > 0;
     if (fa && (sm || !p.x_stats || !p.fa_sums)) return VS_EINVAL;
-    if (sm ? (!p.sm_gprob && !p.sm_gcl) : (!wg || !p.x)) return VS_EINVAL;
+    if (sm ? (!p.sm_gprob && !p.sm_gcl && !dg) : (!wg || !p.x || dg)) return VS_EINVAL;
+    if (dg && (p.sm_gprob || !p.dice.sums || !p.dice.gout || p.dice.k > 2 || (unsigned)p.dice.cls > 1u)) return VS_EINVAL;
     if ((long long)p.N * p.D * p.H * p.W * 8 >= 2147483648ll) return VS_ESHAPE;
-    const size_t lds = K3T_LDS_TILE + (size_t)GEO::TILE_BYTES + K3TW_Q_BYTES + K3TW_ACC_BYTES + (size_t)8 * p.N * 8 * sizeof(float);
+    const size_t lds = K3T_LDS_TILE + (size_t)GEO::TILE_BYTES + K3TW_Q_BYTES + K3TW_ACC_BYTES + (size_t)8 * p.N * 8 * sizeof(float) + (size_t)4 * p.N * sizeof(float);
     p.txn = (p.W + 31) / 32;
     p.tyn = (p.H + 7) / 8;
     p.tiles_per_sample = ((p.D + 3) / 4) * p.tyn * p.txn;
@@ -398,7 +443,8 @@
         if (attr_err != hipSuccess) return (int)attr_err;                                                                                \
         hipLaunchKernelGGL(kern, dim3(gx), dim3(256), lds, stream, p);                                                                   \
     }
-    if (sm) { if (wg) K3TW_GO(2, true) else K3TW_GO(2, false) }
+    if (sm && dg) { if (wg) K3TW_GO(3, true) else K3TW_GO(3, false) }
+    else if (sm) { if (wg) K3TW_GO(2, true) else K3TW_GO(2, false) }
     else if (fa) K3TW_GO(1, true)
     else K3TW_GO(0, true)
 #undef K3TW_GO
diff --git a/vae_segmentation_amd/csrc/misc.hip b/vae_segmentation_amd/csrc/misc.hip
--- a/vae_segmentation_amd/csrc/misc.hip
+++ b/vae_segmentation_amd/csrc/misc.hip
@@ -816,13 +816,13 @@
     const long long v4 = voxels / 4;
     for (long long i = (long long)blockIdx.x * 256 + threadIdx.x; i < v4; i += (long long)gridDim.x * 256) {
         const f32x4 x = *(const f32x4*)(sp + i * 4);
-        aS += (double)(x[0] + x[1]) + (double)(x[2] + x[3]);
+        aS += ((double)x[0] + (double)x[1]) + ((double)x[2] + (double)x[3]);
 #pragma unroll
         for (int j = 0; j < DICE_MULTI_MAX; ++j) {
             if (j < K) {
                 const f32x4 y = dice_target4(a, j, plane, b, c, voxels, i);
-                aI[j] += (double)(x[0] * y[0] + x[1] * y[1]) + (double)(x[2] * y[2] + x[3] * y[3]);
-                aT[j] += (double)(y[0] + y[1]) + (double)(y[2] + y[3]);
+                aI[j] += ((double)x[0] * (double)y[0] + (double)x[1] * (double)y[1]) + ((double)x[2] * (double)y[2] + (double)x[3] * (double)y[3]);
+                aT[j] += ((double)y[0] + (double)y[1]) + ((double)y[2] + (double)y[3]);
             }
         }
     }
@@ -959,6 +959,25 @@
     return VS_OK;
 }
 
+extern "C" size_t vs_dice_fuse_scratch_doubles(int k, int batch, int channels, int slots) {
+    if (k <= 0 || batch <= 0 || channels <= 0 || slots <= 0) return 0;
+    return (size_t)3 * k * batch * channels + (size_t)batch * channels * (1 + 2 * k) * slots;
+}
+
+extern "C" int vs_dice_loss_multi_finish(const float* w, int k, double* scratch, float* terms, float* final_out, int batch, int channels, int bot, int top,
+                                         int slots, float eps, void* stream) {
+    if (!w || !scratch || !terms || !final_out || k <= 0 || k > DICE_MULTI_MAX || batch <= 0 || batch > 64 || channels <= 0 || bot < 0 || top > channels ||
+        bot >= top || slots <= 0) return VS_EINVAL;
+    if ((long long)batch * (top - bot) > 128) return VS_ESHAPE;
+    DiceMulti a = DiceMulti{};
+    a.k = k;
+    for (int j = 0; j < k; ++j) a.w[j] = w[j];
+    hipLaunchKernelGGL(dice_multi_finish_kernel, dim3(1), dim3(256), 0, (hipStream_t)stream, a, scratch + (size_t)3 * k * batch * channels, scratch, terms,
+                       final_out, batch, channels, bot, top, slots, eps);
+    VS_CHECK_LAUNCH();
+    return VS_OK;
+}
+
 __global__ __launch_bounds__(256) void dice_multi_bwd_kernel(const DiceMulti a, const double* __restrict__ sums, const float* __restrict__ gout,
                                                             float* __restrict__ gs, int batch, int channels, long long voxels, int bot,
                                                             int top, float eps) {
@@ -976,33 +995,35 @@
         return;
     }
     float k1[DICE_MULTI_MAX], k2[DICE_MULTI_MAX], k2sum = 0.f;
-    const float g0 = -gout[0] / ((float)batch * (float)(top - bot));
 #pragma unroll
     for (int j = 0; j < DICE_MULTI_MAX; ++j) {
         k1[j] = 0.f; k2[j] = 0.f;
         if (j < K) {
-            const double* q = sums + (((size_t)j * batch + b) * channels + c) * 3;
-            const float I = (float)q[0], den = (float)q[1] + (float)q[2] + eps;
-            const float g = g0 * a.w[j];
-            k1[j] = g * 2.f / den;
-            k2[j] = g * 2.f * I / (den * den);
+            vs_dice_coef(sums + (((size_t)j * batch + b) * channels + c) * 3, vs_dice_g(gout[0], batch, top - bot, a.w[j]), eps, k1[j], k2[j]);
             k2sum += k2[j];
         }
     }
     for (long long i = (long long)blockIdx.x * 256 + threadIdx.x; i < v4; i += (long long)gridDim.x * 256) {
         const f32x4 x = *(const f32x4*)(a.s + plane + i * 4);
-        f32x4 acc = f32x4{-k2sum, -k2sum, -k2sum, -k2sum};
-#pragma unroll
-        for (int j = 0; j < DICE_MULTI_MAX; ++j) {
-            if (j < K) {
-                if (gs) {
-                    const f32x4 y = dice_target4(a, j, plane, b, c, voxels, i);
-                    acc[0] += k1[j] * y[0]; acc[1] += k1[j] * y[1]; acc[2] += k1[j] * y[2]; acc[3] += k1[j] * y[3];
-                }
-                if (a.gt[j]) *(f32x4*)(a.gt[j] + plane + i * 4) = f32x4{k1[j] * x[0] - k2[j], k1[j] * x[1] - k2[j], k1[j] * x[2] - k2[j], k1[j] * x[3] - k2[j]};
+        if (gs) {
+            f32x4 y[DICE_MULTI_MAX];
+#pragma unroll
+            for (int j = 0; j < DICE_MULTI_MAX; ++j) y[j] = j < K ? dice_target4(a, j, plane, b, c, voxels, i) : f32x4{0.f, 0.f, 0.f, 0.f};
+            f32x4 acc;
+#pragma unroll
+            for (int e = 0; e < 4; ++e) {
+                float ye[DICE_MULTI_MAX];
+#pragma unroll
+                for (int j = 0; j < DICE_MULTI_MAX; ++j) ye[j] = y[j][e];
+                acc[e] = vs_dice_grad_source<DICE_MULTI_MAX>(k1, k2sum, ye, K);
             }
-        }
-        if (gs) *(f32x4*)(gs + plane + i * 4) = acc;
+            *(f32x4*)(gs + plane + i * 4) = acc;
+        }
+#pragma unroll
+        for (int j = 0; j < DICE_MULTI_MAX; ++j)
+            if (j < K && a.gt[j])
+                *(f32x4*)(a.gt[j] + plane + i * 4) = f32x4{vs_dice_grad_target(k1[j], k2[j], x[0]), vs_dice_grad_target(k1[j], k2[j], x[1]),
+                                                           vs_dice_grad_target(k1[j], k2[j], x[2]), vs_dice_grad_target(k1[j], k2[j], x[3])};
     }
 }
 
diff --git a/vae_segmentation_amd/ops.py b/vae_segmentation_amd/ops.py
--- a/vae_segmentation_amd/ops.py
+++ b/vae_segmentation_amd/ops.py
@@ -46,7 +46,7 @@
 class VsConfig(_ctypes.Structure):
     _fields_ = [(n, _ctypes.c_int) for n in ("k3_small", "k3_tall", "k3_wgs_per_cu", "k3t_wgs_per_cu", "k3f_min_wgs", "mt_min_wgs", "f32_limbs", "g1_limbs", "k3x_ck",
                                             "k3x_toeplitz", "fuse_wgrad", "epilogue_apply", "chain", "k2s2_stream", "k2s8_wgs_per_cu", "up_wgs_per_cu", "up_rb",
-                                            "wgrad_uber", "wgrad_mpack", "wgrad_swap", "wgrad_big", "wgrad_xcd", "k3_short_tiles", "wgrad_bias_fold", "hist_form")] + \
+                                            "wgrad_uber", "wgrad_mpack", "wgrad_swap", "wgrad_big", "wgrad_xcd", "k3_short_tiles", "wgrad_bias_fold", "hist_form", "fuse_dice")] + \
                [(n, _ctypes.c_longlong) for n in ("wgrad_wgs", "wgrad_f32_tiles", "wgrad_group_wgs", "wgrad_big_min_voxels")]
 
 
@@ -1106,7 +1106,12 @@
         wp = pack_weight_cached(weight, VS_PACK_ROWS_D0, c, k3_pack_dtype(x))
         prob = torch.empty((n, nc, d, h, w), dtype=torch.float32, device=x.device)
         ctx.fused2 = nc == 2 and c == 8
-        if ctx.fused2:
+        dice = _dice_forward_hook(x, weight, n, d, h, w, drop_p, ctx.fused2)
+        if dice is not None:
+            with _timed("k3t_kernel<3,false,8,%s,%s>" % ("true" if xs is not None else "false", _tname(x)), 0, 0, "out_block + Dice sums (%d, %d, %d, %d)" % (n, d, h, w)):
+                check(lib.vs_conv_k3_softmax2_cl_dice_fwd(x.data_ptr(), _p(xs), wp.data_ptr(), _p(bias), prob.data_ptr(), None, _ctypes.addressof(dice), n, d, h, w, c,
+                                                          vs_dtype(x), EPS_IN, 0.0, 0, _stream()), "conv_k3_softmax2_dice_fwd")
+        elif ctx.fused2:
             check(lib.vs_conv_k3_softmax2_dropout_fwd(x.data_ptr(), _p(xs), wp.data_ptr(), _p(bias), prob.data_ptr(), n, d, h, w, c,
                                                       vs_dtype(x), EPS_IN, float(drop_p), drop_seed, _stream()), "conv_k3_softmax2_fwd")
         else:
@@ -1121,18 +1126,26 @@
         ctx.defer = bool(getattr(x, "_vs_defer_apply", False)) and xs is not None
         if ctx.needs_input_grad[2]:
             _count_use(weight)
+        _dice_forward_done(prob, dice is not None)
+        ctx.set_materialize_grads(False)
         return prob
 
     @staticmethod
     def backward(ctx, gprob):
         x, xs, weight, prob = ctx.saved_tensors
         n, d, h, w, c = x.shape
-        gprob = _contig(gprob.float())
+        gprob = None if gprob is None else _contig(gprob.float())
         nc = weight.shape[0]
+        gprob, dice = _dice_take(prob, gprob)
+        if gprob is None and dice is None:
+            return None, None, None, None, None, None
         if nc == 2 and x.dtype != torch.float32:
-            fused = _out_block_bwd_fused(ctx, x, xs, weight, prob, gprob, None)
+            fused = _out_block_bwd_fused(ctx, x, xs, weight, prob, gprob, None, dice)
             if fused is not None:
                 return fused
+        if dice is not None:
+            gd = _dice_dense_for(prob, dice[1])
+            gprob = gd if gprob is None else gprob + gd
         gl = torch.empty((n, d, h, w, 8), dtype=x.dtype, device=x.device)
         if ctx.fused2:
             check(lib.vs_softmax2_dropout_bwd(prob.data_ptr(), gprob.data_ptr(), gl.data_ptr(), n, d * h * w, 8, vs_dtype(x),
@@ -1166,8 +1179,15 @@
         wp = pack_weight_cached(weight, VS_PACK_ROWS_D0, c, k3_pack_dtype(x))
         prob = torch.empty((n, 2, d, h, w), dtype=torch.float32, device=x.device)
         prob_cl = torch.empty((n, d, h, w, 8), dtype=x.dtype, device=x.device)
-        check(lib.vs_conv_k3_softmax2_cl_fwd(x.data_ptr(), _p(xs), wp.data_ptr(), _p(bias), prob.data_ptr(), prob_cl.data_ptr(), n, d, h, w, c,
-                                             vs_dtype(x), EPS_IN, float(drop_p), drop_seed, _stream()), "conv_k3_softmax2_cl_fwd")
+        dice = _dice_forward_hook(x, weight, n, d, h, w, drop_p, c == 8)
+        if dice is not None:
+            with _timed("k3t_kernel<3,false,8,%s,%s>" % ("true" if xs is not None else "false", _tname(x)), 0, 0, "out_block + Dice sums (%d, %d, %d, %d)" % (n, d, h, w)):
+                check(lib.vs_conv_k3_softmax2_cl_dice_fwd(x.data_ptr(), _p(xs), wp.data_ptr(), _p(bias), prob.data_ptr(), prob_cl.data_ptr(), _ctypes.addressof(dice),
+                                                          n, d, h, w, c, vs_dtype(x), EPS_IN, 0.0, 0, _stream()), "conv_k3_softmax2_cl_dice_fwd")
+        else:
+            check(lib.vs_conv_k3_softmax2_cl_fwd(x.data_ptr(), _p(xs), wp.data_ptr(), _p(bias), prob.data_ptr(), prob_cl.data_ptr(), n, d, h, w, c,
+                                                 vs_dtype(x), EPS_IN, float(drop_p), drop_seed, _stream()), "conv_k3_softmax2_cl_fwd")
+        _dice_forward_done(prob, dice is not None)
         ctx.save_for_backward(x, xs, weight, prob)
         ctx.has_bias = bias is not None
         ctx.bias_ref = bias
@@ -1181,14 +1201,18 @@
     @staticmethod
     def backward(ctx, gprob, gcl):
         x, xs, weight, prob = ctx.saved_tensors
-        if gprob is None and gcl is None:
+        gprob = None if gprob is None else _contig(gprob.float())
+        gprob, dice = _dice_take(prob, gprob)
+        if gprob is None and gcl is None and dice is None:
             return None, None, None, None, None, None
         n, d, h, w, c = x.shape
-        gprob = None if gprob is None else _contig(gprob.float())
         gcl = None if gcl is None else _contig(gcl)
-        fused = _out_block_bwd_fused(ctx, x, xs, weight, prob, gprob, gcl)
+        fused = _out_block_bwd_fused(ctx, x, xs, weight, prob, gprob, gcl, dice)
         if fused is not None:
             return fused
+        if dice is not None:
+            gd = _dice_dense_for(prob, dice[1])
+            gprob = gd if gprob is None else gprob + gd
         gl = torch.empty((n, d, h, w, 8), dtype=x.dtype, device=x.device)
         check(lib.vs_softmax2_cl_bwd(prob.data_ptr(), _p(gprob), _p(gcl), gl.data_ptr(), n, d * h * w, 8, vs_dtype(x), ctx.drop[0], ctx.drop[1],
                                      _stream()), "softmax2_cl_bwd")
@@ -1210,7 +1234,7 @@
 FUSE_SOFTMAX_BWD = os.environ.get("VS_FUSE_SOFTMAX_BWD", "1") != "0"
 
 
-def _out_block_bwd_fused(ctx, x, xs, weight, prob, gprob, gcl):
+def _out_block_bwd_fused(ctx, x, xs, weight, prob, gprob, gcl, dice=None):
     n, d, h, w, c = x.shape
     want_w, want_b = ctx.needs_input_grad[2], ctx.has_bias and ctx.needs_input_grad[3]
     if not (FUSE_SOFTMAX_BWD and ctx.needs_input_grad[0] and xs is not None and c == 8 and (gcl is None or gcl.shape[-1] == 8)):
@@ -1233,13 +1257,18 @@
     bpart = torch.empty(nslabs * 2, dtype=torch.float64, device=x.device) if (want_w and want_b) else None
     kid = nb = fl = None
     if PROFILE is not None:
-        kid = "k3tw_kernel<%s,2,%s>" % (_tname(x), "true" if want_w else "false")
+        kid = "k3tw_kernel<%s,%d,%s>" % (_tname(x), 2 if dice is None else 3, "true" if want_w else "false")
         nb = (4 * n * d * h * w * 4) + (0 if gcl is None else gcl.numel() * _esize(x)) + 2 * g.numel() * _esize(x)
         fl = (2.0 if want_w else 1.0) * 2.0 * (g.numel() // c) * 27 * 2 * weight.shape[1]
     with _timed(kid, nb, fl, "out_block bwd%s (%d, %d, %d, %d)" % ("+wgrad" if want_w else "", n, d, h, w)):
-        check(lib.vs_conv_k3_softmax2_bwd_data(prob.data_ptr(), _p(gprob), _p(gcl), wpb.data_ptr(), g.data_ptr(), x.data_ptr(), xs.data_ptr(), sums.data_ptr(),
-                                               _p(slabs), _p(bpart), n, d, h, w, vs_dtype(x), EPS_IN, ctx.drop[0], ctx.drop[1], _stream()),
-              "conv_k3_softmax2_bwd_data")
+        if dice is not None:
+            check(lib.vs_conv_k3_softmax2_dice_bwd_data(prob.data_ptr(), _ctypes.addressof(dice[0]), _p(gcl), wpb.data_ptr(), g.data_ptr(), x.data_ptr(), xs.data_ptr(),
+                                                        sums.data_ptr(), _p(slabs), _p(bpart), n, d, h, w, vs_dtype(x), EPS_IN, ctx.drop[0], ctx.drop[1], _stream()),
+                  "conv_k3_softmax2_dice_bwd_data")
+        else:
+            check(lib.vs_conv_k3_softmax2_bwd_data(prob.data_ptr(), _p(gprob), _p(gcl), wpb.data_ptr(), g.data_ptr(), x.data_ptr(), xs.data_ptr(), sums.data_ptr(),
+                                                   _p(slabs), _p(bpart), n, d, h, w, vs_dtype(x), EPS_IN, ctx.drop[0], ctx.drop[1], _stream()),
+                  "conv_k3_softmax2_bwd_data")
     gw = gb = None
     if want_w:
         if want_b:
@@ -2050,8 +2079,9 @@
         tp = (_ctypes.c_void_p * k)(*[None if lab else t.data_ptr() for t, lab in zip(ts, is_lab)])
         lp = (_ctypes.c_void_p * k)(*[t.data_ptr() if lab else None for t, lab in zip(ts, is_lab)])
         wp = (_ctypes.c_float * k)(*[float(w) for w in weights])
-        check(lib.vs_dice_loss_multi_labels_fwd(s.data_ptr(), _ctypes.addressof(tp), _ctypes.addressof(lp), _ctypes.addressof(wp), k, scratch.data_ptr(),
-                                                terms.data_ptr(), final.data_ptr(), b, c, voxels, bot, top, float(eps), _stream()), "dice_loss_multi_fwd")
+        with _timed("dice_multi_partial_kernel+dice_multi_finish_kernel", (1 + k) * s.numel() * 4, 0, "%d terms %s" % (k, tuple(s.shape))):
+            check(lib.vs_dice_loss_multi_labels_fwd(s.data_ptr(), _ctypes.addressof(tp), _ctypes.addressof(lp), _ctypes.addressof(wp), k, scratch.data_ptr(),
+                                                    terms.data_ptr(), final.data_ptr(), b, c, voxels, bot, top, float(eps), _stream()), "dice_loss_multi_fwd")
         ctx.save_for_backward(s, scratch, *ts)
         ctx.cfg = (bot, top, float(eps), [float(w) for w in weights], is_lab)
         ctx.mark_non_differentiable(terms)
@@ -2065,28 +2095,203 @@
         bot, top, eps, weights, is_lab = ctx.cfg
         if g is None:
             return (None,) * (5 + len(ts))
-        k = len(ts)
-        b, c = s.shape[0], s.shape[1]
-        voxels = s.numel() // (b * c)
-        g = _contig(g.float())
-        gs = torch.empty_like(s) if ctx.needs_input_grad[0] else None
-        gts = [torch.empty_like(t) if ctx.needs_input_grad[5 + j] and not is_lab[j] else None for j, t in enumerate(ts)]
-        if gs is not None or any(x is not None for x in gts):
-            tp = (_ctypes.c_void_p * k)(*[None if lab else t.data_ptr() for t, lab in zip(ts, is_lab)])
-            lp = (_ctypes.c_void_p * k)(*[t.data_ptr() if lab else None for t, lab in zip(ts, is_lab)])
-            gp = (_ctypes.c_void_p * k)(*[_p(x) for x in gts])
-            wp = (_ctypes.c_float * k)(*weights)
+        gs, gts = _dice_dense_bwd(s, ts, is_lab, weights, scratch, _contig(g.float()), bot, top, eps, ctx.needs_input_grad[0],
+                                  [ctx.needs_input_grad[5 + j] for j in range(len(ts))])
+        return (_unpad_quads(gs, ctx.shapes[0]), None, None, None, None) + tuple(_unpad_quads(x, sh) for x, sh in zip(gts, ctx.shapes[1:]))
+
+
+FUSED_LOSS = [os.environ.get("VS_FUSED_LOSS", "1") != "0"]
+
+
+NEXT_OUTPUT = object()
+_DICE = {"ann": None, "tables": {}, "callback": False}
+
+
+class VsDiceFuse(_ctypes.Structure):
+    _fields_ = [("tensor", _ctypes.c_void_p), ("label", _ctypes.c_void_p), ("sums", _ctypes.c_void_p), ("part", _ctypes.c_void_p), ("gout", _ctypes.c_void_p),
+                ("w", _ctypes.c_float * 2), ("eps", _ctypes.c_float), ("k", _ctypes.c_int), ("kind", _ctypes.c_int * 2), ("source", _ctypes.c_int),
+                ("cls", _ctypes.c_int)]
+
+
+class dice_announce:
+
+    def __init__(self, terms, botindex=0, topindex=2, eps=1e-6):
+        self.terms = list(terms)
+        self.bot, self.top, self.eps = int(botindex), min(int(topindex), 2), float(eps)
+        own = [j for j, (t, _) in enumerate(self.terms) if t is NEXT_OUTPUT]
+        labs = [j for j, (t, _) in enumerate(self.terms) if isinstance(t, LabelTarget)]
+        if len(own) != 1 or len(own) + len(labs) != len(self.terms) or len(self.terms) > 2:
+            raise ValueError("dice_announce: one ops.NEXT_OUTPUT term and at most one ops.LabelTarget term")
+        self.own = own[0]
+        self.label = self.terms[labs[0]][0] if labs else None
+        self.state = "open"
+        self.source = self.carrier = self.scratch = None
+        self.slots = 0
+        if not (FUSED_LOSS[0] and get_config()["fuse_dice"] and self.top - self.bot == 1):
+            self.state = "declined"
+
+    def __enter__(self):
+        if _DICE["ann"] is not None:
+            raise RuntimeError("dice_announce: another announcement is still open")
+        _DICE["ann"] = self
+        return self
+
+    def __exit__(self, etype, *exc):
+        _DICE["ann"] = None
+        if etype is None and self.state not in ("consumed", "declined"):
+            raise RuntimeError("dice_announce: the announced Dice terms were not consumed by a dice_loss_sum call (state: %s)" % self.state)
+        return False
+
+    def descriptor(self, own_is, other, **kw):
+        d = VsDiceFuse()
+        d.tensor, d.label = _p(other), _p(None if self.label is None else self.label.label)
+        d.k, d.eps, d.cls = len(self.terms), self.eps, self.bot
+        d.source = 0 if own_is == "source" else 1
+        for j, (t, w) in enumerate(self.terms):
+            d.w[j] = float(w)
+            d.kind[j] = 2 if isinstance(t, LabelTarget) else (1 if own_is == "source" else 0)
+        for k, v in kw.items():
+            setattr(d, k, v)
+        return d
+
+
+def _dice_forward_hook(x, weight, n, d, h, w, drop_p, fused2):
+    ann = _DICE["ann"]
+    if ann is None or ann.state not in ("open", "source"):
+        return None
+    ok = fused2 and x.dtype != torch.float32 and not drop_p and n <= 32 and (ann.label is None or ann.label.label.numel() == n * d * h * w)
+    if ok and ann.state == "source":
+        ok = tuple(ann.source.shape) == (n, 2, d, h, w)
+    if not ok:
+        ann.state = "declined"
+        return None
+    if ann.state == "open":
+        return None
+    ann.slots = lib.vs_dice_fuse_slots(n, d, h, w)
+    ann.scratch = torch.empty(lib.vs_dice_fuse_scratch_doubles(len(ann.terms), n, 2, ann.slots), dtype=torch.float64, device=x.device)
+    return ann.descriptor("target", ann.source, part=ann.scratch.data_ptr() + 8 * 3 * len(ann.terms) * n * 2)
+
+
+def _dice_forward_done(prob, carried):
+    ann = _DICE["ann"]
+    if ann is None or ann.state not in ("open", "source"):
+        return
+    if ann.state == "open":
+        ann.source, ann.state = prob, "source"
+    elif carried:
+        ann.carrier, ann.state = prob, "carried"
+
+
+def _dice_table_put(prob, desc, keep):
+    _DICE["tables"][(prob.data_ptr(), tuple(prob.shape))] = (desc, keep, prob)
+    _on_backward_end(_DICE, _dice_tables_done)
+
+
+def _dice_take(prob, gprob):
+    ent = _DICE["tables"].pop((prob.data_ptr(), tuple(prob.shape)), None) if _DICE["tables"] else None
+    if ent is None:
+        return gprob, None
+    if gprob is not None:
+        return gprob + _dice_dense_for(prob, ent[1]), None
+    return None, ent[:2]
+
+
+def _dice_tables_done():
+    _DICE["callback"] = False
+    left = len(_DICE["tables"])
+    _DICE["tables"].clear()
+    if left:
+        raise RuntimeError("%d Dice gradient descriptor(s) were not taken by the out_block that produced their probabilities: gradients lost" % left)
+
+
+def _dice_dense_bwd(s, ts, is_lab, weights, scratch, g, bot, top, eps, want_s, want_t):
+    k = len(ts)
+    b, c = s.shape[0], s.shape[1]
+    voxels = s.numel() // (b * c)
+    gs = torch.empty_like(s) if want_s else None
+    gts = [torch.empty_like(t) if want_t[j] and not is_lab[j] else None for j, t in enumerate(ts)]
+    if gs is not None or any(x is not None for x in gts):
+        tp = (_ctypes.c_void_p * k)(*[None if lab else t.data_ptr() for t, lab in zip(ts, is_lab)])
+        lp = (_ctypes.c_void_p * k)(*[t.data_ptr() if lab else None for t, lab in zip(ts, is_lab)])
+        gp = (_ctypes.c_void_p * k)(*[_p(x) for x in gts])
+        wp = (_ctypes.c_float * k)(*weights)
+        with _timed("dice_multi_bwd_kernel", (1 + k + sum(x is not None for x in [gs] + gts)) * s.numel() * 4, 0, "%d terms %s" % (k, tuple(s.shape))):
             check(lib.vs_dice_loss_multi_labels_bwd(s.data_ptr(), _ctypes.addressof(tp), _ctypes.addressof(lp), _ctypes.addressof(wp), k, scratch.data_ptr(),
                                                     g.data_ptr(), _p(gs), _ctypes.addressof(gp), b, c, voxels, bot, top, eps, _stream()), "dice_loss_multi_bwd")
-        return (_unpad_quads(gs, ctx.shapes[0]), None, None, None, None) + tuple(_unpad_quads(x, sh) for x, sh in zip(gts, ctx.shapes[1:]))
-
-
-FUSED_LOSS = [os.environ.get("VS_FUSED_LOSS", "1") != "0"]
+    return gs, gts
+
+
+def _wants_dense_grad(t):
+    return _has_hooks(t) or bool(getattr(t, "retains_grad", False))
+
+
+class DiceLossSumFused(torch.autograd.Function):
+
+    @staticmethod
+    def forward(ctx, s, t, ann):
+        k, n = len(ann.terms), s.shape[0]
+        terms = torch.empty(k, dtype=torch.float32, device=s.device)
+        final = torch.empty((), dtype=torch.float32, device=s.device)
+        wp = (_ctypes.c_float * k)(*[float(w) for _, w in ann.terms])
+        with _timed("dice_multi_finish_kernel", ann.scratch.numel() * 8, 0, "%d terms, %d slots" % (k, ann.slots)):
+            check(lib.vs_dice_loss_multi_finish(_ctypes.addressof(wp), k, ann.scratch.data_ptr(), terms.data_ptr(), final.data_ptr(), n, 2, ann.bot, ann.top, ann.slots,
+                                                ann.eps, _stream()), "dice_loss_multi_finish")
+        ctx.save_for_backward(s, t)
+        ctx.ann = ann
+        ctx.dense = (_wants_dense_grad(s), _wants_dense_grad(t))
+        ctx.mark_non_differentiable(terms)
+        ctx.set_materialize_grads(False)
+        return final, terms
+
+    @staticmethod
+    def backward(ctx, g, _gterms):
+        s, t = ctx.saved_tensors
+        ann = ctx.ann
+        if g is None:
+            return None, None, None
+        g = _contig(g.float())
+        out = [None, None]
+        for i, (own, other, role) in enumerate(((s, t, "source"), (t, s, "target"))):
+            if not ctx.needs_input_grad[i]:
+                continue
+            lab = None if ann.label is None else ann.label.label
+            desc = ann.descriptor(role, other, sums=ann.scratch.data_ptr(), gout=g.data_ptr())
+            keep = (other, lab, ann.scratch, g, (ann, s, t, i))
+            if ctx.dense[i]:
+                out[i] = _dice_dense_for(own, keep)
+            else:
+                _dice_table_put(own, desc, keep)
+        return out[0], out[1], None
+
+
+def _dice_dense_for(prob, keep):
+    ann, s, t, i = keep[4]
+    g = keep[3]
+    b = s.shape[0]
+    is_lab = [isinstance(x, LabelTarget) for x, _ in ann.terms]
+    ts = [_pad_quads(x.label, b, 1, -1.0) if lab else _pad_quads(t, b, 2, 0.0) for (x, _), lab in zip(ann.terms, is_lab)]
+    gs, gts = _dice_dense_bwd(_pad_quads(s, b, 2, 0.0), ts, is_lab, [float(w) for _, w in ann.terms], ann.scratch, g, ann.bot, ann.top, ann.eps,
+                              i == 0, [i == 1 and j == ann.own for j in range(len(ts))])
+    return _unpad_quads(gs if i == 0 else gts[ann.own], tuple(prob.shape))
 
 
 def dice_loss_sum(source, targets_and_weights, botindex=0, topindex=2, eps=1e-6):
     channels = source.shape[1]
     bot, top = (botindex, min(topindex, channels)) if channels > 1 else (0, 1)
+    ann = _DICE["ann"]
+    if ann is not None and ann.state != "declined":
+        if ann.state != "carried":
+            raise RuntimeError("dice_loss_sum: Dice terms were announced (ops.dice_announce) but %s" %
+                               ("no two-class out_block ran since" if ann.state == "open" else "only one two-class out_block ran since: nothing carries the sums"
+                                if ann.state == "source" else "they were consumed already"))
+        is_t = lambda a, b: torch.is_tensor(a) and a.data_ptr() == b.data_ptr() and a.shape == b.shape and a.dtype == b.dtype
+        same = (is_t(source, ann.source) and len(targets_and_weights) == len(ann.terms) and (bot, top, float(eps)) == (ann.bot, ann.top, ann.eps)
+                and all(float(w) == float(aw) and (is_t(t, ann.carrier) if at is NEXT_OUTPUT else t is at) for (t, w), (at, aw) in zip(targets_and_weights, ann.terms)))
+        if not same:
+            raise RuntimeError("dice_loss_sum: the call differs from the terms announced with ops.dice_announce (operands, weights, channel range or eps)")
+        ann.state = "consumed"
+        final, terms = DiceLossSumFused.apply(source, targets_and_weights[ann.own][0], ann)
+        return final, list(terms.unbind(0))
     if not FUSED_LOSS[0] or len(targets_and_weights) > 4:
         targets_and_weights = [(onehot(t.label, channels) if isinstance(t, LabelTarget) else t, w) for t, w in targets_and_weights]
         terms = [1 - Dice.apply(source, t, bot, top, eps, True) for t, _ in targets_and_weights]
diff --git a/vae_segmentation_amd/train.py b/vae_segmentation_amd/train.py
--- a/vae_segmentation_amd/train.py
+++ b/vae_segmentation_amd/train.py
@@ -34,6 +34,12 @@
         seg_part, (dsc_loss, ce_loss) = ops.seg_loss(batch["pred"], ops.LabelTarget(label), botindex=1, topindex=n_class, eps=eps, **_seg_loss_args(loss))
         return vae_part + seg_part, {"recon_loss": recon_loss, "dice_loss": dsc_loss, "ce_loss": ce_loss, "batch": batch}
     gt = _gt(batch, label, n_class)
+    if isinstance(gt, ops.LabelTarget) and n_class == 2:
+        with ops.dice_announce([(ops.NEXT_OUTPUT, lambda_vae), (gt, 1.0)], botindex=1, topindex=n_class, eps=eps):
+            batch = joint(batch, "img", "pred", "recon")
+            final, (recon_loss, dsc_loss) = ops.dice_loss_sum(batch["pred"], [(batch["recon"], lambda_vae), (gt, 1.0)],
+                                                              botindex=1, topindex=n_class, eps=eps)
+        return final, {"recon_loss": recon_loss, "dice_loss": dsc_loss, "batch": batch}
     batch = joint(batch, "img", "pred", "recon")
     final, (recon_loss, dsc_loss) = ops.dice_loss_sum(batch["pred"], [(batch["recon"], lambda_vae), (gt, 1.0)],
                                                       botindex=1, topindex=n_class, eps=eps)
```

After: 886.8 volumes/s. No clear change (-0.6%).
